# slinderman/theano_pyglm

Measured on AMD Instinct MI355X. Metric: population ll+grad evals/sec (N neurons x T bins), higher is better.
Workload: dtype f64

## Files before the change

include/pyglm_hip.h:

```cpp
#ifndef PYGLM_HIP_H
#define PYGLM_HIP_H

#include <stdint.h>

#ifdef __cplusplus
extern "C" {
#endif

typedef struct pgl_context* pgl_handle;

#define PGL_OK 0
#define PGL_ERR_ARG (-1)
#define PGL_ERR_HIP (-2)
#define PGL_ERR_STATE (-3)
#define PGL_ERR_UNSUPPORTED (-4)

#define PGL_NLIN_EXP 0
#define PGL_NLIN_EXPLINEAR 1

#define PGL_OPT_FEATURE_F32 1
#define PGL_OPT_NCHUNKS 2
#define PGL_OPT_KERNEL 3

#define PGL_OPT_GIBBS_KERNEL 4
#define PGL_OPT_EPI_F64 5

#define PGL_OPT_TIMING 6
#define PGL_OPT_BFGS_MERGE 7

#define PGL_OPT_RECORD_KERNELS 96


const char* pgl_last_error(void);
int pgl_version(void);
int pgl_device_count(void);

int pgl_create(int N, int64_t nT, int B, int R, int nlin, double dt, int device,
               pgl_handle* out);
int pgl_destroy(pgl_handle h);
int pgl_set_option(pgl_handle h, int option, int value);

int pgl_set_spikes_u8(pgl_handle h, const uint8_t* S);
int pgl_set_spikes_f64(pgl_handle h, const double* S);

int pgl_set_basis(pgl_handle h, const double* ibasis);

int pgl_set_stim_features(pgl_handle h, const double* fstim, int Dstim);

int pgl_set_stimulus(pgl_handle h, const double* stim, int64_t Tstim, int D, double dt_stim,
                     const double* basis_x, int Bx, const double* basis_t, int Rt, int Bt,
                     int layout);
int pgl_get_stim_features(pgl_handle h, double* fstim_out);

int pgl_set_stimulus_separable(pgl_handle h, const double* stim, int64_t Tstim, int D, double dt_stim,
                               const double* basis_x, int Bx, const double* basis_t, int Rt, int Bt);

int pgl_set_time_range(pgl_handle h, int64_t t_lo, int64_t t_hi);

int pgl_ll_grad(pgl_handle h, int n_lo, int n_hi, const double* theta,
                const double* Weff, double* ll_out, double* grad_out);

int pgl_ll_grad_dev(pgl_handle h, int n_lo, int n_hi, const double* d_theta,
                    const double* d_Weff, double* d_ll, double* d_grad);
int pgl_ll_grad_list_dev(pgl_handle h, const int* d_idx, int count, const double* d_theta,
                         const double* d_Weff, double* d_ll, double* d_grad);
int pgl_sync(pgl_handle h);

int pgl_hvp_prepare_dev(pgl_handle h, int n_lo, int n_hi, const double* d_theta, const double* d_Weff);
int pgl_hvp_prepare_list_dev(pgl_handle h, const int* d_idx, int count, const double* d_theta, const double* d_Weff);
int pgl_hvp_apply_dev(pgl_handle h, const double* d_v, double* d_hv);
int pgl_hvp(pgl_handle h, int n_lo, int n_hi, const double* theta, const double* v, const double* Weff, double* hv_out);

long long pgl_bfgs_state_doubles(int M, int P);
int pgl_bfgs_init_dev(pgl_handle h, double* d_state, int M, int P, double gtol);
int pgl_bfgs_trial_dev(pgl_handle h, double* d_state, int M, int P, const int* d_rows, int L, double* d_Xt);
int pgl_bfgs_objective_dev(pgl_handle h, int L, int P, const double* d_Xt, double* d_ll_f, double* d_grad_g,
                           int prior_kind, double mu_b, double sg_b, double stim_sigma, double mu, double sigma,
                           double lam);
int pgl_bfgs_linesearch_dev(pgl_handle h, double* d_state, int M, int P, const int* d_rows, int L, const double* d_Xt,
                            const double* d_f, const double* d_g, int max_trials);
int pgl_bfgs_hmul_dev(pgl_handle h, double* d_state, int M, int P, const int* d_rows, int L, double* d_H, int ld);
int pgl_bfgs_hmul_hist_dev(pgl_handle h, double* d_state, int M, int P, const int* d_rows, int L, const double* d_hist,
                           const double* d_coef, int Kmax, double* d_ab);
int pgl_bfgs_update_dev(pgl_handle h, double* d_state, int M, int P, double gtol, int maxiter, int init_scaling, double* d_hist,
                        double* d_coef, int Kmax);
int pgl_bfgs_step_dev(pgl_handle h, double* d_state, int M, int P, const int* d_rows, int L, const double* d_Xt, double* d_ll_f,
                      double* d_grad_g, int prior_kind, double mu_b, double sg_b, double stim_sigma, double mu, double sigma,
                      double lam, int max_trials, double gtol, int maxiter, int init_scaling, double* d_hist, double* d_coef,
                      int Kmax, double* d_ab, int hk_bound, double* d_H, int ld, const int* d_pos_next, double* d_Xt_next,
                      double* flags_out);

long long pgl_ncg_state_doubles(int M, int P);
int pgl_ncg_init_dev(pgl_handle h, double* d_state, int M, int P, double* d_ll, double* d_grad, int prior_kind, double mu_b,
                     double sg_b, double stim_sigma, double mu, double sigma, double lam, int maxiter, double* d_V,
                     double* flags_out);
int pgl_ncg_cg_step_dev(pgl_handle h, double* d_state, int M, int P, double* d_hv, int prior_kind, double mu_b, double sg_b,
                        double stim_sigma, double mu, double sigma, double lam, double* d_V, double* flags_out);
int pgl_ncg_trial_dev(pgl_handle h, double* d_state, int M, int P, const int* d_rows, int L, double* d_Xt);
int pgl_ncg_search_step_dev(pgl_handle h, double* d_state, int M, int P, const int* d_rows, int L, const double* d_Xt,
                            double* d_ll_f, double* d_grad_g, int prior_kind, double mu_b, double sg_b, double stim_sigma,
                            double mu, double sigma, double lam, int maxiter, const int* d_pos_next, double* d_Xt_next,
                            double* d_V, double* flags_out);

int pgl_features(pgl_handle h, double* fS_out);

int pgl_impulse_currents(pgl_handle h, const double* w, double* I_imp_out);

int pgl_state(pgl_handle h, int n, const double* theta_n, const double* Weff_col,
              double* lam_out, double* I_net_out, double* I_stim_out);

int pgl_ll_from_current(pgl_handle h, int n_post, double I_bias, const double* I_stim,
                        const double* I_other, const double* I_col, const double* w,
                        int K, double* ll_out);

int pgl_gibbs_prepare(pgl_handle h, int n_post, const double* theta_n,
                      const double* Weff_col);
int pgl_gibbs_ll(pgl_handle h, int n_pre, double aw_cur, const double* w, int K,
                 double* ll_out);
int pgl_gibbs_update(pgl_handle h, int n_pre, double delta);

int pgl_gibbs_prepare_all(pgl_handle h, const double* theta, const double* Weff);
int pgl_gibbs_ll_cols(pgl_handle h, int ncols, const int* n_post, const int* n_pre,
                      const double* aw_cur, const double* w, int K, double* ll_out);
int pgl_gibbs_update_cols(pgl_handle h, int ncols, const int* n_post, const int* n_pre,
                          const double* delta);
int pgl_gibbs_currents(pgl_handle h, int n_post, double* x_out);

int pgl_sta(pgl_handle h, const double* stim, int64_t Tstim, int D, double dt_stim, int L,
            const int* neurons, int n_sel, double* A_out);

int pgl_leading_singular_pairs(pgl_handle h, const double* A, int n, int L, int D, double* U, double* sigma, double* V);

int pgl_simulate(int N, int64_t nT, int R, int nlin, double dt, double* X, const double* AW,
                 const double* uniforms, int64_t n_uniforms, uint64_t seed, double* S,
                 int64_t* n_exceptions_out);

int pgl_last_timing(pgl_handle h, double* fused_ms, double* total_ms);

int pgl_timing_summary(pgl_handle h, int reset, int* n_launches, double* mean_fused_ms,
                       double* mean_total_ms);

int pgl_set_stream(pgl_handle h, void* stream);

int pgl_plan_kernels(int N, int B, int R, int Dstim, long long nT, int stim, int n_lo, int count, int path, int opt_kernel,
                     int opt_f32, char* out, int cap);

int pgl_last_kernels(pgl_handle h, char* out, int cap);

int pgl_info(pgl_handle h, int n_lo, int n_hi, double* info, int n_info);

#ifdef __cplusplus
}
#endif
#endif
```

theano_pyglm_amd/_lib.py:

```python
import ctypes as C
import os

import numpy as np

_HERE = os.path.dirname(os.path.abspath(__file__))
LIB_PATH = os.environ.get('PYGLM_HIP_LIB', os.path.join(_HERE, 'libpyglm_hip.so'))

NLIN_EXP = 0
NLIN_EXPLINEAR = 1
OPT_FEATURE_F32 = 1
OPT_NCHUNKS = 2
OPT_KERNEL = 3
OPT_GIBBS_KERNEL = 4
OPT_EPI_F64 = 5
OPT_TIMING = 6
OPT_BFGS_MERGE = 7
OPT_RECORD_KERNELS = 96

SYMBOLS = [
    'pgl_last_error', 'pgl_version', 'pgl_device_count', 'pgl_create', 'pgl_destroy',
    'pgl_set_option', 'pgl_set_time_range', 'pgl_set_spikes_u8', 'pgl_set_spikes_f64', 'pgl_set_basis',
    'pgl_set_stim_features', 'pgl_set_stimulus', 'pgl_get_stim_features', 'pgl_ll_grad', 'pgl_ll_grad_dev', 'pgl_sync', 'pgl_features',
    'pgl_impulse_currents', 'pgl_state', 'pgl_ll_from_current', 'pgl_gibbs_prepare',
    'pgl_gibbs_ll', 'pgl_gibbs_update', 'pgl_last_timing', 'pgl_info', 'pgl_simulate', 'pgl_sta',
    'pgl_timing_summary', 'pgl_set_stream',
    'pgl_set_stimulus_separable', 'pgl_ll_grad_list_dev', 'pgl_gibbs_prepare_all', 'pgl_gibbs_ll_cols', 'pgl_gibbs_update_cols', 'pgl_gibbs_currents',
    'pgl_bfgs_state_doubles', 'pgl_bfgs_init_dev', 'pgl_bfgs_trial_dev', 'pgl_bfgs_objective_dev',
    'pgl_bfgs_linesearch_dev', 'pgl_bfgs_hmul_dev', 'pgl_bfgs_hmul_hist_dev', 'pgl_bfgs_update_dev', 'pgl_bfgs_step_dev', 'pgl_plan_kernels', 'pgl_last_kernels', 'pgl_leading_singular_pairs',
    'pgl_hvp_prepare_dev', 'pgl_hvp_prepare_list_dev', 'pgl_hvp_apply_dev', 'pgl_hvp',
    'pgl_ncg_state_doubles', 'pgl_ncg_init_dev', 'pgl_ncg_cg_step_dev', 'pgl_ncg_trial_dev', 'pgl_ncg_search_step_dev',
]


class PglError(RuntimeError):
    pass


def plan_kernels(N, B=5, R=200, Dstim=0, nT=300000, stim=0, n_lo=0, count=None, path=0, opt_kernel=0, opt_f32=0):
    lib = load()
    buf = C.create_string_buffer(4096)
    rc = lib.pgl_plan_kernels(int(N), int(B), int(R), int(Dstim), int(nT), int(stim), int(n_lo), int(N - n_lo if count is None else count),
                              int(path), int(opt_kernel), int(opt_f32), buf, 4096)
    if rc != 0:
        raise PglError(lib.pgl_last_error().decode())
    return [ln for ln in buf.value.decode().splitlines() if ln]


_lib = None


def _preload_torch_hip():
    if os.environ.get('PYGLM_NO_TORCH_PRELOAD'):
        return
    try:
        import importlib.util
        spec = importlib.util.find_spec('torch')
        if spec is None or not spec.submodule_search_locations:
            return
        libdir = os.path.join(list(spec.submodule_search_locations)[0], 'lib')
        for name in ('libhsa-runtime64.so', 'libamdhip64.so'):
            path = os.path.join(libdir, name)
            if os.path.exists(path):
                C.CDLL(path, mode=C.RTLD_GLOBAL)
    except Exception:
        pass


def load():
    global _lib
    if _lib is not None:
        return _lib
    if not os.path.exists(LIB_PATH):
        raise PglError("HIP library %s not found: run `python -c 'import __graft_entry__ as g; "
                       "g.build()'` (hipcc --offload-arch=gfx950). There is no CPU fallback."
                       % LIB_PATH)
    _preload_torch_hip()
    lib = C.CDLL(LIB_PATH)
    dp = C.POINTER(C.c_double)
    vp = C.c_void_p
    lib.pgl_last_error.restype = C.c_char_p
    lib.pgl_last_error.argtypes = []
    lib.pgl_version.restype = C.c_int
    lib.pgl_device_count.restype = C.c_int
    lib.pgl_create.argtypes = [C.c_int, C.c_int64, C.c_int, C.c_int, C.c_int, C.c_double, C.c_int,
                               C.POINTER(vp)]
    lib.pgl_destroy.argtypes = [vp]
    lib.pgl_set_option.argtypes = [vp, C.c_int, C.c_int]
    lib.pgl_set_time_range.argtypes = [vp, C.c_int64, C.c_int64]
    lib.pgl_set_spikes_u8.argtypes = [vp, vp]
    lib.pgl_set_spikes_f64.argtypes = [vp, vp]
    lib.pgl_set_basis.argtypes = [vp, vp]
    lib.pgl_set_stim_features.argtypes = [vp, vp, C.c_int]
    lib.pgl_set_stimulus.argtypes = [vp, vp, C.c_int64, C.c_int, C.c_double, vp, C.c_int, vp, C.c_int,
                                     C.c_int, C.c_int]
    lib.pgl_get_stim_features.argtypes = [vp, vp]
    lib.pgl_set_stimulus_separable.argtypes = [vp, vp, C.c_int64, C.c_int, C.c_double, vp, C.c_int, vp, C.c_int,
                                               C.c_int]
    lib.pgl_timing_summary.argtypes = [vp, C.c_int, C.POINTER(C.c_int), C.POINTER(C.c_double), C.POINTER(C.c_double)]
    lib.pgl_set_stream.argtypes = [vp, vp]
    lib.pgl_sta.argtypes = [vp, vp, C.c_int64, C.c_int, C.c_double, C.c_int, vp, C.c_int, vp]
    if hasattr(lib, 'pgl_leading_singular_pairs'):
        lib.pgl_leading_singular_pairs.argtypes = [vp, vp, C.c_int, C.c_int, C.c_int, vp, vp, vp]
    lib.pgl_ll_grad.argtypes = [vp, C.c_int, C.c_int, vp, vp, vp, vp]
    lib.pgl_ll_grad_dev.argtypes = [vp, C.c_int, C.c_int, vp, vp, vp, vp]
    lib.pgl_ll_grad_list_dev.argtypes = [vp, vp, C.c_int, vp, vp, vp, vp]
    lib.pgl_sync.argtypes = [vp]
    if hasattr(lib, 'pgl_hvp'):
        lib.pgl_hvp_prepare_dev.argtypes = [vp, C.c_int, C.c_int, vp, vp]
        lib.pgl_hvp_prepare_list_dev.argtypes = [vp, vp, C.c_int, vp, vp]
        lib.pgl_hvp_apply_dev.argtypes = [vp, vp, vp]
        lib.pgl_hvp.argtypes = [vp, C.c_int, C.c_int, vp, vp, vp, vp]
    if hasattr(lib, 'pgl_bfgs_hmul_dev'):
        lib.pgl_bfgs_state_doubles.argtypes = [C.c_int, C.c_int]
        lib.pgl_bfgs_init_dev.argtypes = [vp, vp, C.c_int, C.c_int, C.c_double]
        lib.pgl_bfgs_trial_dev.argtypes = [vp, vp, C.c_int, C.c_int, vp, C.c_int, vp]
        lib.pgl_bfgs_objective_dev.argtypes = [vp, C.c_int, C.c_int, vp, vp, vp, C.c_int] + [C.c_double] * 6
        lib.pgl_bfgs_linesearch_dev.argtypes = [vp, vp, C.c_int, C.c_int, vp, C.c_int, vp, vp, vp, C.c_int]
        lib.pgl_bfgs_hmul_dev.argtypes = [vp, vp, C.c_int, C.c_int, vp, C.c_int, vp, C.c_int]
        lib.pgl_bfgs_update_dev.argtypes = [vp, vp, C.c_int, C.c_int, C.c_double, C.c_int, C.c_int, vp, vp, C.c_int]
        lib.pgl_bfgs_hmul_hist_dev.argtypes = [vp, vp, C.c_int, C.c_int, vp, C.c_int, vp, vp, C.c_int, vp]
    if hasattr(lib, 'pgl_bfgs_step_dev'):
        lib.pgl_bfgs_step_dev.argtypes = ([vp, vp, C.c_int, C.c_int, vp, C.c_int, vp, vp, vp, C.c_int] + [C.c_double] * 6 +
                                          [C.c_int, C.c_double, C.c_int, C.c_int, vp, vp, C.c_int, vp, C.c_int, vp, C.c_int,
                                           vp, vp, vp])
    if hasattr(lib, 'pgl_ncg_init_dev'):
        lib.pgl_ncg_state_doubles.argtypes = [C.c_int, C.c_int]
        lib.pgl_ncg_init_dev.argtypes = [vp, vp, C.c_int, C.c_int, vp, vp, C.c_int] + [C.c_double] * 6 + [C.c_int, vp, vp]
        lib.pgl_ncg_cg_step_dev.argtypes = [vp, vp, C.c_int, C.c_int, vp, C.c_int] + [C.c_double] * 6 + [vp, vp]
        lib.pgl_ncg_trial_dev.argtypes = [vp, vp, C.c_int, C.c_int, vp, C.c_int, vp]
        lib.pgl_ncg_search_step_dev.argtypes = ([vp, vp, C.c_int, C.c_int, vp, C.c_int, vp, vp, vp, C.c_int] +
                                                [C.c_double] * 6 + [C.c_int, vp, vp, vp, vp])
    lib.pgl_features.argtypes = [vp, vp]
    lib.pgl_impulse_currents.argtypes = [vp, vp, vp]
    lib.pgl_state.argtypes = [vp, C.c_int, vp, vp, vp, vp, vp]
    lib.pgl_ll_from_current.argtypes = [vp, C.c_int, C.c_double, vp, vp, vp, vp, C.c_int, vp]
    lib.pgl_gibbs_prepare.argtypes = [vp, C.c_int, vp, vp]
    lib.pgl_gibbs_ll.argtypes = [vp, C.c_int, C.c_double, vp, C.c_int, vp]
    lib.pgl_gibbs_update.argtypes = [vp, C.c_int, C.c_double]
    lib.pgl_gibbs_prepare_all.argtypes = [vp, vp, vp]
    lib.pgl_gibbs_ll_cols.argtypes = [vp, C.c_int, vp, vp, vp, vp, C.c_int, vp]
    lib.pgl_gibbs_update_cols.argtypes = [vp, C.c_int, vp, vp, vp]
    lib.pgl_gibbs_currents.argtypes = [vp, C.c_int, vp]
    lib.pgl_last_timing.argtypes = [vp, dp, dp]
    lib.pgl_info.argtypes = [vp, C.c_int, C.c_int, vp, C.c_int]
    if hasattr(lib, 'pgl_plan_kernels'):
        lib.pgl_plan_kernels.argtypes = [C.c_int, C.c_int, C.c_int, C.c_int, C.c_longlong, C.c_int, C.c_int, C.c_int, C.c_int,
                                         C.c_int, C.c_int, C.c_char_p, C.c_int]
    if hasattr(lib, 'pgl_last_kernels'):
        lib.pgl_last_kernels.argtypes = [vp, C.c_char_p, C.c_int]
    lib.pgl_simulate.argtypes = [C.c_int, C.c_int64, C.c_int, C.c_int, C.c_double, vp, vp, vp,
                                 C.c_int64, C.c_uint64, vp, vp]
    for name in SYMBOLS:
        if 'PYGLM_HIP_LIB' in os.environ and not hasattr(lib, name):
            continue
        fn = getattr(lib, name)
        if name in ('pgl_bfgs_state_doubles', 'pgl_ncg_state_doubles'):
            fn.restype = C.c_longlong
        elif name not in ('pgl_last_error',):
            fn.restype = C.c_int
    _lib = lib
    return lib


def device_count():
    return load().pgl_device_count()


def _chk(rc):
    if rc != 0:
        raise PglError("libpyglm_hip error %d: %s" % (rc, load().pgl_last_error().decode()))


def _f64(a, shape=None):
    a = np.ascontiguousarray(a, dtype=np.float64)
    if shape is not None and tuple(a.shape) != tuple(shape):
        raise ValueError("expected shape %s, got %s" % (shape, a.shape))
    return a


def _ptr(a):
    return None if a is None else a.ctypes.data_as(C.c_void_p)


def simulate(X0, AW, nlin, dt, uniforms=None, seed=0):
    lib = load()
    X = np.array(X0, dtype=np.float64, order='C')
    nT, N = X.shape
    AW = _f64(AW)
    assert AW.ndim == 3 and AW.shape[0] == N and AW.shape[2] == N
    R = AW.shape[1]
    S = np.empty((nT, N))
    u = None if uniforms is None else _f64(uniforms)
    nexc = C.c_int64(0)
    kind = {'exp': NLIN_EXP, 'explinear': NLIN_EXPLINEAR}.get(nlin, nlin)
    _chk(lib.pgl_simulate(N, nT, R, int(kind), float(dt), _ptr(X), _ptr(AW), _ptr(u),
                          0 if u is None else u.size, int(seed), _ptr(S), C.byref(nexc)))
    return S, X, int(nexc.value)


class DeviceGlm(object):

    def __init__(self, N, nT, B, R, nlin, dt, device=0):
        self.lib = load()
        self.N, self.nT, self.B, self.R, self.dt = int(N), int(nT), int(B), int(R), float(dt)
        self.nlin = {'exp': NLIN_EXP, 'explinear': NLIN_EXPLINEAR}.get(nlin, nlin)
        self.Dstim = 0
        h = C.c_void_p()
        _chk(self.lib.pgl_create(self.N, self.nT, self.B, self.R, int(self.nlin), self.dt,
                                 int(device), C.byref(h)))
        self.h = h

    def close(self):
        if getattr(self, 'h', None) is not None and self.h.value:
            self.lib.pgl_destroy(self.h)
            self.h = C.c_void_p()

    def __del__(self):
        try:
            self.close()
        except Exception:
            pass

    @property
    def P(self):
        return 1 + self.Dstim + self.N * self.B

    def set_option(self, opt, value):
        _chk(self.lib.pgl_set_option(self.h, int(opt), int(value)))

    def set_time_range(self, t_lo, t_hi):
        _chk(self.lib.pgl_set_time_range(self.h, int(t_lo), int(t_hi)))

    def set_spikes(self, S):
        S = np.asarray(S)
        if S.shape != (self.nT, self.N):
            raise ValueError("S must be (nT,N)=(%d,%d), got %s" % (self.nT, self.N, S.shape))
        if S.dtype == np.uint8:
            S = np.ascontiguousarray(S)
            _chk(self.lib.pgl_set_spikes_u8(self.h, _ptr(S)))
        else:
            S = _f64(S)
            _chk(self.lib.pgl_set_spikes_f64(self.h, _ptr(S)))

    def set_basis(self, ibasis):
        ib = _f64(ibasis, (self.R, self.B))
        _chk(self.lib.pgl_set_basis(self.h, _ptr(ib)))

    def set_stim_features(self, fstim):
        if fstim is None:
            _chk(self.lib.pgl_set_stim_features(self.h, None, 0))
            self.Dstim = 0
            return
        f = _f64(fstim)
        if f.ndim != 2 or f.shape[0] != self.nT:
            raise ValueError("fstim must be (nT,Dstim)")
        _chk(self.lib.pgl_set_stim_features(self.h, _ptr(f), int(f.shape[1])))
        self.Dstim = int(f.shape[1])

    def set_stimulus(self, stim, dt_stim, basis_t, basis_x=None, layout=0):
        stim = _f64(stim)
        if stim.ndim != 2:
            raise ValueError("stim must be (Tstim, D)")
        bt = _f64(basis_t)
        bx = None if basis_x is None else _f64(basis_x, (stim.shape[1], np.shape(basis_x)[1]))
        Bx = stim.shape[1] if bx is None else bx.shape[1]
        _chk(self.lib.pgl_set_stimulus(self.h, _ptr(stim), stim.shape[0], stim.shape[1], float(dt_stim),
                                       _ptr(bx), int(Bx), _ptr(bt), bt.shape[0], bt.shape[1],
                                       int(layout)))
        self.Dstim = int(Bx * bt.shape[1])

    def set_stimulus_separable(self, stim, dt_stim, basis_t, basis_x=None):
        stim = _f64(stim)
        if stim.ndim != 2:
            raise ValueError("stim must be (Tstim, D)")
        bt = _f64(basis_t)
        bx = None if basis_x is None else _f64(basis_x, (stim.shape[1], np.shape(basis_x)[1]))
        Bx = stim.shape[1] if bx is None else bx.shape[1]
        _chk(self.lib.pgl_set_stimulus_separable(self.h, _ptr(stim), stim.shape[0], stim.shape[1],
                                                 float(dt_stim), _ptr(bx), int(Bx), _ptr(bt), bt.shape[0],
                                                 bt.shape[1]))
        self.Dstim = int(Bx + bt.shape[1])

    def get_stim_features(self):
        out = np.empty((self.nT, self.Dstim))
# ... 21 lines not shown
            n, L, D = A.shape
        U, sig, V = np.empty((n, L)), np.empty(n), np.empty((n, D))
        _chk(self.lib.pgl_leading_singular_pairs(self.h, _ptr(A), n, L, D, _ptr(U), _ptr(sig), _ptr(V)))
        return U, sig, V

    def ll_grad(self, theta, Weff, n_lo=0, n_hi=None, want_grad=True):
        n_hi = self.N if n_hi is None else n_hi
        npost = n_hi - n_lo
        th = _f64(theta, (npost, self.P))
        We = _f64(Weff, (self.N, self.N))
        ll = np.empty(npost)
        g = np.empty((npost, self.P)) if want_grad else None
        _chk(self.lib.pgl_ll_grad(self.h, int(n_lo), int(n_hi), _ptr(th), _ptr(We), _ptr(ll),
                                  _ptr(g)))
        return ll, g

    def ll_grad_dev(self, d_theta, d_Weff, d_ll, d_grad, n_lo=0, n_hi=None):
        n_hi = self.N if n_hi is None else n_hi
        _chk(self.lib.pgl_ll_grad_dev(self.h, int(n_lo), int(n_hi), C.c_void_p(d_theta),
                                      C.c_void_p(d_Weff), C.c_void_p(d_ll),
                                      C.c_void_p(d_grad) if d_grad else None))

    def ll_grad_list_dev(self, d_idx, count, d_theta, d_Weff, d_ll, d_grad):
        _chk(self.lib.pgl_ll_grad_list_dev(self.h, C.c_void_p(d_idx), int(count), C.c_void_p(d_theta),
                                           C.c_void_p(d_Weff), C.c_void_p(d_ll),
                                           C.c_void_p(d_grad) if d_grad else None))

    def hvp_prepare(self, d_theta, d_Weff, n_lo=0, n_hi=None, d_idx=0, count=None):
        if d_idx:
            _chk(self.lib.pgl_hvp_prepare_list_dev(self.h, C.c_void_p(d_idx), int(count), C.c_void_p(d_theta),
                                                   C.c_void_p(d_Weff)))
            return
        n_hi = self.N if n_hi is None else n_hi
        _chk(self.lib.pgl_hvp_prepare_dev(self.h, int(n_lo), int(n_hi), C.c_void_p(d_theta), C.c_void_p(d_Weff)))

    def hvp_apply(self, d_v, d_hv):
        _chk(self.lib.pgl_hvp_apply_dev(self.h, C.c_void_p(d_v), C.c_void_p(d_hv)))

    def hvp(self, theta, v, Weff, n_lo=0, n_hi=None):
        n_hi = self.N if n_hi is None else n_hi
        npost = n_hi - n_lo
        th = _f64(theta, (npost, self.P))
        vv = _f64(v, (npost, self.P))
        We = _f64(Weff, (self.N, self.N))
        out = np.empty((npost, self.P))
        _chk(self.lib.pgl_hvp(self.h, int(n_lo), int(n_hi), _ptr(th), _ptr(vv), _ptr(We), _ptr(out)))
        return out

    def bfgs_state_doubles(self, M, P):
        return int(self.lib.pgl_bfgs_state_doubles(int(M), int(P)))

    def bfgs_trial_dev(self, d_state, M, P, d_rows, L, d_Xt):
        _chk(self.lib.pgl_bfgs_trial_dev(self.h, C.c_void_p(d_state), int(M), int(P),
                                         C.c_void_p(d_rows) if d_rows else None, int(L), C.c_void_p(d_Xt)))

    def bfgs_objective_dev(self, L, P, d_Xt, d_ll_f, d_grad_g, prior_kind, mu_b, sg_b, stim_sigma, mu, sigma, lam):
        _chk(self.lib.pgl_bfgs_objective_dev(self.h, int(L), int(P), C.c_void_p(d_Xt), C.c_void_p(d_ll_f),
                                             C.c_void_p(d_grad_g), int(prior_kind), float(mu_b), float(sg_b),
                                             float(stim_sigma), float(mu), float(sigma), float(lam)))

    def bfgs_init_dev(self, d_state, M, P, gtol):
        _chk(self.lib.pgl_bfgs_init_dev(self.h, C.c_void_p(d_state), int(M), int(P), float(gtol)))

    def bfgs_linesearch_dev(self, d_state, M, P, d_rows, L, d_Xt, d_f, d_g, max_trials=100):
        _chk(self.lib.pgl_bfgs_linesearch_dev(self.h, C.c_void_p(d_state), int(M), int(P),
                                              C.c_void_p(d_rows) if d_rows else None, int(L), C.c_void_p(d_Xt),
                                              C.c_void_p(d_f), C.c_void_p(d_g), int(max_trials)))

    def bfgs_hmul_dev(self, d_state, M, P, d_rows, L, d_H, ld):
        _chk(self.lib.pgl_bfgs_hmul_dev(self.h, C.c_void_p(d_state), int(M), int(P),
                                        C.c_void_p(d_rows) if d_rows else None, int(L), C.c_void_p(d_H), int(ld)))

    def bfgs_hmul_hist_dev(self, d_state, M, P, d_rows, L, d_hist, d_coef, Kmax, d_ab):
        _chk(self.lib.pgl_bfgs_hmul_hist_dev(self.h, C.c_void_p(d_state), int(M), int(P),
                                             C.c_void_p(d_rows) if d_rows else None, int(L), C.c_void_p(d_hist),
                                             C.c_void_p(d_coef), int(Kmax), C.c_void_p(d_ab)))

    def bfgs_update_dev(self, d_state, M, P, gtol, maxiter, init_scaling=False, d_hist=0, d_coef=0, Kmax=0):
        _chk(self.lib.pgl_bfgs_update_dev(self.h, C.c_void_p(d_state), int(M), int(P), float(gtol), int(maxiter),
                                          1 if init_scaling else 0, C.c_void_p(d_hist) if d_hist else None,
                                          C.c_void_p(d_coef) if d_coef else None, int(Kmax)))

    def bfgs_step_dev(self, d_state, M, P, d_rows, L, d_Xt, d_f, d_g, prior=None, max_trials=100, gtol=1e-5, maxiter=225,
                      init_scaling=False, d_hist=0, d_coef=0, Kmax=0, d_ab=0, hk_bound=0, d_H=0, ld=0, d_pos_next=0,
                      d_Xt_next=0, flags_out=0):
        vp = lambda a: C.c_void_p(a) if a else None
        pr = (-1, 0.0, 1.0, 1.0, 0.0, 1.0, 0.0) if prior is None else prior
        _chk(self.lib.pgl_bfgs_step_dev(self.h, C.c_void_p(d_state), int(M), int(P), vp(d_rows), int(L), C.c_void_p(d_Xt),
                                        C.c_void_p(d_f), C.c_void_p(d_g), int(pr[0]), *[float(z) for z in pr[1:]],
                                        int(max_trials), float(gtol), int(maxiter), 1 if init_scaling else 0, vp(d_hist),
                                        vp(d_coef), int(Kmax), vp(d_ab), int(hk_bound), vp(d_H), int(ld), vp(d_pos_next),
                                        vp(d_Xt_next), vp(flags_out)))

    def ncg_state_doubles(self, M, P):
        return int(self.lib.pgl_ncg_state_doubles(int(M), int(P)))

    def ncg_init_dev(self, d_state, M, P, d_ll, d_grad, prior, maxiter, d_V, flags_out=0):
        _chk(self.lib.pgl_ncg_init_dev(self.h, C.c_void_p(d_state), int(M), int(P), C.c_void_p(d_ll), C.c_void_p(d_grad),
                                       int(prior[0]), *[float(z) for z in prior[1:]], int(maxiter), C.c_void_p(d_V),
                                       C.c_void_p(flags_out) if flags_out else None))

    def ncg_cg_step_dev(self, d_state, M, P, d_hv, prior, d_V, flags_out=0):
        _chk(self.lib.pgl_ncg_cg_step_dev(self.h, C.c_void_p(d_state), int(M), int(P), C.c_void_p(d_hv), int(prior[0]),
                                          *[float(z) for z in prior[1:]], C.c_void_p(d_V),
                                          C.c_void_p(flags_out) if flags_out else None))

    def ncg_trial_dev(self, d_state, M, P, d_rows, L, d_Xt):
        _chk(self.lib.pgl_ncg_trial_dev(self.h, C.c_void_p(d_state), int(M), int(P),
                                        C.c_void_p(d_rows) if d_rows else None, int(L), C.c_void_p(d_Xt)))

    def ncg_search_step_dev(self, d_state, M, P, d_rows, L, d_Xt, d_f, d_g, prior, maxiter, d_pos_next, d_Xt_next, d_V,
                            flags_out=0):
        vp = lambda a: C.c_void_p(a) if a else None
        _chk(self.lib.pgl_ncg_search_step_dev(self.h, C.c_void_p(d_state), int(M), int(P), vp(d_rows), int(L),
                                              C.c_void_p(d_Xt), C.c_void_p(d_f), C.c_void_p(d_g), int(prior[0]),
                                              *[float(z) for z in prior[1:]], int(maxiter), vp(d_pos_next), vp(d_Xt_next),
                                              C.c_void_p(d_V), vp(flags_out)))

    def sync(self):
        _chk(self.lib.pgl_sync(self.h))

    def last_timing(self):
        a, b = C.c_double(), C.c_double()
        _chk(self.lib.pgl_last_timing(self.h, C.byref(a), C.byref(b)))
        return a.value, b.value

    def last_kernels(self):
        buf = C.create_string_buffer(16384)
        _chk(self.lib.pgl_last_kernels(self.h, buf, 16384))
        return [ln for ln in buf.value.decode().splitlines() if ln]

    def timing_summary(self, reset=True):
        n, a, b = C.c_int(), C.c_double(), C.c_double()
        _chk(self.lib.pgl_timing_summary(self.h, 1 if reset else 0, C.byref(n), C.byref(a), C.byref(b)))
        return n.value, a.value, b.value

    def set_stream(self, stream_ptr):
        if stream_ptr is None:
            _chk(self.lib.pgl_set_stream(self.h, None))
            return
        if int(stream_ptr) == 0:
            raise ValueError("stream handle 0 is the NULL stream: create a torch.cuda.Stream(), make it "
                             "current and pass its .cuda_stream")
        _chk(self.lib.pgl_set_stream(self.h, C.c_void_p(int(stream_ptr))))

    def info(self, n_lo=0, n_hi=None):
        n_hi = self.N if n_hi is None else n_hi
        v = np.zeros(13)
        _chk(self.lib.pgl_info(self.h, int(n_lo), int(n_hi), _ptr(v), 13))
        keys = ['blocks', 'threads', 'chunks', 'ktiles', 'lds_bytes', 'tile_rows', 'flops',
                'bytes', 'events', 'kernel_version', 'resident_feature_bytes', 'streamed_bytes', 'stim_path']
        return dict(zip(keys, v.tolist()))

    def features(self):
        out = np.empty((self.nT, self.N, self.B))
        _chk(self.lib.pgl_features(self.h, _ptr(out)))
        return out

    def impulse_currents(self, w):
        w = _f64(w, (self.N, self.B))
        out = np.empty((self.nT, self.N))
        _chk(self.lib.pgl_impulse_currents(self.h, _ptr(w), _ptr(out)))
        return out

    def state(self, n, theta_n, Weff_col):
        th = _f64(theta_n, (self.P,))
        wc = _f64(Weff_col, (self.N,))
        lam = np.empty(self.nT)
        inet = np.empty(self.nT)
        istim = np.empty(self.nT)
        _chk(self.lib.pgl_state(self.h, int(n), _ptr(th), _ptr(wc), _ptr(lam), _ptr(inet),
                                _ptr(istim)))
        return lam, inet, istim

    def ll_from_current(self, n_post, I_bias, I_stim, I_other, I_col, ws):
        ws = _f64(np.atleast_1d(ws))
        I_other = _f64(I_other, (self.nT,))
        I_col = _f64(I_col, (self.nT,))
        I_stim = None if I_stim is None else _f64(I_stim, (self.nT,))
        out = np.empty(len(ws))
        _chk(self.lib.pgl_ll_from_current(self.h, int(n_post), float(I_bias), _ptr(I_stim),
                                          _ptr(I_other), _ptr(I_col), _ptr(ws), len(ws),
                                          _ptr(out)))
        return out

    def gibbs_prepare(self, n_post, theta_n, Weff_col):
        th = _f64(theta_n, (self.P,))
        wc = _f64(Weff_col, (self.N,))
        _chk(self.lib.pgl_gibbs_prepare(self.h, int(n_post), _ptr(th), _ptr(wc)))

    def gibbs_ll(self, n_pre, aw_cur, ws):
        ws = _f64(np.atleast_1d(ws))
        out = np.empty(len(ws))
        _chk(self.lib.pgl_gibbs_ll(self.h, int(n_pre), float(aw_cur), _ptr(ws), len(ws),
                                   _ptr(out)))
        return out

    def gibbs_update(self, n_pre, delta):
        _chk(self.lib.pgl_gibbs_update(self.h, int(n_pre), float(delta)))

    def gibbs_prepare_all(self, theta, Weff):
        th = _f64(theta, (self.N, self.P))
        We = _f64(Weff, (self.N, self.N))
        _chk(self.lib.pgl_gibbs_prepare_all(self.h, _ptr(th), _ptr(We)))

    def gibbs_ll_cols(self, n_post, n_pre, aw_cur, ws):
        n_post = np.ascontiguousarray(n_post, dtype=np.int32)
        n_pre = np.ascontiguousarray(n_pre, dtype=np.int32)
        ws = _f64(ws)
        if ws.ndim == 1:
            ws = ws[None, :]
        aw = _f64(aw_cur, (len(n_post),))
        if n_pre.shape != n_post.shape or ws.shape[0] != len(n_post):
            raise ValueError("n_post, n_pre, aw_cur, ws must describe the same columns")
        out = np.empty(ws.shape)
        K = ws.shape[1]
        for k0 in range(0, K, 16):
            wk = np.ascontiguousarray(ws[:, k0:k0 + 16])
            ok = np.empty(wk.shape)
            _chk(self.lib.pgl_gibbs_ll_cols(self.h, len(n_post), _ptr(n_post), _ptr(n_pre), _ptr(aw),
                                            _ptr(wk), wk.shape[1], _ptr(ok)))
            out[:, k0:k0 + 16] = ok
        return out

    def gibbs_update_cols(self, n_post, n_pre, delta):
        n_post = np.ascontiguousarray(n_post, dtype=np.int32)
        n_pre = np.ascontiguousarray(n_pre, dtype=np.int32)
        d = _f64(delta, (len(n_post),))
        if len(n_post) == 0:
            return
        _chk(self.lib.pgl_gibbs_update_cols(self.h, len(n_post), _ptr(n_post), _ptr(n_pre), _ptr(d)))

    def gibbs_currents(self, n_post, nrows=None):
        out = np.empty(self.nT if nrows is None else int(nrows))
        _chk(self.lib.pgl_gibbs_currents(self.h, int(n_post), _ptr(out)))
        return out
```

theano_pyglm_amd/csrc/pglm_capi.hip:

```cpp
#include "pglm_kernels.hip.h"
#include "../../include/pyglm_hip.h"

#include <algorithm>
#include <cmath>
#include <cstdio>
#include <cstring>
#include <map>
#include <mutex>
#include <string>
#include <thread>
#include <type_traits>
#include <vector>

static thread_local std::string g_err;
static int fail(int code, const std::string& msg)
{
    g_err = msg;
    return code;
}
static thread_local std::vector<std::string>* g_dry = nullptr;
static thread_local std::vector<std::string>* g_rec = nullptr;
#define HIPCHK(expr)                                                                         \
    do {                                                                                     \
        hipError_t e_ = (expr);                                                              \
        if (e_ != hipSuccess)                                                                \
            return fail(PGL_ERR_HIP, std::string(#expr) + ": " + hipGetErrorString(e_));     \
    } while (0)

struct DevBuf {
    void* p = nullptr;
    size_t cap = 0;
};

struct pgl_context {
    int N = 0, B = 0, R = 0, nlin = 0, device = 0;
    int64_t nT = 0;
    double dt = 0;
    int Dstim = 0, Kimp = 0, Ktot = 0, nT16 = 0;
    int numCU = 256;
    hipStream_t stream = nullptr;
    hipStream_t own_stream = nullptr;
    hipStream_t aux_stream = nullptr;
    hipEvent_t ev_fork = nullptr, ev_join = nullptr;
    static constexpr int NEV = 256;
    hipEvent_t evr[NEV][4] = {};
    hipEvent_t* ev = evr[0];
    long long ev_launches = 0;
    bool have_spikes = false, have_basis = false;
    int64_t nnz = 0;
    DevBuf S, ST, spk, wlo, whi, phi, fstim;
    std::vector<int> h_ptr;
    std::vector<int2> h_ev;
    int Rk = 0;
    DevBuf theta, Weff, ll, grad, Wfrag, bias, Gpart, llpart, gbpart, Xbuf;
    struct ImgSlot {
        DevBuf buf;
        int key = 0, tile0 = 0, ntiles = 0;
        unsigned long long stamp = 0;
    };
    static constexpr int NIMG = 8;
    ImgSlot imgs[NIMG];
    int img_cur = 0;
    unsigned long long img_clock = 0;
    double* pin_out = nullptr;
    DevBuf IimpT, Inet, Istim, tmpA, tmpB, tmpC, wsmall, part, outK, lam, wcol, thetan;
    bool sep = false;
    int sepBt = 0, sepBx = 0, sepRt = 0;
    int64_t sepT = 0;
    double sep_dt_stim = 0;
    DevBuf zf, zfT, sbt, Yf, Qb, Qf, spart;
    bool sepf = false;
    int sepq = 0, sepM = 0, sepJ = 0, sepBTp = 0;
    int sepNH = 0, sepGs = 0;
    bool sepA_ok = false;
    DevBuf sepC, sepA, sepAT, sepD, YfT, Hb, wpart, QvT;
    int opt_sepf = 0;
    const int* cur_pidx = nullptr;
    int gibbs_npost = -1;
    double gibbs_bias = 0;
    DevBuf GX, gtheta, gargs, gpart, gout, ghs, gfs;
    DevBuf staA;
    int sta_n = 0, sta_L = 0, sta_D = 0;
    int gx_xs = 0;
    int64_t gx_t_lo = 0, gx_t_hi = 0;
    unsigned char* pin_args = nullptr;
    size_t pin_args_cap = 0;
    int opt_f32 = 0, opt_nchunks = 0, opt_dbg = 0, opt_kernel = 0, opt_ptw = 0, opt_gibbs = 0, opt_finw = 0, opt_sb6 = 0, opt_epi64 = 0, opt_timing = 1, opt_slice_cols = 0, opt_hlp = 0, opt_pbmajor = 0;
    int opt_img32 = 0;
    int opt_record = 0;
    std::vector<std::string> last_kernels;
    long long call_no = 0;
    int64_t t_lo = 0, t_hi = 0;
    bool timing_valid = false;
    double* flags_host[4] = {nullptr, nullptr, nullptr, nullptr};
    double* flags_dev[4] = {nullptr, nullptr, nullptr, nullptr};
    int flags_next = 0;
    int opt_bfgs_merge = 65536;
    bool hvp_ok = false, hvp_fused = false, hvp_list = false;
    int hvp_n_lo = 0, hvp_count = 0;
    int64_t hvp_t_lo = 0, hvp_t_hi = 0;
    DevBuf Cbuf, hvp_idx, hvp_Weff, hvp_ll, hvp_v, hvp_out;
    std::vector<double> hvp_host;
};

static int ensure(DevBuf& b, size_t bytes)
{
    if (g_dry) return PGL_OK;
    if (bytes <= b.cap && b.p) return PGL_OK;
    if (b.p) (void)hipFree(b.p);
    b.p = nullptr;
    b.cap = 0;
    if (bytes == 0) bytes = 16;
    HIPCHK(hipMalloc(&b.p, bytes));
    b.cap = bytes;
    return PGL_OK;
}
static void release(DevBuf& b)
{
    if (b.p) (void)hipFree(b.p);
    b.p = nullptr;
    b.cap = 0;
}
static int find_img(const pgl_context* h, int key, int tile0, int ntiles)
{
    for (int i = 0; i < pgl_context::NIMG; ++i)
        if (h->imgs[i].key == key && h->imgs[i].tile0 == tile0 && h->imgs[i].ntiles == ntiles && h->imgs[i].buf.p)
            return i;
    return -1;
}
static void invalidate_images(pgl_context* h)
{
    h->hvp_ok = false;
    for (int i = 0; i < pgl_context::NIMG; ++i) h->imgs[i].key = 0;
}
static bool img_room(const pgl_context* h, size_t want)
{
    size_t free_b = 0, total_b = 0;
    if (hipMemGetInfo(&free_b, &total_b) != hipSuccess) return true;
    size_t reclaim = 0;
    int lru = 0;
    for (int i = 1; i < pgl_context::NIMG; ++i)
        if (h->imgs[i].stamp < h->imgs[lru].stamp) lru = i;
    for (int i = 0; i < pgl_context::NIMG; ++i)
        if (h->imgs[i].key == 0) reclaim = std::max(reclaim, h->imgs[i].buf.cap);
    reclaim = std::max(reclaim, h->imgs[lru].buf.cap);
    return want <= reclaim || want - reclaim <= free_b / 10 * 9;
}
#define ENSURE(buf, bytes)                       \
    do {                                         \
        int rc_ = ensure(buf, bytes);            \
        if (rc_ != PGL_OK) return rc_;           \
    } while (0)

#include "pglm_plan.h"
#include "pglm_launch.h"

static int gibbs_rate_wg_per_cu(size_t lds)
{
    static std::map<size_t, int> cache;
    static std::mutex mu;
    std::lock_guard<std::mutex> lock(mu);
    int& c = cache[lds];
    if (c == 0) {
        int occ = 0;
        if (hipOccupancyMaxActiveBlocksPerMultiprocessor(&occ, k_gibbs_rate_cols, 256, lds) != hipSuccess || occ < 1)
            occ = 3;
        c = occ;
    }
    return c;
}

template <int J, int BT>
static void launch_sepf(int which, const SepfParams& sp, hipStream_t s);
static inline bool gemm_aligned(const void* p, long long ld) { return ((uintptr_t)p % 16) == 0 && (ld % 2) == 0; }

template <int J, int BT>
static void launch_sepf(int which, const SepfParams& sp, hipStream_t s)
{
    const long long nF = sp.F1 - sp.F0 + 1;
    const int nG = (sp.nPT + 3) / 4;
    dim3 grid((unsigned)((nF + 3) / 4), (unsigned)nG);
    if (which == 0) hipLaunchKernelGGL((k_sepf_fwd<J, BT>), grid, dim3(256), 0, s, sp);
    else if (which == 1) hipLaunchKernelGGL((k_sepf_bwd<J, BT>), grid, dim3(256), 0, s, sp);
    else {
        const int nA = (int)((sp.Tstim + 15) / 16) * nG;
        hipLaunchKernelGGL((k_sepf_finish<J, BT>), dim3(nA + nG * BT), dim3(1024), 0, s, sp, nA, nG);
    }
}

extern "C" {

const char* pgl_last_error(void) { return g_err.c_str(); }
int pgl_version(void) { return 103; }

int pgl_device_count(void)
{
    int n = 0;
    if (hipGetDeviceCount(&n) != hipSuccess) return 0;
    return n;
}

int pgl_create(int N, int64_t nT, int B, int R, int nlin, double dt, int device, pgl_handle* out)
{
    if (!out) return fail(PGL_ERR_ARG, "out is NULL");
    *out = nullptr;
    if (N <= 0 || nT <= 0 || B <= 0 || R <= 0) return fail(PGL_ERR_ARG, "N, nT, B, R must be positive");
    if (B > PGL_MAXB) return fail(PGL_ERR_UNSUPPORTED, "B > 8 basis functions");
    if (nlin != PGL_NLIN_EXP && nlin != PGL_NLIN_EXPLINEAR) return fail(PGL_ERR_ARG, "unknown nonlinearity");
    if (nT > (int64_t)1 << 30) return fail(PGL_ERR_UNSUPPORTED, "nT > 2^30 bins");
    if (!(dt > 0)) return fail(PGL_ERR_ARG, "dt must be positive");
    int ndev = 0;
    HIPCHK(hipGetDeviceCount(&ndev));
    if (ndev <= 0) return fail(PGL_ERR_HIP, "no HIP device visible");
    if (device < 0 || device >= ndev) return fail(PGL_ERR_ARG, "device index out of range");
    HIPCHK(hipSetDevice(device));
    pgl_context* h = new pgl_context();
    h->N = N; h->nT = nT; h->B = B; h->R = R; h->Rk = R; h->nlin = nlin; h->dt = dt; h->device = device;
    h->Kimp = N * B; h->Ktot = h->Kimp; h->nT16 = (int)((nT + 15) / 16);
    h->t_lo = 0; h->t_hi = nT;
    hipDeviceProp_t prop;
    if (hipGetDeviceProperties(&prop, device) == hipSuccess) h->numCU = prop.multiProcessorCount;
    hipError_t e = hipStreamCreateWithFlags(&h->own_stream, hipStreamNonBlocking);
    if (e != hipSuccess) { delete h; return fail(PGL_ERR_HIP, hipGetErrorString(e)); }
    h->stream = h->own_stream;
    {
        int prio_lo = 0, prio_hi = 0;
        if (hipDeviceGetStreamPriorityRange(&prio_lo, &prio_hi) != hipSuccess) prio_hi = 0;
        e = hipStreamCreateWithPriority(&h->aux_stream, hipStreamNonBlocking, prio_hi);
    }
    if (e == hipSuccess) e = hipEventCreateWithFlags(&h->ev_fork, hipEventDisableTiming);
    if (e == hipSuccess) e = hipEventCreateWithFlags(&h->ev_join, hipEventDisableTiming);
    if (e != hipSuccess) { pgl_destroy(h); return fail(PGL_ERR_HIP, hipGetErrorString(e)); }
    for (int s = 0; s < pgl_context::NEV; ++s)
        for (int i = 0; i < 4; ++i) {
            e = hipEventCreate(&h->evr[s][i]);
            if (e != hipSuccess) { pgl_destroy(h); return fail(PGL_ERR_HIP, hipGetErrorString(e)); }
        }
    *out = h;
    return PGL_OK;
}

int pgl_destroy(pgl_handle h)
{
    if (!h) return PGL_OK;
    (void)hipSetDevice(h->device);
    if (h->stream) (void)hipStreamSynchronize(h->stream);
    DevBuf* bufs[] = {&h->S, &h->ST, &h->spk, &h->wlo, &h->whi, &h->phi, &h->fstim, &h->theta,
                      &h->Weff, &h->ll, &h->grad, &h->Wfrag, &h->bias, &h->Gpart, &h->llpart,
                      &h->gbpart, &h->Xbuf, &h->imgs[0].buf, &h->imgs[1].buf, &h->imgs[2].buf, &h->imgs[3].buf, &h->imgs[4].buf, &h->imgs[5].buf, &h->imgs[6].buf, &h->imgs[7].buf, &h->IimpT, &h->Inet, &h->Istim, &h->tmpA, &h->tmpB, &h->tmpC,
                      &h->wsmall, &h->part, &h->outK, &h->lam, &h->wcol, &h->thetan, &h->GX, &h->gtheta,
                      &h->gargs, &h->gpart, &h->gout, &h->ghs, &h->gfs, &h->zf, &h->zfT, &h->sbt, &h->Yf, &h->Qb, &h->Qf,
                      &h->spart, &h->sepC, &h->sepA, &h->sepAT, &h->sepD, &h->YfT, &h->Hb, &h->wpart, &h->QvT, &h->staA,
                      &h->Cbuf, &h->hvp_idx, &h->hvp_Weff, &h->hvp_ll, &h->hvp_v, &h->hvp_out};
    for (DevBuf* b : bufs) release(*b);
    for (int s = 0; s < pgl_context::NEV; ++s)
        for (int i = 0; i < 4; ++i)
            if (h->evr[s][i]) (void)hipEventDestroy(h->evr[s][i]);
    if (h->pin_out) (void)hipHostFree(h->pin_out);
    if (h->pin_args) (void)hipHostFree(h->pin_args);
    if (h->ev_fork) (void)hipEventDestroy(h->ev_fork);
    if (h->ev_join) (void)hipEventDestroy(h->ev_join);
    if (h->aux_stream) { (void)hipStreamSynchronize(h->aux_stream); (void)hipStreamDestroy(h->aux_stream); }
    if (h->own_stream) (void)hipStreamDestroy(h->own_stream);
    delete h;
    return PGL_OK;
}

int pgl_set_time_range(pgl_handle h, int64_t t_lo, int64_t t_hi)
{
    if (!h) return fail(PGL_ERR_ARG, "null handle");
    if (t_lo < 0 || t_hi > h->nT || t_lo >= t_hi) return fail(PGL_ERR_ARG, "bad time range");
    if (t_lo % 16 != 0) return fail(PGL_ERR_ARG, "t_lo must be a multiple of 16 bins");
    h->t_lo = t_lo;
    h->t_hi = t_hi;
    return PGL_OK;
}

int pgl_set_option(pgl_handle h, int option, int value)
{
    if (!h) return fail(PGL_ERR_ARG, "null handle");
    switch (option) {
    case PGL_OPT_FEATURE_F32: h->opt_f32 = (value == 1) ? 1 : 0; h->opt_img32 = (value == 2) ? 1 : 0; return PGL_OK;
    case 99: h->opt_dbg = value; return PGL_OK;
    case 98: h->opt_ptw = value; return PGL_OK;
    case 97: if (value < 0 || value > 16) return fail(PGL_ERR_ARG, "finalize waves: 0 (auto) .. 16"); h->opt_finw = value; return PGL_OK;
    case 91: h->opt_pbmajor = value; return PGL_OK;
    case 92: h->opt_hlp = value; return PGL_OK;
    case 93: h->opt_slice_cols = value; return PGL_OK;
    case 94: h->opt_sepf = value; return PGL_OK;
    case 95: h->opt_sb6 = value; return PGL_OK;
    case PGL_OPT_RECORD_KERNELS: h->opt_record = value ? 1 : 0; h->last_kernels.clear(); return PGL_OK;
    case PGL_OPT_KERNEL: h->opt_kernel = value; return PGL_OK;
    case PGL_OPT_GIBBS_KERNEL: h->opt_gibbs = value; return PGL_OK;
    case PGL_OPT_EPI_F64: h->opt_epi64 = value ? 1 : 0; return PGL_OK;
    case PGL_OPT_TIMING: if (value < 0) return fail(PGL_ERR_ARG, "timing interval < 0"); h->opt_timing = value; h->call_no = 0; return PGL_OK;
    case PGL_OPT_BFGS_MERGE: if (value < 0) return fail(PGL_ERR_ARG, "merge threshold < 0"); h->opt_bfgs_merge = value; return PGL_OK;
    case PGL_OPT_NCHUNKS: if (value < 0) return fail(PGL_ERR_ARG, "nchunks < 0"); h->opt_nchunks = value; return PGL_OK;
    }
    return fail(PGL_ERR_ARG, "unknown option");
}

static int upload_windows(pgl_handle h)
{
    const int N = h->N, nT16 = h->nT16;
    const std::vector<int>& ptr = h->h_ptr;
    const std::vector<int2>& ev = h->h_ev;
    std::vector<int> wlo((size_t)nT16 * N), whi((size_t)nT16 * N);
    for (int n = 0; n < N; ++n) {
        int lo = ptr[n], hi = ptr[n];
        const int end = ptr[n + 1];
        for (int tile = 0; tile < nT16; ++tile) {
            const int64_t klo = (int64_t)16 * tile - h->Rk;
            const int64_t khi = (int64_t)16 * tile + 15;
            while (lo < end && ev[(size_t)lo].x < klo) ++lo;
            while (hi < end && ev[(size_t)hi].x < khi) ++hi;
            wlo[(size_t)tile * N + n] = lo;
            whi[(size_t)tile * N + n] = hi;
        }
    }
    ENSURE(h->wlo, wlo.size() * 4);
    ENSURE(h->whi, whi.size() * 4);
    HIPCHK(hipMemcpyAsync(h->wlo.p, wlo.data(), wlo.size() * 4, hipMemcpyHostToDevice, h->stream));
    HIPCHK(hipMemcpyAsync(h->whi.p, whi.data(), whi.size() * 4, hipMemcpyHostToDevice, h->stream));
    HIPCHK(hipStreamSynchronize(h->stream));
    return PGL_OK;
}

static int upload_spikes(pgl_handle h, const uint8_t* S)
{
    HIPCHK(hipSetDevice(h->device));
    const int N = h->N;
    const int64_t nT = h->nT;
    const int nth = (int)std::max<int64_t>(1, std::min<int64_t>(std::min<int64_t>(16, std::max(1u, std::thread::hardware_concurrency())),
                                                               nT / 65536));
    std::vector<int64_t> t0s(nth + 1);
    for (int i = 0; i <= nth; ++i) t0s[i] = nT * i / nth;
    std::vector<std::vector<int>> slab((size_t)nth, std::vector<int>((size_t)N, 0));
    auto run = [&](auto&& fn) {
        std::vector<std::thread> th;
        for (int i = 1; i < nth; ++i) th.emplace_back(fn, i);
        fn(0);
        for (auto& t : th) t.join();
    };
    run([&](const int i) {
        int* c = slab[(size_t)i].data();
        for (int64_t t = t0s[i]; t < t0s[i + 1]; ++t) {
            const uint8_t* row = S + t * N;
            for (int n = 0; n < N; ++n) c[n] += row[n] != 0;
        }
    });
    std::vector<int> cnt(N + 1, 0);
    for (int n = 0; n < N; ++n) {
        int tot = cnt[n];
        for (int i = 0; i < nth; ++i) {
            const int c = slab[(size_t)i][(size_t)n];
            slab[(size_t)i][(size_t)n] = tot;
            tot += c;
        }
        cnt[n + 1] = tot;
    }
    const int64_t nnz = cnt[N];
    std::vector<int2> ev((size_t)std::max<int64_t>(nnz, 1));
    run([&](const int i) {
        int* cur = slab[(size_t)i].data();
        for (int64_t t = t0s[i]; t < t0s[i + 1]; ++t) {
            const uint8_t* row = S + t * N;
            for (int n = 0; n < N; ++n)
                if (row[n]) ev[(size_t)cur[n]++] = make_int2((int)t, (int)row[n]);
        }
    });
    h->h_ptr = cnt;
    h->h_ev.swap(ev);
    const std::vector<int2>& evr = h->h_ev;
    const size_t s_rows = (size_t)h->nT16 * 16;
    ENSURE(h->S, s_rows * N);
    ENSURE(h->ST, (size_t)nT * N);
    ENSURE(h->spk, evr.size() * sizeof(int2));
    HIPCHK(hipMemsetAsync((uint8_t*)h->S.p + (size_t)nT * N, 0, (s_rows - (size_t)nT) * N, h->stream));
    HIPCHK(hipMemcpyAsync(h->S.p, S, (size_t)nT * N, hipMemcpyHostToDevice, h->stream));
    HIPCHK(hipMemcpyAsync(h->spk.p, evr.data(), evr.size() * sizeof(int2), hipMemcpyHostToDevice, h->stream));
    {
        const int rc = upload_windows(h);
        if (rc) return rc;
    }
    dim3 grid((unsigned)((nT + 63) / 64), (unsigned)((N + 63) / 64));
    hipLaunchKernelGGL(k_transpose_u8, grid, dim3(256), 0, h->stream, (const uint8_t*)h->S.p,
                       (uint8_t*)h->ST.p, (long long)nT, N);
    HIPCHK(hipGetLastError());
    HIPCHK(hipStreamSynchronize(h->stream));
    h->nnz = nnz;
    h->have_spikes = true;
    h->gibbs_npost = -1;
    invalidate_images(h);
    h->gx_xs = 0;
    return PGL_OK;
}

int pgl_set_spikes_u8(pgl_handle h, const uint8_t* S)
{
    if (!h || !S) return fail(PGL_ERR_ARG, "null argument");
    return upload_spikes(h, S);
}

int pgl_set_spikes_f64(pgl_handle h, const double* S)
{
    if (!h || !S) return fail(PGL_ERR_ARG, "null argument");
// ... 365 lines not shown
}

int pgl_sta(pgl_handle h, const double* stim, int64_t Tstim, int D, double dt_stim, int L,
            const int* neurons, int n_sel, double* A_out)
{
    if (!h || !stim) return fail(PGL_ERR_ARG, "null argument");
    if (!h->have_spikes) return fail(PGL_ERR_STATE, "pgl_set_spikes_* has not been called");
    if (Tstim <= 0 || D <= 0 || L <= 0 || !(dt_stim > 0)) return fail(PGL_ERR_ARG, "bad stimulus description");
    const int nSel = neurons ? n_sel : h->N;
    if (nSel <= 0 || nSel > 65535) return fail(PGL_ERR_ARG, "bad neuron selection");
    std::vector<int> eoff((size_t)2 * nSel);
    for (int i = 0; i < nSel; ++i) {
        const int n = neurons ? neurons[i] : i;
        if (n < 0 || n >= h->N) return fail(PGL_ERR_ARG, "neuron index out of range");
        eoff[2 * i] = h->h_ptr[n];
        eoff[2 * i + 1] = h->h_ptr[n + 1];
    }
    const long long LD = (long long)L * D;
    const long long xb = (LD + 255) / 256;
    if (xb > 0x7fffffffLL) return fail(PGL_ERR_UNSUPPORTED, "L*D too large");
    int echunks = (int)std::min<long long>(64, std::max<long long>(1, 4096 / (xb * nSel)));
    HIPCHK(hipSetDevice(h->device));
    DevBuf dstim, distim, deoff, dpart, dA;
    auto cleanup = [&]() { release(dstim); release(distim); release(deoff); release(dpart); release(dA); };
    auto keep = [&]() {
        release(h->staA);
        h->staA = dA;
        dA = DevBuf();
        h->sta_n = nSel; h->sta_L = L; h->sta_D = D;
    };
    const double ratio = dt_stim / h->dt;
    const long long q = llround(ratio);
    const bool frame_rate = q >= 1 && std::fabs(ratio - (double)q) <= 1e-9 * ratio && (Tstim % 2) == 0 && Tstim >= 2 &&
                            (long long)nSel * L * Tstim <= (1ll << 28) && h->opt_sepf != 7;
    int rc = ensure(dstim, (size_t)Tstim * D * 8);
    if (!rc && !frame_rate) rc = ensure(distim, (size_t)h->nT * D * 8);
    if (!rc) rc = ensure(deoff, eoff.size() * sizeof(int));
    if (!rc && !frame_rate) rc = ensure(dpart, (size_t)echunks * nSel * LD * 8);
    if (!rc) rc = ensure(dA, (size_t)nSel * LD * 8);
    if (rc) { cleanup(); return rc; }
    hipError_t e = hipMemcpyAsync(dstim.p, stim, (size_t)Tstim * D * 8, hipMemcpyHostToDevice, h->stream);
    if (e == hipSuccess)
        e = hipMemcpyAsync(deoff.p, eoff.data(), eoff.size() * sizeof(int), hipMemcpyHostToDevice, h->stream);
    if (frame_rate && e == hipSuccess) {
        DevBuf dW, dscale;
        std::vector<double> scale((size_t)nSel);
        for (int i = 0; i < nSel; ++i) {
            double cnt = 0.0;
            for (int j = eoff[2 * i]; j < eoff[2 * i + 1]; ++j) cnt += (double)h->h_ev[j].y;
            scale[i] = (h->dt / dt_stim) / cnt;
        }
        rc = ensure(dW, (size_t)nSel * L * Tstim * 8);
        if (!rc) rc = ensure(dscale, (size_t)nSel * 8);
        if (rc) { release(dW); release(dscale); cleanup(); return rc; }
        e = hipMemcpyAsync(dscale.p, scale.data(), (size_t)nSel * 8, hipMemcpyHostToDevice, h->stream);
        if (e == hipSuccess) {
            hipLaunchKernelGGL(k_sta_weights, dim3((unsigned)((Tstim + 255) / 256), (unsigned)L, (unsigned)nSel), dim3(256), 0,
                               h->stream, (const int2*)h->spk.p, (const int*)deoff.p, (const double*)dscale.p, L,
                               (long long)Tstim, (int)q, (double*)dW.p);
            e = hipGetLastError();
        }
        if (e == hipSuccess) {
            const int Mrows = nSel * L;
            hipLaunchKernelGGL((k_gemm_kc<1, 0, 16>), dim3((unsigned)((Mrows + 15) / 16), (unsigned)((D + 15) / 16)), dim3(512), 0,
                               h->stream, (const double*)dW.p, (long long)Tstim, (const double*)dstim.p, (long long)D,
                               (double*)dA.p, (long long)D, 1LL, Mrows, D, (int)Tstim);
            e = hipGetLastError();
        }
        if (e == hipSuccess && A_out)
            e = hipMemcpyAsync(A_out, dA.p, (size_t)nSel * LD * 8, hipMemcpyDeviceToHost, h->stream);
        if (e == hipSuccess) e = hipStreamSynchronize(h->stream);
        release(dW); release(dscale);
        if (e == hipSuccess && !A_out) keep();
        cleanup();
        if (e != hipSuccess) return fail(PGL_ERR_HIP, std::string("pgl_sta: ") + hipGetErrorString(e));
        return PGL_OK;
    }
    if (e == hipSuccess) {
        const long long total = (long long)h->nT * D;
        const int blocks = (int)std::min<long long>((total + 255) / 256, 65535);
        hipLaunchKernelGGL(k_stim_project, dim3(blocks), dim3(256), 0, h->stream, (const double*)dstim.p,
                           (long long)Tstim, D, dt_stim, h->dt, (const double*)nullptr, D,
                           (double*)distim.p, (long long)h->nT);
        e = hipGetLastError();
    }
    if (e == hipSuccess) {
        hipLaunchKernelGGL(k_sta, dim3((unsigned)xb, (unsigned)nSel, (unsigned)echunks), dim3(256), 0,
                           h->stream, (const int2*)h->spk.p, (const int*)deoff.p, (const double*)distim.p,
                           D, L, (double*)dpart.p);
        e = hipGetLastError();
    }
    if (e == hipSuccess) {
        hipLaunchKernelGGL(k_sta_finish, dim3((unsigned)xb, (unsigned)nSel), dim3(256), 0, h->stream,
                           (const double*)dpart.p, (const int2*)h->spk.p, (const int*)deoff.p, LD, echunks,
                           h->dt / dt_stim, (double*)dA.p);
        e = hipGetLastError();
    }
    if (e == hipSuccess && A_out)
        e = hipMemcpyAsync(A_out, dA.p, (size_t)nSel * LD * 8, hipMemcpyDeviceToHost, h->stream);
    if (e == hipSuccess) e = hipStreamSynchronize(h->stream);
    if (e == hipSuccess && !A_out) keep();
    cleanup();
    if (e != hipSuccess) return fail(PGL_ERR_HIP, std::string("pgl_sta: ") + hipGetErrorString(e));
    return PGL_OK;
}

int pgl_get_stim_features(pgl_handle h, double* fstim_out)
{
    if (h && h->sep) return fail(PGL_ERR_STATE, "a separable stimulus has no dense feature matrix");
    if (!h || !fstim_out) return fail(PGL_ERR_ARG, "null argument");
    if (h->Dstim <= 0) return fail(PGL_ERR_STATE, "no stimulus features on the device");
    HIPCHK(hipSetDevice(h->device));
    HIPCHK(hipMemcpyAsync(fstim_out, h->fstim.p, (size_t)h->nT * h->Dstim * 8, hipMemcpyDeviceToHost, h->stream));
    HIPCHK(hipStreamSynchronize(h->stream));
    return PGL_OK;
}

static int check_ready(pgl_handle h)
{
    if (!h) return fail(PGL_ERR_ARG, "null handle");
    if (!h->have_spikes) return fail(PGL_ERR_STATE, "pgl_set_spikes_* has not been called");
    if (!h->have_basis) return fail(PGL_ERR_STATE, "pgl_set_basis has not been called");
    return PGL_OK;
}

static void fill_params(pgl_handle h, const Plan& pl, const Slice& sl, int n_lo, bool want_grad,
                        int mode, FusedParams& fp)
{
    fp.nT = h->nT; fp.N = sl.Ns; fp.B = h->B; fp.R = h->Rk; fp.nlin = h->nlin;
    fp.Dstim = sl.Ds; fp.Kimp = sl.Ns * h->B; fp.Ktot = fp.Kimp + sl.Ds; fp.dt = h->dt;
    fp.Nall = h->N; fp.np0 = sl.np0; fp.DsAll = h->Dstim; fp.ds0 = sl.ds0;
    fp.mode = mode; fp.Xbuf = (double*)h->Xbuf.p; fp.xstride = pl.nPT * 16;
    fp.sepA = nullptr; fp.sepZ = nullptr; fp.sepTheta = nullptr; fp.sepT = 0;
    fp.sepLdy = fp.sepQ = fp.sepM = fp.sepNH = fp.sepG = fp.sepBt = 0;
    fp.sepAT = nullptr; fp.sepD = nullptr; fp.sepB0 = 0; fp.sepSL = 0;
    fp.spk = (const int2*)h->spk.p; fp.wlo = (const int*)h->wlo.p; fp.whi = (const int*)h->whi.p;
    fp.S = (const uint8_t*)h->S.p; fp.fstim = (const double*)h->fstim.p; fp.phi = (const double*)h->phi.p;
    fp.Wfrag = (const double*)h->Wfrag.p; fp.bias = (const double*)h->bias.p;
    fp.n_lo = n_lo; fp.npost = pl.npost; fp.nPT = pl.nPT;
    fp.nT16 = h->nT16; fp.tilesPerChunk = pl.tilesPerChunk; fp.nChunks = pl.nChunks; fp.nTiles = pl.nTiles;
    fp.pb_major = pl.pb_major;
    fp.rsf = pl.rsf;
    fp.RP = pl.RP;
    fp.Gpart = (double*)h->Gpart.p; fp.llpart = (double*)h->llpart.p; fp.gbpart = (double*)h->gbpart.p;
    fp.tile0 = pl.tile0;
    fp.t_hi = h->t_hi;
    fp.want_grad = want_grad ? 1 : 0;
    fp.dbg = h->opt_dbg;
    fp.Fimg = (const unsigned char*)h->imgs[h->img_cur].buf.p;
    fp.img_tile0 = h->imgs[h->img_cur].tile0;
    fp.pidx = h->cur_pidx;
    fp.theta = nullptr; fp.Weff = nullptr; fp.P = 1 + h->Dstim + h->Kimp;
    fp.epi64 = h->opt_epi64 ? 2 : 0;
}

static bool plan_reads_theta(const Plan& pl)
{
    return pl.version == 6 || (pl.version == 7 && pl.KS <= PGL_WREG_MAX);
}

static int launch_prep(pgl_handle h, const Plan& pl, const Slice& sl, int n_lo, const double* d_theta,
                       const double* d_Weff)
{
    if (g_dry) return PGL_OK;
    ENSURE(h->Wfrag, (size_t)pl.nPT * pl.KS * 64 * 8);
    ENSURE(h->bias, (size_t)pl.nPT * 16 * 8);
    const long long total = (long long)pl.nPT * pl.KS * 64;
    const int blocks = (int)std::min<long long>((total + 255) / 256, 1024);
    hipLaunchKernelGGL(k_prep_w, dim3(blocks), dim3(256), 0, h->stream, d_theta, d_Weff,
                       (double*)h->Wfrag.p, (double*)h->bias.p, sl.Ns, h->B, sl.Ds, sl.Ns * h->B,
                       sl.Ns * h->B + sl.Ds, pl.KS, n_lo, pl.npost, pl.nPT, 1,
                       h->N, sl.np0, h->Dstim, sl.ds0, h->cur_pidx);
    HIPCHK(hipGetLastError());
    return PGL_OK;
}

static int launch_finalize_grad(pgl_handle h, const Plan& pl, const Slice& sl, int n_lo,
                                const double* d_Weff, double* d_ll, double* d_grad, bool with_ll = false,
                                int kt0 = 0, int nkt = -1, hipStream_t stream = nullptr,
                                const double* wtpart = nullptr, int nwt = 0, int ldy = 0)
{
    if (g_dry) return PGL_OK;
    if (nkt < 0) nkt = pl.KT;
    if (!stream) stream = h->stream;
    const long long nfrag = (long long)pl.nPT * nkt * 256;
    int nwf = h->opt_finw > 0 ? h->opt_finw : std::max(4, std::min(8, pl.nChunks / 32));
    if (with_ll) nwf = std::max(nwf, 4);
    int blocks = (int)((nfrag + 63) / 64);
    if (with_ll) blocks += pl.npost;
    if (with_ll && wtpart) blocks += h->sepBt;
    hipLaunchKernelGGL(k_finalize, dim3(blocks), dim3(64 * nwf), 0, stream, (const double*)h->Gpart.p,
                       (const double*)h->llpart.p, (const double*)h->gbpart.p, d_Weff, d_ll, d_grad,
                       sl.Ns, h->B, sl.Ds, sl.Ns * h->B, sl.Ns * h->B + sl.Ds, pl.KT, n_lo, pl.npost,
                       pl.nPT, pl.nChunks, h->N, sl.np0, h->Dstim, sl.ds0, with_ll ? pl.KSPLIT : 0, kt0,
                       nkt, h->cur_pidx, wtpart, nwt, ldy, h->sepBt);
    HIPCHK(hipGetLastError());
    return PGL_OK;
}

static int ensure_feature_images(pgl_handle h, int ktl, int kth, int tile0, int ntiles, const Slice* sl = nullptr,
                                 int slice_no = 0, int blk = 0)
{
    if (g_dry) return PGL_OK;
    const int key = (sl ? (slice_no + 1) << 16 : 0) | (blk ? img_key6(ktl, blk) : ktl << 8 | kth);
    int slot = find_img(h, key, tile0, ntiles);
    if (slot >= 0) {
        h->img_cur = slot;
        h->imgs[slot].stamp = ++h->img_clock;
        return PGL_OK;
    }
    slot = 0;
    for (int i = 0; i < pgl_context::NIMG; ++i)
        if (h->imgs[i].key == 0) { slot = i; break; }
        else if (h->imgs[i].stamp < h->imgs[slot].stamp) slot = i;
    pgl_context::ImgSlot& im = h->imgs[slot];
    im.key = 0;
    const size_t bytes = (size_t)ntiles * (kth ? img_pair_bytes(ktl, kth) : img_bytes6(ktl, blk));
    if (bytes > im.buf.cap) {
        for (int i = 0; i < pgl_context::NIMG; ++i)
            if (i != slot && h->imgs[i].key == 0) release(h->imgs[i].buf);
    }
    ENSURE(im.buf, bytes);
    dim3 grid((unsigned)ntiles, kth ? 2 : 1);
    hipLaunchKernelGGL(k_build_fimg, grid, dim3(256), (size_t)h->B * h->Rk * 8, h->stream,
                       (const int2*)h->spk.p, (const int*)h->wlo.p, (const int*)h->whi.p,
                       (const double*)h->phi.p, (const double*)h->fstim.p, (long long)h->nT, sl ? sl->Ns : h->N, h->B,
                       h->Rk, sl ? sl->Ds : (h->sep ? 0 : h->Dstim), ktl, kth, tile0, (unsigned char*)im.buf.p,
                       h->N, sl ? sl->np0 : 0, h->Dstim, sl ? sl->ds0 : 0, blk);
    HIPCHK(hipGetLastError());
    im.key = key;
    im.tile0 = tile0;
    im.ntiles = ntiles;
    im.stamp = ++h->img_clock;
    h->img_cur = slot;
    return PGL_OK;
}


struct KernelRecord {
    explicit KernelRecord(pgl_context* h)
    {
        if (h->opt_record && !g_dry) {
            h->last_kernels.clear();
            g_rec = &h->last_kernels;
        }
    }
    ~KernelRecord() { g_rec = nullptr; }
};


static int ensure_partials(pgl_handle h, const std::vector<Plan>& plans, bool with_G)
{
    size_t maxG = 0, maxLL = 0;
    for (const Plan& pl : plans) {
        maxG = std::max(maxG, (size_t)pl.nChunks * pl.nPT * pl.KT * 256 * 8);
        maxLL = std::max(maxLL, (size_t)pl.nChunks * pl.nPT * pl.KSPLIT * 64 * 8);
    }
    ENSURE(h->llpart, maxLL);
    ENSURE(h->gbpart, maxLL);
    if (with_G) ENSURE(h->Gpart, maxG);
    return PGL_OK;
}

struct RowRange {
    int xs;
    long long row0, row1;
};
static RowRange row_range(const pgl_context* h, const Plan& p0)
{
    return RowRange{p0.nPT * 16, (long long)p0.tile0 * 16, std::min<long long>(h->nT, (long long)(p0.tile0 + p0.nTiles) * 16)};
}
static int zero_slab(pgl_handle h, double* X, const RowRange& rr)
{
    if (g_dry) return PGL_OK;
    HIPCHK(hipMemsetAsync(X + rr.row0 * rr.xs, 0, (size_t)(rr.row1 - rr.row0) * rr.xs * 8, h->stream));
    return PGL_OK;
}

static int ensure_tile_slab(pgl_handle h, const Plan& pl)
{
    const size_t need = (size_t)pl.nTiles * pl.nPT * 256 * 8;
    const bool fresh = need > h->Xbuf.cap || !h->Xbuf.p;
    ENSURE(h->Xbuf, need);
    if (fresh && !g_dry) HIPCHK(hipMemsetAsync(h->Xbuf.p, 0, need, h->stream));
    return PGL_OK;
}

static int ensure_plan_images(pgl_handle h, const Plan& pl)
{
    if (pl.version == 5) return ensure_feature_images(h, pl.ktl, pl.kth, pl.tile0, pl.nTiles);
    if (pl.version == 6 || pl.version == 7)
        return ensure_feature_images(h, pl.KT, 0, pl.tile0, pl.nTiles, nullptr, 0, (pl.version == 6 && pl.sb6 == 2) ? 1 + pl.img32 : 0);
    return PGL_OK;
}

static int launch_finalize_ll(pgl_handle h, const Plan& pl, double* d_ll, double* d_grad)
{
    if (g_dry) return PGL_OK;
    hipLaunchKernelGGL(k_finalize_ll, dim3(pl.npost), dim3(256), 0, h->stream, (const double*)h->llpart.p,
                       (const double*)h->gbpart.p, d_ll, d_grad, 1 + h->Dstim + h->Kimp, pl.npost, pl.nPT, pl.nChunks, pl.KSPLIT);
    HIPCHK(hipGetLastError());
    return PGL_OK;
}

static int forward_slices(pgl_handle h, const std::vector<Slice>& slices, const std::vector<Plan>& plans, int n_lo,
                          const double* d_theta, const double* d_Weff, double* X, int xs, const char* what)
{
    for (size_t i = 0; i < slices.size(); ++i) {
        int rc = launch_prep(h, plans[i], slices[i], n_lo, d_theta, d_Weff);
        if (rc) return rc;
        FusedParams fp;
        fill_params(h, plans[i], slices[i], n_lo, false, 1, fp);
        fp.Xbuf = X;
        fp.xstride = xs;
        hipError_t e = launch_plan(plans[i], fp, h->stream);
        if (e != hipSuccess) return fail(PGL_ERR_HIP, std::string(what) + hipGetErrorString(e));
    }
    return PGL_OK;
}

static int row_pass(pgl_handle h, const Plan& p0, const RowRange& rr, int n_lo, const double* c, double* d_ll, double* d_out)
{
    if (g_dry) return PGL_OK;
    const int rows = 512;
    const long long nrows = h->t_hi - h->t_lo;
    const int nblk = (int)((nrows + rows - 1) / rows);
    ENSURE(h->tmpA, (size_t)nblk * p0.npost * 8);
    ENSURE(h->tmpB, (size_t)nblk * p0.npost * 8);
    const dim3 grid((unsigned)nblk, (unsigned)((p0.npost + 255) / 256));
    if (c)
        hipLaunchKernelGGL(k_hvp_rows_mul, grid, dim3(256), 0, h->stream, (double*)h->Xbuf.p, c, rr.xs, (const double*)h->bias.p,
                           p0.npost, (long long)h->t_lo, (long long)h->t_hi, rows, (double*)h->tmpA.p, (double*)h->tmpB.p);
    else
        hipLaunchKernelGGL(k_rows_epilogue, grid, dim3(256), 0, h->stream, (double*)h->Xbuf.p, rr.xs, (const double*)h->bias.p,
                           (const uint8_t*)h->S.p, h->N, n_lo, p0.npost, (long long)h->t_lo, (long long)h->t_hi, rows, h->nlin,
                           h->dt, (double*)h->tmpA.p, (double*)h->tmpB.p, h->cur_pidx);
    HIPCHK(hipGetLastError());
    if (rr.row1 > h->t_hi) {
        hipLaunchKernelGGL(k_rows_zero, dim3(64), dim3(256), 0, h->stream, (double*)h->Xbuf.p, rr.xs, (long long)h->t_hi, rr.row1);
        HIPCHK(hipGetLastError());
    }
    hipLaunchKernelGGL(k_rows_reduce, dim3(p0.npost), dim3(64), 0, h->stream, (const double*)h->tmpA.p,
                       (const double*)h->tmpB.p, nblk, p0.npost, 1 + h->Dstim + h->Kimp, d_ll, d_out);
    HIPCHK(hipGetLastError());
    return PGL_OK;
}

static int backward_slices(pgl_handle h, const std::vector<Slice>& slices, const std::vector<Plan>& plans, int n_lo,
                           const double* d_theta, const double* d_Weff, double* d_ll, double* d_out)
{
    for (size_t i = 0; i < slices.size(); ++i) {
        int rc = launch_prep(h, plans[i], slices[i], n_lo, d_theta, d_Weff);
        if (rc) return rc;
        FusedParams fp;
        fill_params(h, plans[i], slices[i], n_lo, true, 2, fp);
        hipError_t e = launch_plan(plans[i], fp, h->stream);
        if (e != hipSuccess) return fail(PGL_ERR_HIP, std::string("backward launch: ") + hipGetErrorString(e));
        rc = launch_finalize_grad(h, plans[i], slices[i], n_lo, d_Weff, d_ll, d_out);
        if (rc) return rc;
    }
    return PGL_OK;
}

static int enqueue_ll_grad(pgl_handle h, int n_lo, int n_hi, const double* d_theta,
                           const double* d_Weff, double* d_ll, double* d_grad)
{
    KernelRecord record(h);
    std::vector<Slice> slices;
    std::vector<Plan> plans;
    bool sepf = false, sliced = false, wide = false;
    {
        int rc = select_plans(h, n_lo, n_hi, slices, plans, sepf, sliced, &wide);
        if (rc) return rc;
    }
    {
        int rc = ensure_partials(h, plans, d_grad != nullptr);
        if (rc) return rc;
    }

    const bool rec = h->opt_timing > 0 && (h->call_no++ % h->opt_timing) == 0;
    if (rec) {
        h->ev = h->evr[h->ev_launches % pgl_context::NEV];
        HIPCHK(hipEventRecord(h->ev[0], h->stream));
    }
    if (sepf) {
        const Plan& pl = plans[0];
        const bool direct = plan_reads_theta(pl);
        int rc = direct ? PGL_OK : launch_prep(h, pl, slices[0], n_lo, d_theta, d_Weff);
        if (rc) return rc;
        ENSURE(h->Xbuf, (size_t)pl.nTiles * pl.nPT * 256 * 8);
        rc = ensure_plan_images(h, pl);
        if (rc) return rc;
        if (rec) HIPCHK(hipEventRecord(h->ev[1], h->stream));
        SepfParams sp{};
        const bool fused_fwd = pl.version == 7 && fused7_built(pl.KT, pl.nw7, 2) && h->sepA_ok && h->opt_sepf != 3;
        const bool fused_bwd = fused_fwd && d_grad && fused7_built(pl.KT, pl.nw7, 3) && h->opt_sepf != 4;
        rc = sepf_forward(h, pl, d_theta, sp, fused_fwd);
        if (rc) return rc;
        if (fused_bwd && !g_dry) {
            const long long q = h->sepq, M = h->sepM;
            const long long tE = (long long)pl.tile0 + pl.nTiles - 1;
            sp.B0 = std::max<long long>(((long long)pl.tile0 * 16) / q - M, 0);
            sp.B1 = std::max<long long>((tE * 16) / q - M, 0);
            const long long span = ((M + 1) * q + 15) / 16 + 1;
            sp.SL = (int)(span / pl.tilesPerChunk) + 2;
            sp.tilesPerChunk = pl.tilesPerChunk;
            ENSURE(h->sepD, (size_t)(sp.B1 - sp.B0 + 1) * sp.SL * pl.nPT * 320 * 8);
            sp.D = (const double*)h->sepD.p;
        }
        FusedParams fp;
        fill_params(h, pl, slices[0], n_lo, d_grad != nullptr, 0, fp);
        if (direct) {
            fp.theta = d_theta;
            fp.Weff = d_Weff;
        }
        if (fused_fwd) {
            fp.sepA = (const double*)h->sepA.p; fp.sepZ = sp.YfT; fp.sepTheta = d_theta; fp.sepT = h->sepT;
            fp.sepLdy = sp.ldy; fp.sepQ = h->sepq; fp.sepM = h->sepM; fp.sepNH = h->sepNH; fp.sepG = h->sepGs;
            fp.sepBt = h->sepBt;
        }
        if (fused_bwd) {
            fp.sepAT = (const double*)h->sepAT.p; fp.sepD = (double*)h->sepD.p; fp.sepB0 = sp.B0; fp.sepSL = sp.SL;
        }
        hipError_t e = hipSuccess;
        if (pl.version == 5) {
            e = launch_fused5(pl, fp, h->stream, 1, 1);
            if (e == hipSuccess && d_grad) e = launch_fused5(pl, fp, h->stream, 2);
        } else {
            e = launch_fused7(pl, fp, h->stream, fused_bwd ? 3 : (fused_fwd ? 2 : 1));
        }
        if (e != hipSuccess) return fail(PGL_ERR_HIP, std::string("fused launch: ") + hipGetErrorString(e));
        if (d_grad) {
            int nwt = 0;
            rc = sepf_backward(h, sp, d_grad, fused_bwd, &nwt);
            if (rc) return rc;
            if (rec) HIPCHK(hipEventRecord(h->ev[2], h->stream));
            rc = launch_finalize_grad(h, pl, slices[0], n_lo, d_Weff, d_ll, d_grad, true, 0, -1, nullptr,
                                      fused_bwd ? (const double*)h->wpart.p : nullptr, nwt, sp.ldy);
            if (rc) return rc;
        } else {
            if (rec) HIPCHK(hipEventRecord(h->ev[2], h->stream));
            rc = launch_finalize_ll(h, pl, d_ll, d_grad);
            if (rc) return rc;
        }
    } else if (!sliced) {
        const Plan& pl = plans[0];
        const bool direct = plan_reads_theta(pl);
        int rc = direct ? PGL_OK : launch_prep(h, pl, slices[0], n_lo, d_theta, d_Weff);
        if (rc) return rc;
        if ((pl.version == 4 || pl.version == 5) && d_grad) {
            rc = ensure_tile_slab(h, pl);
            if (rc) return rc;
        }
        rc = ensure_plan_images(h, pl);
        if (rc) return rc;
        FusedParams fp;
        fill_params(h, pl, slices[0], n_lo, d_grad != nullptr, 0, fp);
        if (direct) {
            fp.theta = d_theta;
            fp.Weff = d_Weff;
        }
        if (rec) HIPCHK(hipEventRecord(h->ev[1], h->stream));
        hipError_t e = launch_plan(pl, fp, h->stream);
        if (e != hipSuccess) return fail(PGL_ERR_HIP, std::string("fused launch: ") + hipGetErrorString(e));
        if (rec) HIPCHK(hipEventRecord(h->ev[2], h->stream));
        rc = d_grad ? launch_finalize_grad(h, pl, slices[0], n_lo, d_Weff, d_ll, d_grad, true) : launch_finalize_ll(h, pl, d_ll, d_grad);
        if (rc) return rc;
    } else if (wide) {
        const Plan& p0 = plans[0];
        const size_t S = slices.size();
        ENSURE(h->Xbuf, (size_t)p0.nTiles * p0.nPT * 256 * 8);
        std::vector<int> slot(S);
        for (size_t i = 0; i < S; ++i) {
            int rc = ensure_feature_images(h, plans[i].ktl, plans[i].kth, p0.tile0, p0.nTiles, &slices[i], (int)i);
            if (rc) return rc;
            slot[i] = h->img_cur;
        }
        if (rec) HIPCHK(hipEventRecord(h->ev[1], h->stream));
        auto params = [&](const size_t i, FusedParams& fp) {
            h->img_cur = slot[i];
            fill_params(h, plans[i], slices[i], n_lo, d_grad != nullptr, 0, fp);
        };
        for (size_t i = 0; i < S; ++i) {
            int rc = launch_prep(h, plans[i], slices[i], n_lo, d_theta, d_Weff);
            if (rc) return rc;
            FusedParams fp;
            params(i, fp);
            const bool last = i + 1 == S;
            hipError_t e = launch_fused5_wide(plans[i], fp, h->stream, last ? 2 : (i == 0 ? 0 : 1));
            if (e == hipSuccess && last && d_grad) e = launch_fused5_wide(plans[i], fp, h->stream, 3);
            if (e != hipSuccess) return fail(PGL_ERR_HIP, std::string("wide launch: ") + hipGetErrorString(e));
        }
        if (d_grad) {
            int rc = launch_finalize_grad(h, plans[S - 1], slices[S - 1], n_lo, d_Weff, d_ll, d_grad, true);
            if (rc) return rc;
            for (size_t i = 0; i + 1 < S; ++i) {
                FusedParams fp;
                params(i, fp);
                hipError_t e = launch_fused5_wide(plans[i], fp, h->stream, 4);
                if (e == hipSuccess) e = launch_fused5_wide(plans[i], fp, h->stream, 3);
                if (e != hipSuccess) return fail(PGL_ERR_HIP, std::string("wide backward launch: ") + hipGetErrorString(e));
                rc = launch_finalize_grad(h, plans[i], slices[i], n_lo, d_Weff, d_ll, d_grad);
                if (rc) return rc;
            }
        } else {
            int rc = launch_finalize_ll(h, plans[S - 1], d_ll, d_grad);
            if (rc) return rc;
        }
        if (rec) HIPCHK(hipEventRecord(h->ev[2], h->stream));
    } else {
        const Plan& p0 = plans[0];
        const RowRange rr = row_range(h, p0);
        ENSURE(h->Xbuf, (size_t)h->nT * rr.xs * 8);
        double* X = (double*)h->Xbuf.p;
        int rc = zero_slab(h, X, rr);
        if (rc) return rc;
        if (rec) HIPCHK(hipEventRecord(h->ev[1], h->stream));
        SepParams sp;
        if (h->sep) {
            if (h->cur_pidx) return fail(PGL_ERR_UNSUPPORTED, "neuron lists with a separable stimulus");
            rc = sep_forward(h, d_theta, p0.npost, X, rr.xs, h->t_lo, h->t_hi, sp);
            if (rc) return rc;
        }
        rc = forward_slices(h, slices, plans, n_lo, d_theta, d_Weff, X, rr.xs, "forward launch: ");
        if (rc) return rc;
        rc = row_pass(h, p0, rr, n_lo, nullptr, d_ll, d_grad);
        if (rc) return rc;
        if (d_grad) {
            rc = backward_slices(h, slices, plans, n_lo, d_theta, d_Weff, d_ll, d_grad);
            if (rc) return rc;
            if (h->sep) {
                rc = sep_backward(h, sp, d_grad);
                if (rc) return rc;
            }
        }
        if (rec) HIPCHK(hipEventRecord(h->ev[2], h->stream));
    }
    if (rec) HIPCHK(hipEventRecord(h->ev[3], h->stream));
    h->timing_valid = rec;
    if (rec) ++h->ev_launches;
    return PGL_OK;
}

int pgl_ll_grad_dev(pgl_handle h, int n_lo, int n_hi, const double* d_theta, const double* d_Weff,
                    double* d_ll, double* d_grad)
{
    int rc = check_ready(h);
    if (rc) return rc;
    if (!d_theta || !d_Weff || !d_ll) return fail(PGL_ERR_ARG, "null argument");
    HIPCHK(hipSetDevice(h->device));
    if (n_lo < 0 || n_hi > h->N || n_lo >= n_hi) return fail(PGL_ERR_ARG, "bad neuron range");
    return enqueue_ll_grad(h, n_lo, n_hi, d_theta, d_Weff, d_ll, d_grad);
}

int pgl_ll_grad_list_dev(pgl_handle h, const int* d_idx, int count, const double* d_theta,
                         const double* d_Weff, double* d_ll, double* d_grad)
{
    int rc = check_ready(h);
    if (rc) return rc;
    if (!d_idx || !d_theta || !d_Weff || !d_ll) return fail(PGL_ERR_ARG, "null argument");
    if (count <= 0 || count > h->N) return fail(PGL_ERR_ARG, "bad neuron count");
    HIPCHK(hipSetDevice(h->device));
    h->cur_pidx = d_idx;
    rc = enqueue_ll_grad(h, 0, count, d_theta, d_Weff, d_ll, d_grad);
    h->cur_pidx = nullptr;
    return rc;
}



static int enqueue_hvp_prepare(pgl_handle h, int n_lo, int n_hi, const double* d_theta, const double* d_Weff)
{
    KernelRecord record(h);
    std::vector<Slice> slices;
    std::vector<Plan> plans;
    bool fused = false;
    int rc = hvp_select(h, n_lo, n_hi, slices, plans, fused);
    if (rc) return rc;
    rc = ensure_partials(h, plans, false);
    if (rc) return rc;
    const Plan& p0 = plans[0];
    const RowRange rr = row_range(h, p0);
    long long total = 0;
    double* cb = nullptr;
    if (fused) {
        total = (long long)p0.nTiles * p0.nPT * 256;
        ENSURE(h->Cbuf, (size_t)total * 8);
        cb = (double*)h->Cbuf.p;
        rc = launch_prep(h, p0, slices[0], n_lo, d_theta, d_Weff);
        if (rc) return rc;
        rc = ensure_plan_images(h, p0);
        if (rc) return rc;
        FusedParams fp;
        fill_params(h, p0, slices[0], n_lo, false, 0, fp);
        fp.Xbuf = cb;
        hipError_t e = launch_hvp5(p0, fp, nullptr, h->stream, 1);
        if (e != hipSuccess) return fail(PGL_ERR_HIP, std::string("curvature forward launch: ") + hipGetErrorString(e));
    } else {
        total = (rr.row1 - rr.row0) * rr.xs;
        ENSURE(h->Cbuf, (size_t)h->nT * rr.xs * 8);
        cb = (double*)h->Cbuf.p + rr.row0 * rr.xs;
        rc = zero_slab(h, (double*)h->Cbuf.p, rr);
        if (rc) return rc;
        rc = forward_slices(h, slices, plans, n_lo, d_theta, d_Weff, (double*)h->Cbuf.p, rr.xs, "curvature forward launch: ");
        if (rc) return rc;
    }
    if (!g_dry) {
        const int blocks = (int)std::min<long long>((total + 255) / 256, 8 * 1024);
        hipLaunchKernelGGL(k_hvp_curv, dim3(blocks), dim3(256), 0, h->stream, cb, (const double*)h->bias.p,
                           (const uint8_t*)h->S.p, h->N, n_lo, p0.npost, h->cur_pidx, rr.xs, rr.row0, (long long)h->t_hi, total,
                           fused ? 1 : 0, h->nlin, h->dt);
        HIPCHK(hipGetLastError());
    }
    h->hvp_fused = fused;
    return PGL_OK;
}

static int enqueue_hvp_apply(pgl_handle h, const double* d_v, double* d_hv)
{
    KernelRecord record(h);
    const int n_lo = h->hvp_list ? 0 : h->hvp_n_lo, n_hi = n_lo + h->hvp_count;
    const double* d_Weff = (const double*)h->hvp_Weff.p;
    std::vector<Slice> slices;
    std::vector<Plan> plans;
    bool fused = false;
    int rc = hvp_select(h, n_lo, n_hi, slices, plans, fused);
    if (rc) return rc;
    if (fused != h->hvp_fused) return fail(PGL_ERR_STATE, "the dispatch changed since pgl_hvp_prepare_*: prepare again");
    rc = ensure_partials(h, plans, true);
// ... 388 lines not shown
    int rc = check_ready(h);
    if (rc) return rc;
    if (!theta || !Weff || !ll_out) return fail(PGL_ERR_ARG, "null argument");
    HIPCHK(hipSetDevice(h->device));
    if (n_lo < 0 || n_hi > h->N || n_lo >= n_hi) return fail(PGL_ERR_ARG, "bad neuron range");
    const size_t P = 1 + (size_t)h->Dstim + h->Kimp;
    const size_t np = (size_t)(n_hi - n_lo);
    ENSURE(h->theta, np * P * 8);
    ENSURE(h->Weff, (size_t)h->N * h->N * 8);
    ENSURE(h->ll, np * 8);
    if (grad_out) ENSURE(h->grad, np * P * 8);
    HIPCHK(hipMemcpyAsync(h->theta.p, theta, np * P * 8, hipMemcpyHostToDevice, h->stream));
    HIPCHK(hipMemcpyAsync(h->Weff.p, Weff, (size_t)h->N * h->N * 8, hipMemcpyHostToDevice, h->stream));
    rc = enqueue_ll_grad(h, n_lo, n_hi, (const double*)h->theta.p, (const double*)h->Weff.p,
                         (double*)h->ll.p, grad_out ? (double*)h->grad.p : nullptr);
    if (rc) return rc;
    HIPCHK(hipMemcpyAsync(ll_out, h->ll.p, np * 8, hipMemcpyDeviceToHost, h->stream));
    if (grad_out)
        HIPCHK(hipMemcpyAsync(grad_out, h->grad.p, np * P * 8, hipMemcpyDeviceToHost, h->stream));
    HIPCHK(hipStreamSynchronize(h->stream));
    return PGL_OK;
}

int pgl_last_timing(pgl_handle h, double* fused_ms, double* total_ms)
{
    if (!h) return fail(PGL_ERR_ARG, "null handle");
    if (!h->timing_valid) return fail(PGL_ERR_STATE, "the last pgl_ll_grad call recorded no events (none yet, or PGL_OPT_TIMING skipped it)");
    HIPCHK(hipSetDevice(h->device));
    HIPCHK(hipEventSynchronize(h->ev[3]));
    float a = 0, b = 0;
    HIPCHK(hipEventElapsedTime(&a, h->ev[1], h->ev[2]));
    HIPCHK(hipEventElapsedTime(&b, h->ev[0], h->ev[3]));
    if (fused_ms) *fused_ms = a;
    if (total_ms) *total_ms = b;
    return PGL_OK;
}

int pgl_timing_summary(pgl_handle h, int reset, int* n_launches, double* mean_fused_ms, double* mean_total_ms)
{
    if (!h) return fail(PGL_ERR_ARG, "null handle");
    HIPCHK(hipSetDevice(h->device));
    HIPCHK(hipStreamSynchronize(h->stream));
    const long long n = std::min<long long>(h->ev_launches, pgl_context::NEV);
    double sa = 0, sb = 0;
    for (long long i = 0; i < n; ++i) {
        hipEvent_t* ev = h->evr[(h->ev_launches - 1 - i) % pgl_context::NEV];
        float a = 0, b = 0;
        HIPCHK(hipEventElapsedTime(&a, ev[1], ev[2]));
        HIPCHK(hipEventElapsedTime(&b, ev[0], ev[3]));
        sa += a;
        sb += b;
    }
    if (n_launches) *n_launches = (int)n;
    if (mean_fused_ms) *mean_fused_ms = n ? sa / n : 0.0;
    if (mean_total_ms) *mean_total_ms = n ? sb / n : 0.0;
    if (reset) h->ev_launches = 0;
    return PGL_OK;
}

int pgl_set_stream(pgl_handle h, void* stream)
{
    if (!h) return fail(PGL_ERR_ARG, "null handle");
    HIPCHK(hipSetDevice(h->device));
    HIPCHK(hipStreamSynchronize(h->stream));
    h->stream = stream ? (hipStream_t)stream : h->own_stream;
    h->ev_launches = 0;
    h->timing_valid = false;
    return PGL_OK;
}

static int enqueue_gibbs_forward(pgl_handle h);

int pgl_last_kernels(pgl_handle h, char* out, int cap)
{
    if (!h || !out || cap <= 0) return fail(PGL_ERR_ARG, "null argument");
    if (!h->opt_record) return fail(PGL_ERR_STATE, "kernel recording is off (PGL_OPT_RECORD_KERNELS)");
    std::string all;
    for (const std::string& n : h->last_kernels) all += n + "\n";
    if ((int)all.size() + 1 > cap) return fail(PGL_ERR_ARG, "output buffer too small");
    std::memcpy(out, all.c_str(), all.size() + 1);
    return PGL_OK;
}

int pgl_plan_kernels(int N, int B, int R, int Dstim, long long nT, int stim, int n_lo, int count, int path, int opt_kernel,
                     int opt_f32, char* out, int cap)
{
    if (!out || cap <= 0) return fail(PGL_ERR_ARG, "null argument");
    if (N <= 0 || B <= 0 || B > PGL_MAXB || R <= 0 || nT <= 0 || Dstim < 0 || count <= 0 || n_lo < 0 || n_lo + count > N)
        return fail(PGL_ERR_ARG, "bad shape");
    pgl_context c;
    c.N = N; c.B = B; c.R = R; c.Rk = R; c.nT = nT; c.Dstim = Dstim; c.Kimp = N * B;
    c.nT16 = (int)((nT + 15) / 16); c.t_lo = 0; c.t_hi = nT; c.numCU = 256;
    c.sep = stim >= 1; c.sepf = stim >= 2; c.sepA_ok = stim == 2; c.opt_sepf = 0;
    c.Ktot = c.Kimp + (c.sep ? 0 : Dstim);
    c.opt_kernel = opt_kernel; c.opt_f32 = (opt_f32 == 1) ? 1 : 0; c.opt_img32 = (opt_f32 == 2) ? 1 : 0;
    c.opt_timing = 0;
    std::vector<std::string> names;
    double dummy = 0;
    int rc = PGL_OK;
    if (path == 3 || path == 4) {
        if (c.sep) return fail(PGL_ERR_UNSUPPORTED, "Hessian-vector products with a separable stimulus");
        std::vector<std::string> prep;
        g_dry = (path == 3) ? &names : &prep;
        rc = enqueue_hvp_prepare(&c, n_lo, n_lo + count, nullptr, nullptr);
        if (rc == PGL_OK && path == 4) {
            c.hvp_n_lo = n_lo;
            c.hvp_count = count;
            g_dry = &names;
            rc = enqueue_hvp_apply(&c, nullptr, &dummy);
        }
    } else {
        g_dry = &names;
        rc = (path == 2) ? enqueue_gibbs_forward(&c)
                         : enqueue_ll_grad(&c, n_lo, n_lo + count, nullptr, nullptr, &dummy, path == 0 ? &dummy : nullptr);
    }
    g_dry = nullptr;
    if (rc == PGL_ERR_HIP) return fail(PGL_ERR_UNSUPPORTED, "no kernel instantiation for this plan");
    if (rc) return rc;
    std::string all;
    for (const std::string& n : names) all += n + "\n";
    if ((int)all.size() + 1 > cap) return fail(PGL_ERR_ARG, "output buffer too small");
    std::memcpy(out, all.c_str(), all.size() + 1);
    return PGL_OK;
}

int pgl_info(pgl_handle h, int n_lo, int n_hi, double* info, int n_info)
{
    if (!h || !info) return fail(PGL_ERR_ARG, "null argument");
    std::vector<Slice> slices;
    std::vector<Plan> plans;
    bool sepf = false, sliced = false, wide = false;
    int rc = select_plans(h, n_lo, n_hi, slices, plans, sepf, sliced, &wide);
    if (rc) return rc;
    const int stim_path = sepf ? 2 : (h->sep ? 1 : 0);
    const Plan& pl = plans[0];
    const double P = 1.0 + h->Dstim + h->Kimp;
    double v[13];
    v[12] = stim_path;
    v[9] = pl.version;
    v[10] = (pl.version == 5) ? (double)pl.nTiles * (double)img_pair_bytes(pl.ktl, pl.kth)
            : (pl.version == 6 || pl.version == 7) ? (double)pl.nTiles * (double)img_bytes6(pl.KT, (pl.version == 6 && pl.sb6 == 2) ? 1 + pl.img32 : 0) : 0.0;
    v[11] = (pl.version == 5) ? v[10] + (double)pl.nTiles * pgl_img_bytes(pl.kth) + 2.0 * (double)pl.nTiles * pl.nPT * 2048.0
            : (pl.version == 4) ? 2.0 * (double)pl.nTiles * pl.nPT * 2048.0
            : (pl.version == 6 || pl.version == 7) ? v[10] * pl.nPB : 0.0;
    if (wide) {
        v[10] = v[11] = 0.0;
        for (const Plan& q : plans) {
            const double b = (double)q.nTiles * (double)img_pair_bytes(q.ktl, q.kth);
            v[10] += b;
            v[11] += 2.0 * b * q.nPB;
        }
        v[11] += 2.0 * (double)plans.size() * (double)pl.nTiles * pl.nPT * 2048.0;
    }
    v[0] = pl.blocks; v[1] = pl.threads; v[2] = pl.nChunks; v[3] = pl.KT; v[4] = (double)pl.lds;
    v[5] = 16;
    const double nrows = (double)(h->t_hi - h->t_lo);
    v[6] = 4.0 * nrows * (double)h->Ktot * (double)pl.npost;
    v[7] = nrows * h->N + (h->sep ? (double)h->sepT * h->sepBx * 8.0 : nrows * h->Dstim * 8.0) + 8.0 * pl.npost * P +
           8.0 * pl.npost * (1.0 + P);
    v[8] = (double)h->nnz;
    for (int i = 0; i < n_info && i < 13; ++i) info[i] = v[i];
    return PGL_OK;
}

int pgl_features(pgl_handle h, double* fS_out)
{
    int rc = check_ready(h);
    if (rc) return rc;
    if (!fS_out) return fail(PGL_ERR_ARG, "null argument");
    HIPCHK(hipSetDevice(h->device));
    const size_t bytes = (size_t)h->nT * h->Kimp * 8;
    ENSURE(h->tmpA, bytes);
    hipLaunchKernelGGL(k_features, dim3(h->nT16), dim3(256), (size_t)h->B * h->Rk * 8, h->stream,
                       (const int2*)h->spk.p, (const int*)h->wlo.p, (const int*)h->whi.p,
                       (const double*)h->phi.p, (double*)h->tmpA.p, (long long)h->nT, h->N, h->B, h->Rk);
    HIPCHK(hipGetLastError());
    HIPCHK(hipMemcpyAsync(fS_out, h->tmpA.p, bytes, hipMemcpyDeviceToHost, h->stream));
    HIPCHK(hipStreamSynchronize(h->stream));
    return PGL_OK;
}

static int enqueue_impulse_T(pgl_handle h, const double* d_w)
{
    ENSURE(h->IimpT, (size_t)h->N * h->nT * 8);
    const int blocks = (int)((h->nT + 63) / 64);
    const size_t lds = ((size_t)h->B * h->Rk + (size_t)h->N * h->B) * 8;
    hipLaunchKernelGGL(k_impulse_T, dim3(blocks), dim3(256), lds, h->stream, (const int2*)h->spk.p,
                       (const int*)h->wlo.p, (const int*)h->whi.p, (const double*)h->phi.p, d_w,
                       (double*)h->IimpT.p, (long long)h->nT, h->nT16, h->N, h->B, h->Rk);
    HIPCHK(hipGetLastError());
    return PGL_OK;
}

int pgl_impulse_currents(pgl_handle h, const double* w, double* I_imp_out)
{
    int rc = check_ready(h);
    if (rc) return rc;
    if (!w || !I_imp_out) return fail(PGL_ERR_ARG, "null argument");
    HIPCHK(hipSetDevice(h->device));
    ENSURE(h->wsmall, (size_t)h->Kimp * 8);
    HIPCHK(hipMemcpyAsync(h->wsmall.p, w, (size_t)h->Kimp * 8, hipMemcpyHostToDevice, h->stream));
    rc = enqueue_impulse_T(h, (const double*)h->wsmall.p);
    if (rc) return rc;
    h->gibbs_npost = -1;
    std::vector<double> T((size_t)h->N * h->nT);
    HIPCHK(hipMemcpyAsync(T.data(), h->IimpT.p, T.size() * 8, hipMemcpyDeviceToHost, h->stream));
    HIPCHK(hipStreamSynchronize(h->stream));
    for (int n = 0; n < h->N; ++n)
        for (int64_t t = 0; t < h->nT; ++t) I_imp_out[(size_t)t * h->N + n] = T[(size_t)n * h->nT + t];
    return PGL_OK;
}

int pgl_gibbs_prepare(pgl_handle h, int n_post, const double* theta_n, const double* Weff_col)
{
    int rc = check_ready(h);
    if (rc) return rc;
    if (!theta_n || !Weff_col) return fail(PGL_ERR_ARG, "null argument");
    if (n_post < 0 || n_post >= h->N) return fail(PGL_ERR_ARG, "n_post out of range");
    HIPCHK(hipSetDevice(h->device));
    const size_t P = 1 + (size_t)h->Dstim + h->Kimp;
    ENSURE(h->thetan, P * 8);
    ENSURE(h->wcol, (size_t)h->N * 8);
    ENSURE(h->Inet, (size_t)h->nT * 8);
    ENSURE(h->Istim, (size_t)h->nT * 8);
    HIPCHK(hipMemcpyAsync(h->thetan.p, theta_n, P * 8, hipMemcpyHostToDevice, h->stream));
    HIPCHK(hipMemcpyAsync(h->wcol.p, Weff_col, (size_t)h->N * 8, hipMemcpyHostToDevice, h->stream));
    const double* d_th = (const double*)h->thetan.p;
    rc = enqueue_impulse_T(h, d_th + 1 + h->Dstim);
    if (rc) return rc;
    hipLaunchKernelGGL(k_inet, dim3(1024), dim3(256), 0, h->stream, (const double*)h->IimpT.p,
                       (const double*)h->wcol.p, (const double*)h->fstim.p, d_th + 1,
                       (double*)h->Inet.p, (double*)h->Istim.p, (long long)h->nT, h->N, h->sep ? 0 : h->Dstim);
    HIPCHK(hipGetLastError());
    if (h->sep) {
        SepParams sp;
        rc = sep_forward(h, d_th, 1, (double*)h->Istim.p, 1, 0, h->nT, sp);
        if (rc) return rc;
    }
    HIPCHK(hipStreamSynchronize(h->stream));
    h->gibbs_npost = n_post;
    h->gibbs_bias = theta_n[0];
    return PGL_OK;
}

static int run_ll_current(pgl_handle h, const double* d_base, const double* d_stim,
                          const double* d_col, int n_post, double bias, double aw_cur,
                          const double* w, int K, double* ll_out)
{
    const int nblocks = (int)std::min<int64_t>(1024, (h->t_hi - h->t_lo + 255) / 256);
    const int2* evb = h->h_ev.data();
    const auto before = [](const int2& e, int64_t t) { return (int64_t)e.x < t; };
    const int e_lo = (int)(std::lower_bound(evb + h->h_ptr[n_post], evb + h->h_ptr[n_post + 1], h->t_lo, before) - evb);
    const int e_hi = (int)(std::lower_bound(evb + h->h_ptr[n_post], evb + h->h_ptr[n_post + 1], h->t_hi, before) - evb);
    const int sblocks = std::max(1, std::min(256, (e_hi - e_lo + 255) / 256));
    ENSURE(h->part, (size_t)(nblocks + sblocks) * PGL_KMAX * 8);
    ENSURE(h->outK, PGL_KMAX * 8);
    if (!h->pin_out) HIPCHK(hipHostMalloc((void**)&h->pin_out, PGL_KMAX * 8, hipHostMallocDefault));
    for (int k0 = 0; k0 < K; k0 += PGL_KMAX) {
        const int kk = std::min(PGL_KMAX, K - k0);
        PglWeights wv;
        for (int k = 0; k < PGL_KMAX; ++k) wv.w[k] = (k < kk) ? w[k0 + k] : 0.0;
        hipLaunchKernelGGL(k_ll_current, dim3(nblocks), dim3(256), 0, h->stream, d_base, d_stim,
                           d_col, bias, aw_cur, wv, kk, h->nlin, h->dt,
                           (long long)h->t_lo, (long long)h->t_hi, (double*)h->part.p);
        HIPCHK(hipGetLastError());
        hipLaunchKernelGGL(k_ll_current_spikes, dim3(sblocks), dim3(256), 0, h->stream,
                           (const int2*)h->spk.p, e_lo, e_hi, d_base, d_stim, d_col, bias, aw_cur,
                           wv, kk, h->nlin,
                           (double*)h->part.p + (size_t)nblocks * PGL_KMAX);
        HIPCHK(hipGetLastError());
        hipLaunchKernelGGL(k_reduce_parts, dim3(kk), dim3(64), 0, h->stream, (const double*)h->part.p,
                           nblocks + sblocks, kk, (double*)h->outK.p);
        HIPCHK(hipGetLastError());
        HIPCHK(hipMemcpyAsync(h->pin_out, h->outK.p, (size_t)kk * 8, hipMemcpyDeviceToHost, h->stream));
        HIPCHK(hipStreamSynchronize(h->stream));
        std::memcpy(ll_out + k0, h->pin_out, (size_t)kk * 8);
    }
    return PGL_OK;
}

int pgl_gibbs_ll(pgl_handle h, int n_pre, double aw_cur, const double* w, int K, double* ll_out)
{
    int rc = check_ready(h);
    if (rc) return rc;
    if (h->gibbs_npost < 0) return fail(PGL_ERR_STATE, "pgl_gibbs_prepare has not been called");
    if (!w || !ll_out || K <= 0) return fail(PGL_ERR_ARG, "bad argument");
    if (n_pre < 0 || n_pre >= h->N) return fail(PGL_ERR_ARG, "n_pre out of range");
    HIPCHK(hipSetDevice(h->device));
    const double* col = (const double*)h->IimpT.p + (size_t)n_pre * h->nT;
    return run_ll_current(h, (const double*)h->Inet.p, (const double*)h->Istim.p, col,
                          h->gibbs_npost, h->gibbs_bias, aw_cur, w, K, ll_out);
}

int pgl_gibbs_update(pgl_handle h, int n_pre, double delta)
{
    int rc = check_ready(h);
    if (rc) return rc;
    if (h->gibbs_npost < 0) return fail(PGL_ERR_STATE, "pgl_gibbs_prepare has not been called");
    if (n_pre < 0 || n_pre >= h->N) return fail(PGL_ERR_ARG, "n_pre out of range");
    HIPCHK(hipSetDevice(h->device));
    const double* col = (const double*)h->IimpT.p + (size_t)n_pre * h->nT;
    hipLaunchKernelGGL(k_axpy, dim3(1024), dim3(256), 0, h->stream, (double*)h->Inet.p, col, delta,
                       (long long)h->nT);
    HIPCHK(hipGetLastError());
    return PGL_OK;
}

int pgl_gibbs_prepare_all(pgl_handle h, const double* theta, const double* Weff)
{
    int rc = check_ready(h);
    if (rc) return rc;
    if (!theta || !Weff) return fail(PGL_ERR_ARG, "null argument");
    HIPCHK(hipSetDevice(h->device));
    const size_t P = 1 + (size_t)h->Dstim + h->Kimp;
// ... 461 lines not shown
```

theano_pyglm_amd/csrc/pglm_common.hip.h:

```cpp
#pragma once
#include <hip/hip_runtime.h>
#include <stdint.h>
#include <type_traits>

typedef double d4_t __attribute__((ext_vector_type(4)));

#define PGL_CAP 16
#ifndef PGL_PD
#define PGL_PD 4
#endif
#ifndef PGL_PW
#define PGL_PW 8
#endif
#define PGL_MAXB 8
#ifdef PGL_ABLATE
#define PGL_DBG(bit) ((p.dbg & (bit)) != 0)
#else
#define PGL_DBG(bit) (false)
#endif
#ifndef PGL_PRIO
#define PGL_PRIO 1
#ifndef PGL_EPI_PRIO
#define PGL_EPI_PRIO 1
#endif
#endif
#ifndef PGL_EBAR
#define PGL_EBAR 1
#endif
#ifndef PGL_EPI_F32
#define PGL_EPI_F32 1
#endif
#ifndef PGL_DS1
#define PGL_DS1 4
#endif
#ifndef PGL_ENE
#define PGL_ENE 4
#endif

#ifndef PGL_DMA_IL
#define PGL_DMA_IL 1
#endif
#ifndef PGL_WREG_MAX
#define PGL_WREG_MAX 28
#endif
#ifndef PGL_LDS1
#define PGL_LDS1 1
#endif
__device__ __forceinline__ double pgl_lds_f64(const double* p)
{
#if PGL_LDS1
    return *(const volatile __attribute__((address_space(3))) double*)p;
#else
    return *p;
#endif
}

__device__ __forceinline__ double* pgl_gpart(double* G, const int pt, const int KT, const int kt0,
                                             const int nChunks, const int chunk, const int lane)
{
    return G + (((size_t)pt * KT + kt0) * 4) * ((size_t)nChunks * 64) + (size_t)chunk * 64 + lane;
}

struct FusedParams {
    long long nT;
    int N, B, R, nlin;
    int Dstim, Kimp, Ktot;
    double dt;
    const int2* __restrict__ spk;
    const int* __restrict__ wlo;
    const int* __restrict__ whi;
    const uint8_t* __restrict__ S;
    const double* __restrict__ fstim;
    const double* __restrict__ phi;
    const double* __restrict__ Wfrag;
    const double* __restrict__ bias;
    int n_lo, npost, nPT;
    int nT16, tilesPerChunk, nChunks, nTiles;
    int rsf;
    int RP;
    double* __restrict__ Gpart;
    double* __restrict__ llpart;
    double* __restrict__ gbpart;
    int Nall, np0, DsAll, ds0;
    int mode;
    double* __restrict__ Xbuf;
    int xstride;
    int tile0;
    long long t_hi;
    int want_grad;
    int dbg;
    const unsigned char* __restrict__ Fimg;
    int img_tile0;
    const int* __restrict__ pidx;
    const double* __restrict__ theta;
    const double* __restrict__ Weff;
    int P;
    int epi64;
    const double* __restrict__ sepA;
    const double* __restrict__ sepZ;
    const double* __restrict__ sepTheta;
    long long sepT;
    int sepLdy, sepQ, sepM, sepNH, sepG;
    int sepBt;
    const double* __restrict__ sepAT;
    double* __restrict__ sepD;
    long long sepB0;
    int sepSL;
    int pb_major;
};

__device__ __forceinline__ void pgl_store_ll(const FusedParams& p, const int chunk, const int pt, const int sub,
                                             const int nsub, const int lane, double ll, double gb)
{
    ll += __shfl_xor(ll, 16, 64);
    gb += __shfl_xor(gb, 16, 64);
    ll += __shfl_xor(ll, 32, 64);
    gb += __shfl_xor(gb, 32, 64);
    if (lane < 16) {
        const size_t o = (((size_t)pt * 16 + lane) * p.nChunks + chunk) * nsub + sub;
        p.llpart[o] = ll;
        p.gbpart[o] = gb;
    }
}

__device__ __forceinline__ long long pgl_sepd_first_tile(const long long b, const int M, const int q, const long long tile0)
{
    const long long t = (b <= 0) ? 0 : ((b + M) * (long long)q + 15) / 16;
    return t > tile0 ? t : tile0;
}

template <int NS>
__device__ __forceinline__ void pgl_wfrag_direct(const FusedParams& p, const int ks0, const int grp, const int nloc,
                                                 const int nglob, const bool valid_n, double (&w)[NS])
{
    const double* row = p.theta + (size_t)(valid_n ? nloc : 0) * p.P;
    const double* wcol = p.Weff + (valid_n ? nglob : 0);
    const int imp0 = 1 + p.DsAll + p.np0 * p.B, st0 = 1 + p.ds0 - p.Kimp;
    const float rB = 1.0f / (float)p.B;
    double tv[NS], wv[NS];
#pragma unroll
    for (int s = 0; s < NS; ++s) {
        const int k = 4 * (ks0 + s) + grp;
        const int kc = (k < p.Ktot) ? k : 0;
        const bool imp = kc < p.Kimp;
        const int npre = p.np0 + (int)(((float)(imp ? kc : 0) + 0.5f) * rB);
        tv[s] = row[(imp ? imp0 : st0) + kc];
        wv[s] = wcol[(size_t)npre * p.Nall];
    }
#pragma unroll
    for (int s = 0; s < NS; ++s) {
        const int k = 4 * (ks0 + s) + grp;
        const double v = (k < p.Kimp) ? tv[s] * wv[s] : tv[s];
        w[s] = (valid_n && k < p.Ktot) ? v : 0.0;
    }
}

__constant__ double PGL_C[32] = {
    1.4426950408889634,
    6.93147180369123816490e-01,
    1.90821492927058770002e-10,
    1.6059043836821613e-10,
    2.08767569878681e-09,
    2.505210838544172e-08,
    2.755731922398589e-07,
    2.7557319223985893e-06,
    2.48015873015873e-05,
    0.0001984126984126984,
    0.001388888888888889,
    0.008333333333333333,
    0.041666666666666664,
    0.16666666666666666,
    1.479819860511658591e-01,
    1.531383769920937332e-01,
    1.818357216161805012e-01,
    2.222219843214978396e-01,
    2.857142874366239149e-01,
    3.999999999940941908e-01,
    6.666666666666735130e-01,
    0.70710678118654752440,
    1.0 / 3.0,
    9.6e-5,
    0, 0, 0, 0, 0, 0, 0, 0};

__device__ __forceinline__ double pgl_rcp(const double b)
{
    double r = __builtin_amdgcn_rcp(b);
    r = fma(fma(-b, r, 1.0), r, r);
    r = fma(fma(-b, r, 1.0), r, r);
    return r;
}

template <typename CP>
__device__ __forceinline__ double pgl_exp(const double y, const CP C)
{
    const double k = rint(y * C[0]);
    double r = fma(-k, C[1], y);
    r = fma(-k, C[2], r);
    double p = C[3];
#pragma unroll
    for (int i = 4; i <= 13; ++i) p = fma(p, r, C[i]);
    p = fma(p, r, 0.5);
    p = fma(p, r, 1.0);
    p = fma(p, r, 1.0);
    const double kc = fmin(fmax(k, -2200.0), 2200.0);
    return ldexp(p, (int)kc);
}

template <typename CP>
__device__ __forceinline__ double pgl_log(const double v, const CP C)
{
    double m = __builtin_amdgcn_frexp_mant(v);
    int e = __builtin_amdgcn_frexp_exp(v);
    const bool lt = m < C[21];
    m = lt ? m + m : m;
    e = lt ? e - 1 : e;
    const double f = m - 1.0;
    const double den = 2.0 + f;
    const double rc = pgl_rcp(den);
    double s = f * rc;
    s = fma(fma(-den, s, f), rc, s);
    const double z = s * s;
    double R = C[14];
#pragma unroll
    for (int i = 15; i <= 20; ++i) R = fma(R, z, C[i]);
    R = R * z;
    const double hfsq = 0.5 * f * f;
    const double de = (double)e;
    double res = de * C[1] - ((hfsq - (s * (hfsq + R) + de * C[2])) - f);
    res = (v == 0.0) ? -__builtin_huge_val() : res;
    res = (v < __builtin_huge_val()) ? res : v;
    return res;
}

template <int NE, typename CP>
__device__ __forceinline__ void pgl_rate_terms_n(const double (&x)[NE], const double (&s)[NE],
                                                 const int nlin_, const double dt, double (&term)[NE],
                                                 double (&res)[NE], const CP C)
{
    const int nlin = nlin_ & 1;
    const bool allf64 = (nlin_ & 2) != 0;
    if (nlin == 1) {
        double e[NE], l1p[NE], inv[NE], lam[NE], sig[NE];
        bool small = true, spike = false, hi = (PGL_EPI_F32 != 0) && !allf64;
#pragma unroll
        for (int i = 0; i < NE; ++i) {
            hi = hi && (x[i] > 12.0);
            spike = spike || (s[i] > 0.0);
        }
        const bool fast = __all(hi);
        if (fast) {
#pragma unroll
            for (int i = 0; i < NE; ++i) e[i] = (double)__builtin_amdgcn_exp2f((float)x[i] * -1.44269504088896340736f);
        } else {
#pragma unroll
            for (int i = 0; i < NE; ++i) {
                e[i] = pgl_exp(-fabs(x[i]), C);
                small = small && (e[i] < C[23]);
            }
        }
        if (fast) {
#pragma unroll
            for (int i = 0; i < NE; ++i) {
                const double ei = e[i];
                l1p[i] = ei * fma(ei, -0.5, 1.0);
                inv[i] = fma(-ei, fma(-ei, fma(-ei, 1.0, 1.0), 1.0), 1.0);
            }
        } else if (__all(small)) {
#pragma unroll
            for (int i = 0; i < NE; ++i) {
                const double ei = e[i];
                l1p[i] = ei * fma(-ei, fma(-ei, fma(-ei, fma(-ei, 0.2, 0.25), C[22]), 0.5), 1.0);
                inv[i] = fma(-ei, fma(-ei, fma(-ei, fma(-ei, fma(-ei, 1.0, 1.0), 1.0), 1.0), 1.0), 1.0);
            }
        } else {
#pragma unroll
            for (int i = 0; i < NE; ++i) {
                const double u = 1.0 + e[i];
                inv[i] = pgl_rcp(u);
                l1p[i] = pgl_log(u, C) + (e[i] - (u - 1.0)) * inv[i];
            }
        }
#pragma unroll
        for (int i = 0; i < NE; ++i) {
            lam[i] = fmax(x[i], 0.0) + l1p[i];
            sig[i] = (x[i] >= 0.0) ? inv[i] : e[i] * inv[i];
            term[i] = -dt * lam[i];
            res[i] = -dt * sig[i];
        }
        if (spike) {
#pragma unroll
            for (int i = 0; i < NE; ++i) {
                const double tl = fma(pgl_log(lam[i], C), s[i], term[i]);
                const double rl = (-dt + s[i] * pgl_rcp(lam[i])) * sig[i];
                term[i] = (s[i] > 0.0) ? tl : term[i];
                res[i] = (s[i] > 0.0) ? rl : res[i];
            }
        }
#pragma unroll
        for (int i = 0; i < NE; ++i) {
            term[i] = (lam[i] == 0.0) ? __builtin_nan("") : term[i];
            res[i] = (lam[i] == 0.0 || x[i] != x[i]) ? __builtin_nan("") : res[i];
        }
    } else {
#pragma unroll
        for (int i = 0; i < NE; ++i) {
            const double lam = pgl_exp(x[i], C);
            term[i] = fma(x[i], s[i], -dt * lam);
            res[i] = fma(-dt, lam, s[i]);
        }
    }
}

#ifdef PGL_PROF
__device__ long long g_pgl_prof[2][4096][8][12];
__device__ long long g_pgl_prof_ts[4096][5];
#define PGL_PROF_ENTRY const long long prof_entry = __builtin_amdgcn_s_memrealtime();
#define PGL_PROF_EXIT                                                                              \
    do {                                                                                           \
        if (threadIdx.x == 0 && blockIdx.x < 4096) {                                               \
            g_pgl_prof_ts[blockIdx.x][0] = prof_entry;                                             \
            g_pgl_prof_ts[blockIdx.x][3] = __builtin_amdgcn_s_memrealtime();                       \
            g_pgl_prof_ts[blockIdx.x][4] = ((long long)__builtin_amdgcn_s_getreg((20 << 0) | (0 << 6) | (3 << 11)) << 16) | \
                                           (long long)__builtin_amdgcn_s_getreg((4 << 0) | (0 << 6) | (15 << 11));   \
        }                                                                                          \
    } while (0)
#define PGL_PROF_DECL long long prof_acc[12] = {0, 0, 0, 0, 0, 0, 0, 0, 0, 0, 0, 0}; long long prof_t = __builtin_amdgcn_s_memtime(); \
    const long long prof_rt0 = __builtin_amdgcn_s_memrealtime(), prof_t0 = prof_t;
#define PGL_PROF_MARK(i)                                           \
    do {                                                           \
        const long long t_ = __builtin_amdgcn_s_memtime();         \
        prof_acc[i] += t_ - prof_t;                                \
        prof_t = t_;                                               \
    } while (0)
#define PGL_PROF_STORE(pass)                                                                  \
    do {                                                                                      \
        prof_acc[10] = __builtin_amdgcn_s_memtime() - prof_t0;           \
        prof_acc[11] = __builtin_amdgcn_s_memrealtime() - prof_rt0;       \
        if (lane == 0 && blockIdx.x < 4096)                                                   \
            for (int i_ = 0; i_ < 12; ++i_) g_pgl_prof[pass - 1][blockIdx.x][wave][i_] = prof_acc[i_]; \
        if (threadIdx.x == 0 && blockIdx.x < 4096) {                                          \
            g_pgl_prof_ts[blockIdx.x][1] = prof_rt0;                                          \
            g_pgl_prof_ts[blockIdx.x][2] = prof_rt0 + prof_acc[11];                           \
        }                                                                                     \
    } while (0)
#else
#define PGL_PROF_ENTRY
#define PGL_PROF_EXIT
#define PGL_PROF_DECL
#define PGL_PROF_MARK(i)
#define PGL_PROF_STORE(pass)
#endif
#ifdef PGL_PROF
#define PGL_PROF_ARGS , long long (&prof_acc)[12], long long& prof_t
#define PGL_PROF_PASS , prof_acc, prof_t
#define PGL_PROF_DUMMY , pgl_prof_dummy_acc, pgl_prof_dummy_t
#else
#define PGL_PROF_ARGS
#define PGL_PROF_PASS
#define PGL_PROF_DUMMY
#endif
typedef double pgl_d2 __attribute__((ext_vector_type(2)));
typedef double pgl_d16 __attribute__((ext_vector_type(16)));
typedef const __attribute__((address_space(4))) double* pgl_k_cdp;
#define PGL_ROW __builtin_amdgcn_sched_barrier(0)

template <int NE, int CAP>
__device__ __forceinline__ bool pgl_rate_fx(const double (&x)[NE], const unsigned (&sc)[NE], const int nlin_,
                                            const double dt, const pgl_k_cdp C, double* scratch,
                                            const int lane, double& term, double (&res)[NE] PGL_PROF_ARGS)
{
    const int nlin = nlin_ & 1;
    const bool allf64 = (nlin_ & 2) != 0;
    double k[NE], r[NE], q[NE], e[NE];
    double c[14];
#pragma unroll
    for (int j = 0; j < 14; ++j) c[j] = C[j];
    const double c13 = C[22], cthr = C[23];
    double lam[NE], sig[NE];
    bool fastdone = false;
#if PGL_EPI_F32
    if (nlin == 1 && !allf64) {
        bool hi = true;
#pragma unroll
        for (int i = 0; i < NE; ++i) hi = hi && (x[i] > 12.0);
        if (__all(hi)) {
#pragma unroll
            for (int i = 0; i < NE; ++i) {
                const double ef = (double)__builtin_amdgcn_exp2f((float)x[i] * -1.44269504088896340736f);
                lam[i] = fma(ef, fma(ef, -0.5, 1.0), x[i]);
                sig[i] = fma(-ef, fma(-ef, fma(-ef, 1.0, 1.0), 1.0), 1.0);
            }
            fastdone = true;
        }
    }
#endif
    if (!fastdone) {
#pragma unroll
    for (int i = 0; i < NE; ++i) k[i] = rint((nlin == 1 ? -fabs(x[i]) : x[i]) * c[0]);
    PGL_ROW;
#pragma unroll
    for (int i = 0; i < NE; ++i) r[i] = fma(-k[i], c[1], (nlin == 1 ? -fabs(x[i]) : x[i]));
    PGL_ROW;
#pragma unroll
    for (int i = 0; i < NE; ++i) r[i] = fma(-k[i], c[2], r[i]);
    PGL_ROW;
#pragma unroll
    for (int i = 0; i < NE; ++i) q[i] = fma(c[3], r[i], c[4]);
    PGL_ROW;
#pragma unroll
    for (int j = 5; j <= 13; ++j) {
#pragma unroll
        for (int i = 0; i < NE; ++i) q[i] = fma(q[i], r[i], c[j]);
        PGL_ROW;
    }
#pragma unroll
    for (int i = 0; i < NE; ++i) q[i] = fma(q[i], r[i], 0.5);
    PGL_ROW;
#pragma unroll
    for (int i = 0; i < NE; ++i) q[i] = fma(q[i], r[i], 1.0);
    PGL_ROW;
#pragma unroll
    for (int i = 0; i < NE; ++i) q[i] = fma(q[i], r[i], 1.0);
    PGL_ROW;
#pragma unroll
    for (int i = 0; i < NE; ++i) k[i] = fmin(fmax(k[i], -2200.0), 2200.0);
    PGL_ROW;
#pragma unroll
    for (int i = 0; i < NE; ++i) e[i] = ldexp(q[i], (int)k[i]);
    PGL_ROW;
    PGL_PROF_MARK(7);
    if (nlin != 1) {
        double t = 0.0;
#pragma unroll
        for (int i = 0; i < NE; ++i) {
            const double sd = (double)sc[i];
            res[i] = fma(-dt, e[i], sd);
            t += fma(x[i], sd, -dt * e[i]);
        }
        term = t;
        return true;
    }
    bool small = true;
#pragma unroll
    for (int i = 0; i < NE; ++i) small = small && (e[i] < cthr);
    double l1p[NE], inv[NE];
    if (!__all(small)) {
#pragma unroll
        for (int i = 0; i < NE; ++i) {
            const double u = 1.0 + e[i];
            inv[i] = pgl_rcp(u);
            l1p[i] = pgl_log(u, C) + (e[i] - (u - 1.0)) * inv[i];
        }
        PGL_ROW;
    } else {
#pragma unroll
    for (int i = 0; i < NE; ++i) l1p[i] = fma(-e[i], 0.2, 0.25);
#pragma unroll
    for (int i = 0; i < NE; ++i) inv[i] = fma(-e[i], 1.0, 1.0);
    PGL_ROW;
#pragma unroll
    for (int i = 0; i < NE; ++i) l1p[i] = fma(-e[i], l1p[i], c13);
#pragma unroll
    for (int i = 0; i < NE; ++i) inv[i] = fma(-e[i], inv[i], 1.0);
    PGL_ROW;
#pragma unroll
    for (int i = 0; i < NE; ++i) l1p[i] = fma(-e[i], l1p[i], 0.5);
#pragma unroll
    for (int i = 0; i < NE; ++i) inv[i] = fma(-e[i], inv[i], 1.0);
    PGL_ROW;
#pragma unroll
    for (int i = 0; i < NE; ++i) l1p[i] = fma(-e[i], l1p[i], 1.0);
#pragma unroll
    for (int i = 0; i < NE; ++i) inv[i] = fma(-e[i], inv[i], 1.0);
    PGL_ROW;
#pragma unroll
    for (int i = 0; i < NE; ++i) l1p[i] = e[i] * l1p[i];
#pragma unroll
    for (int i = 0; i < NE; ++i) inv[i] = fma(-e[i], inv[i], 1.0);
    PGL_ROW;
    }
#pragma unroll
    for (int i = 0; i < NE; ++i) lam[i] = fmax(x[i], 0.0) + l1p[i];
#pragma unroll
    for (int i = 0; i < NE; ++i) sig[i] = (x[i] >= 0.0) ? inv[i] : e[i] * inv[i];
    PGL_ROW;
    }
    bool ok = true;
#pragma unroll
    for (int i = 0; i < NE; ++i) ok = ok && (lam[i] > 0.0);
    if (!__all(ok)) return false;
    double t = 0.0;
#pragma unroll
    for (int i = 0; i < NE; ++i) t = fma(-dt, lam[i], t);
    PGL_PROF_MARK(8);
    unsigned long long m[NE];
    int base[NE], total = 0;
#pragma unroll
    for (int i = 0; i < NE; ++i) {
        m[i] = __ballot(sc[i] != 0u);
        base[i] = total;
        total += __popcll(m[i]);
    }
    if (total == 0) {
#pragma unroll
        for (int i = 0; i < NE; ++i) res[i] = -dt * sig[i];
    } else if (total < CAP) {
        int slot[NE];
#pragma unroll
        for (int i = 0; i < NE; ++i) {
            slot[i] = base[i] + (int)__builtin_amdgcn_mbcnt_hi((unsigned)(m[i] >> 32),
                                         __builtin_amdgcn_mbcnt_lo((unsigned)m[i], 0u));
            if (sc[i] != 0u) scratch[slot[i]] = lam[i];
            slot[i] = (sc[i] != 0u) ? slot[i] : CAP - 1;
        }
        __builtin_amdgcn_wave_barrier();
        const double lc = (lane < total) ? scratch[lane] : 1.0;
        pgl_d2 LI;
        LI.x = pgl_log(lc, C);
        LI.y = pgl_rcp(lc);
        pgl_d2* const so = reinterpret_cast<pgl_d2*>(scratch + CAP);
        if (CAP == 64 || lane < CAP) so[lane] = LI;
        __builtin_amdgcn_wave_barrier();
        pgl_d2 g[NE];
#pragma unroll
        for (int i = 0; i < NE; ++i) g[i] = so[slot[i]];
#pragma unroll
        for (int i = 0; i < NE; ++i) {
            const double sd = (double)sc[i];
            t = fma(g[i].x, sd, t);
            res[i] = fma(sd, g[i].y, -dt) * sig[i];
        }
    } else {
#pragma unroll
        for (int i = 0; i < NE; ++i) {
            res[i] = -dt * sig[i];
            if (m[i] != 0ull) {
                const double sd = (double)sc[i];
                const double L = pgl_log(lam[i], C);
                const double I = pgl_rcp(lam[i]);
                t = (sc[i] != 0u) ? fma(L, sd, t) : t;
                res[i] = (sc[i] != 0u) ? fma(sd, I, -dt) * sig[i] : res[i];
            }
        }
    }
    PGL_PROF_MARK(9);
    term = t;
    return true;
}

__device__ __forceinline__ bool pgl_rate4(const double (&x)[4], const unsigned (&sc)[4], const int nlin,
                                          const double dt, const pgl_k_cdp C, double* scratch,
                                          const int lane, double& term, double (&res)[4] PGL_PROF_ARGS)
{
    return pgl_rate_fx<4, 64>(x, sc, nlin, dt, C, scratch, lane, term, res PGL_PROF_PASS);
}

template <typename CP>
__device__ __forceinline__ void pgl_rate_terms(const double x, const double s, const int nlin,
                                               const double dt, double& term, double& res,
                                               const CP C)
{
    const double xa[1] = {x}, sa[1] = {s};
    double ta[1], ra[1];
    pgl_rate_terms_n<1>(xa, sa, nlin, dt, ta, ra, C);
    term = ta[0];
    res = ra[0];
}

__device__ __forceinline__ double pgl_softplus_parts(double x, double& sig, double& loglam)
{
    const double e = exp(-fabs(x));
    const double lam = fmax(x, 0.0) + log1p(e);
    const double inv = 1.0 / (1.0 + e);
    sig = (x >= 0.0) ? inv : e * inv;
    loglam = log(lam);
    return lam;
}
```

theano_pyglm_amd/csrc/pglm_fused_resident.hip.h:

```cpp
#pragma once
__device__ __forceinline__ double conv_one(const int2* __restrict__ spk, int lo, int hi, int tg,
                                           int R, const double* __restrict__ phi_b)
{
    double a = 0.0;
    for (int j = lo; j < hi; ++j) {
        const int2 e = spk[j];
        const int d = tg - e.x - 1;
        if (d >= 0 && d < R) a = fma((double)e.y, phi_b[d], a);
    }
    return a;
}

__host__ __device__ constexpr int pgl_img_rsh(int kt) { return kt * 16 + 2; }
__host__ __device__ constexpr int pgl_img_row(int i) { return 2 * (i >> 2) + ((i & 1) << 3) + ((i >> 1) & 1); }
__host__ __device__ constexpr int pgl_img_brow(int grp) { return ((grp & 1) << 3) + (grp >> 1); }
__host__ __device__ constexpr int pgl_img_row_inv(int p) { return 4 * ((p & 7) >> 1) + ((p >> 3) & 1) + 2 * (p & 1); }
__host__ __device__ constexpr int pgl_img_bytes(int kt) { return ((16 * pgl_img_rsh(kt) * 8 + 1023) / 1024) * 1024; }

__global__ __launch_bounds__(256) void k_build_fimg(const int2* __restrict__ spk,
                                                    const int* __restrict__ wlo,
                                                    const int* __restrict__ whi,
                                                    const double* __restrict__ phi,
                                                    const double* __restrict__ fstim, long long nT,
                                                    int N, int B, int R, int Dstim, int ktl, int kth,
                                                    int tile0, unsigned char* __restrict__ Fimg,
                                                    int Nall, int np0, int DsAll, int ds0, int blk = 0)
{
    extern __shared__ __attribute__((aligned(16))) unsigned char smem[];
    double* phiS = reinterpret_cast<double*>(smem);
    for (int i = threadIdx.x; i < B * R; i += blockDim.x) phiS[i] = phi[i];
    __syncthreads();
    const int tile = tile0 + blockIdx.x, part = blockIdx.y;
    if (blk) {
        double* dstb = reinterpret_cast<double*>(Fimg + (size_t)blockIdx.x * ktl * 2048);
        const int Kimpb = N * B;
        for (int i = threadIdx.x; i < ktl * 256; i += blockDim.x) {
            const int kb = i >> 8, t = (i >> 4) & 15, pc = i & 15;
            const int col = kb * 16 + (pc ^ (2 * (t >> 1)));
            const long long tg = (long long)tile * 16 + t;
            double v = 0.0;
            if (col < Kimpb) {
                const int np = col / B, b = col - np * B;
                v = conv_one(spk, wlo[(size_t)tile * Nall + np0 + np], whi[(size_t)tile * Nall + np0 + np], (int)tg, R, phiS + b * R);
            } else if (col < Kimpb + Dstim) {
                v = (tg < nT) ? fstim[tg * DsAll + ds0 + (col - Kimpb)] : 0.0;
            }
            if (blk == 2) {
                float* dstf = reinterpret_cast<float*>(Fimg + (size_t)blockIdx.x * ktl * 1024) + kb * 256;
                const int e = i & 255, hi2 = e >> 7, l = (e & 127) >> 1;
                dstf[4 * l + 2 * hi2 + (e & 1)] = (float)v;
            } else {
                dstb[i] = v;
            }
        }
        return;
    }
    const int kt = part ? kth : ktl;
    const int rsh = pgl_img_rsh(kt), cw = kt * 16, cbeg = part ? ktl * 16 : 0, Kimp = N * B;
    const size_t imgl = (size_t)pgl_img_bytes(ktl), imgh = (gridDim.y > 1) ? (size_t)pgl_img_bytes(kth) : 0;
    double* dst = reinterpret_cast<double*>(Fimg + (size_t)blockIdx.x * (imgl + imgh) + (part ? imgl : 0));
    const int nel = (int)((part ? imgh : imgl) / 8);
    for (int i = threadIdx.x; i < nel; i += blockDim.x) {
        const int tp = i / rsh, c = i - tp * rsh;
        const int t = pgl_img_row_inv(tp & 15);
        double v = 0.0;
        if (tp < 16 && c < cw) {
            const int col = cbeg + c;
            const long long tg = (long long)tile * 16 + t;
            if (col < Kimp) {
                const int np = col / B, b = col - np * B;
                v = conv_one(spk, wlo[(size_t)tile * Nall + np0 + np], whi[(size_t)tile * Nall + np0 + np], (int)tg, R, phiS + b * R);
            } else if (col < Kimp + Dstim) {
                v = (tg < nT) ? fstim[tg * DsAll + ds0 + (col - Kimp)] : 0.0;
            }
        }
        dst[i] = v;
    }
}

template <int KT>
__device__ __forceinline__ void pgl_dma_half(const unsigned char* __restrict__ gimg, unsigned char* lds_dst,
                                             const int wave, const int lane)
{
    typedef __attribute__((address_space(1))) void gvoid;
    typedef __attribute__((address_space(3))) void lvoid;
    constexpr int NCH = pgl_img_bytes(KT) / 1024;
#pragma unroll
    for (int c0 = 0; c0 < NCH; c0 += 8) {
        const int c = c0 + wave;
        if (c < NCH)
            __builtin_amdgcn_global_load_lds((gvoid*)(gimg + (size_t)c * 1024 + lane * 16),
                                             (lvoid*)(lds_dst + (size_t)c * 1024), 16, 0, 0);
    }
}

template <int KT, int NWV>
__device__ __forceinline__ void pgl_dma_img(const unsigned char* __restrict__ gimg, unsigned char* lds_dst,
                                            const int wave, const int lane)
{
    typedef __attribute__((address_space(1))) void gvoid;
    typedef __attribute__((address_space(3))) void lvoid;
    constexpr int NCH = pgl_img_bytes(KT) / 1024;
#pragma unroll
    for (int c0 = 0; c0 < NCH; c0 += NWV) {
        const int c = c0 + wave;
        if (c < NCH)
            __builtin_amdgcn_global_load_lds((gvoid*)(gimg + (size_t)c * 1024 + lane * 16),
                                             (lvoid*)(lds_dst + (size_t)c * 1024), 16, 0, 0);
    }
}

template <int KT>
__device__ __forceinline__ void pgl_dma_round(const unsigned char* __restrict__ gimg, unsigned char* lds_dst,
                                              const int round, const int wave, const int lane)
{
    typedef __attribute__((address_space(1))) void gvoid;
    typedef __attribute__((address_space(3))) void lvoid;
    constexpr int NCH = pgl_img_bytes(KT) / 1024;
    const int c = round * 8 + wave;
    if (c < NCH) {
        const unsigned char* gs = gimg + (size_t)c * 1024;
        asm volatile("" : "+s"(gs));
        __builtin_amdgcn_global_load_lds((gvoid*)(gs + lane * 16), (lvoid*)(lds_dst + (size_t)c * 1024), 16, 0, 0);
    }
}

template <int KTL, int KTH, int PASS, int XIN = 0, int PART = 0, int HLP = 0>
__global__ __launch_bounds__(512, 2) void k_fused5(const FusedParams p)
{
    static_assert(!HLP || (KTL >= 2 && KTH >= 2), "helper waves: at least two k-tiles per column part");
    constexpr int TT = 16, NW = 8;
    constexpr int KT_ALL = KTL + KTH;
    constexpr int KS_ALL = 4 * KT_ALL;
    constexpr int KSL = 4 * KTL;
    constexpr int RSL = pgl_img_rsh(KTL), RSH = pgl_img_rsh(KTH);
    constexpr int IMGL = pgl_img_bytes(KTL), IMGH = pgl_img_bytes(KTH);
    constexpr int KTP = PART ? KTL : KTH;
    constexpr int IMGP = PART ? pgl_img_bytes(KTL) : pgl_img_bytes(KTH);
    constexpr size_t OFFP = PART ? 0 : (size_t)pgl_img_bytes(KTL);
    constexpr int KTG = (PASS == 1) ? KTL : KTP;
    constexpr bool FWO = (PASS == 1) && (XIN >= 2);
    constexpr bool XRD = (XIN == 1) || (XIN == 3);
    extern __shared__ __attribute__((aligned(16))) unsigned char smem[];
    PGL_PROF_ENTRY

    const int tid = threadIdx.x;
    const int lane = tid & 63;
    const int wave = __builtin_amdgcn_readfirstlane(tid >> 6);
    const int nPB = (p.nPT + NW - 1) / NW;
    const int pb = p.pb_major ? (int)blockIdx.x / p.nChunks : (int)blockIdx.x % nPB;
    const int chunk = p.pb_major ? (int)blockIdx.x % p.nChunks : (int)blockIdx.x / nPB;
    const int pt = pb * NW + wave;
    const bool active = pt < p.nPT;
    int role = 0, wpt = pt, hslot = 0;
    if constexpr (HLP != 0) {
        const int nb = (p.nPT - pb * NW < NW) ? p.nPT - pb * NW : NW;
        if (nb == 5) {
            role = (wave == 0 || wave == 4) ? 1 : ((wave == 5 || wave == 6) ? 2 : 0);
            wpt = pb * NW + ((wave == 5) ? 0 : ((wave == 6) ? 4 : wave));
            hslot = (wave == 4 || wave == 6) ? 1 : 0;
        } else if (nb == 6) {
            role = (wave <= 1) ? 1 : ((wave >= 6) ? 2 : 0);
            wpt = pb * NW + ((wave >= 6) ? wave - 6 : wave);
            hslot = (wave == 1 || wave == 7) ? 1 : 0;
        } else if (nb <= 4) {
            int ht = -1;
            if (nb == 4) ht = (wave >= 4) ? wave - 4 : -1;
            else if (nb == 3) ht = (wave == 3) ? 0 : ((wave == 7) ? 1 : ((wave == 5) ? 2 : -1));
            else if (nb == 2) ht = (wave == 2 || wave == 3) ? wave - 2 : -1;
            else ht = (wave == 1) ? 0 : -1;
            role = (wave < nb) ? 1 : ((ht >= 0) ? 2 : 0);
            wpt = pb * NW + ((ht >= 0) ? ht : wave);
            hslot = (ht >= 0) ? ht : ((wave < nb) ? wave : 0);
        }
        role = __builtin_amdgcn_readfirstlane(role);
        wpt = __builtin_amdgcn_readfirstlane(wpt);
        hslot = __builtin_amdgcn_readfirstlane(hslot);
    }
    const bool helper = (HLP != 0) && role == 2;
    const bool works = active || helper;
    constexpr int QS = ((4 * (KTL + KTH)) / 2 + 3) / 4 * 4;
    constexpr int KTPH = ((PART ? KTL : KTH) + 1) / 2;

    unsigned char* buf0 = smem;
    unsigned char* buf2 = smem + IMGL;
    unsigned char* buf1 = smem + ((PASS == 1) ? 2 * IMGL : IMGP);
    double* Cs = reinterpret_cast<double*>(smem + ((PASS == 1) ? 2 * IMGL + IMGH : 2 * IMGP));
    if (tid < 32) Cs[tid] = PGL_C[tid];


    const int col = lane & 15;
    const int grp = lane >> 4;
    const int nloc = pt * 16 + col;
    const bool valid_n = active && (nloc < p.npost);
    const int nglob = p.pidx ? p.pidx[valid_n ? nloc : 0] : p.n_lo + (valid_n ? nloc : 0);

    const int tile_beg = p.tile0 + chunk * p.tilesPerChunk;
    int tile_end = tile_beg + p.tilesPerChunk;
    if (tile_end > p.tile0 + p.nTiles) tile_end = p.tile0 + p.nTiles;
    double* const rslab = p.Xbuf + ((size_t)(works ? wpt : 0)) * 256 + lane;
    const size_t rstride = (size_t)p.nPT * 256;
    const unsigned char* __restrict__ fimg = p.Fimg - (size_t)p.img_tile0 * (IMGL + IMGH);
    constexpr size_t IMGS = (size_t)IMGL + IMGH;

    constexpr int NRL = (IMGL / 1024 + 7) / 8, NRH = (IMGH / 1024 + 7) / 8;
    constexpr int NR0 = (PASS == 1 || PART) ? NRL : NRH, NR1 = (PASS == 1) ? NRH : 0;
    constexpr int RSG = (PASS == 1 || PART) ? RSL : RSH;
    auto bwd_part = [&](auto k0c, auto nkc, auto& G, const int krt, const unsigned char* Fb, const double (&rq)[4],
                        const unsigned char* g0, unsigned char* l0, const unsigned char* g1, unsigned char* l1,
                        const bool dma) {
        constexpr int K0 = decltype(k0c)::value, NK = decltype(nkc)::value;
        const double* fb = reinterpret_cast<const double*>(Fb) + pgl_img_brow(grp) * RSG + col + 16 * (K0 + krt);
        constexpr int NS = 4 * NK;
        constexpr int PD = (NS < PGL_PD) ? NS : PGL_PD;
        constexpr int NRT = NR0 + NR1;
        constexpr int DSFULL = NS / NRT;
        constexpr int DSCAP = (PGL_DS1 > 0) ? PGL_DS1 : NS;
        constexpr int DSTEP = (NS >= 2 * NRT) ? ((DSFULL < DSCAP) ? DSFULL : DSCAP) : 0;
        double ar[PD];
#pragma unroll
        for (int s = 0; s < PD; ++s) ar[s] = pgl_lds_f64(fb + (2 * (s / NK)) * RSG + 16 * (s % NK));
        auto round = [&](const int j) {
            if (j < NR0) {
                pgl_dma_round<(PASS == 1 || PART) ? KTL : KTH>(g0, l0, j, wave, lane);
            } else {
                pgl_dma_round<KTH>(g1, l1, j - NR0, wave, lane);
            }
        };
        if (DSTEP == 0 && dma) {
#pragma unroll
            for (int j = 0; j < NRT; ++j) round(j);
        }
        const int phase = (wave < 4) ? ((DSTEP > 1) ? DSTEP / 2 - 1 : 0) : DSTEP - 1;
        if (PGL_PRIO && wave >= 4) __builtin_amdgcn_s_setprio(1);
#pragma unroll
        for (int s = 0; s < NS; ++s) {
            if (PGL_PRIO && s == NS / 2 && wave >= 4) __builtin_amdgcn_s_setprio(0);
            const double a = ar[s % PD];
            if (s + PD < NS) ar[s % PD] = pgl_lds_f64(fb + (2 * ((s + PD) / NK)) * RSG + 16 * ((s + PD) % NK));
            G[s % NK] = __builtin_amdgcn_mfma_f64_16x16x4f64(a, rq[s / NK], G[s % NK], 0, 0, 0);
            if ((s & 3) == 3) __builtin_amdgcn_sched_barrier(0);
            if (DSTEP > 0) {
                constexpr int DS = (DSTEP > 0) ? DSTEP : 1;
                const int j = s / DS;
                const int ph = s % DS;
                if ((ph == DS - 1 || (DS > 1 && ph == DS / 2 - 1)) && j < NRT) {
                    if (ph == phase && dma) round(j);
                    __builtin_amdgcn_sched_barrier(0);
                }
            }
        }
    };
    if constexpr (PASS == 1) {
        d4_t G[KTL];
#pragma unroll
        for (int kt = 0; kt < KTL; ++kt) G[kt] = (d4_t){0.0, 0.0, 0.0, 0.0};
        double ll_acc = 0.0, gb_acc = 0.0;
        const double bias_l = valid_n ? p.bias[nloc] : (p.nlin == 1 ? 30.0 : 0.0);
        const double* __restrict__ wrow = p.Wfrag + (size_t)(works ? wpt : 0) * KS_ALL * 64;
        double* const wscratch = reinterpret_cast<double*>(smem + 2 * IMGL + IMGH + 256) + wave * 192;
        double* const Xh = reinterpret_cast<double*>(smem + 2 * IMGL + IMGH + 256) + NW * 192 + hslot * 256 + lane;
        if (tile_beg < tile_end) {
            pgl_dma_half<KTL>(fimg + (size_t)tile_beg * IMGS, buf0, wave, lane);
            pgl_dma_half<KTH>(fimg + (size_t)tile_beg * IMGS + IMGL, buf1, wave, lane);
        }
        unsigned scb[4] = {0u, 0u, 0u, 0u}, scn[4] = {0u, 0u, 0u, 0u};
        const uint8_t* cnt_ptr = p.S + ((size_t)tile_beg * TT + grp) * p.Nall + nglob;
        const int cnt_r1 = 4 * p.Nall, cnt_tile = TT * p.Nall;
        auto load_counts = [&](unsigned (&dst)[4]) {
#pragma unroll
            for (int r = 0; r < 4; ++r) dst[r] = cnt_ptr[r * cnt_r1];
            cnt_ptr += cnt_tile;
        };
        if (tile_beg < tile_end) load_counts(scn);
        __builtin_amdgcn_s_waitcnt(0x0f70);
        __syncthreads();
        PGL_PROF_DECL
        for (int tile = tile_beg; tile < tile_end; ++tile) {
            const int t0 = tile * TT;
            const int par = (tile - tile_beg) & 1;
            const unsigned char* Lb = par ? buf2 : buf0;
            unsigned char* Ln = par ? buf0 : buf2;
            const bool more = tile + 1 < tile_end;
#pragma unroll
            for (int r = 0; r < 4; ++r) scb[r] = scn[r];
            d4_t acc0 = (d4_t){0.0, 0.0, 0.0, 0.0};
            d4_t acc1 = (d4_t){0.0, 0.0, 0.0, 0.0};
            auto forward = [&](auto q0c, auto q1c) {
                constexpr int Q0 = decltype(q0c)::value, Q1 = decltype(q1c)::value, NQ = Q1 - Q0;
                constexpr int PW2 = (NQ / 2 < PGL_PW / 2) ? NQ / 2 : PGL_PW / 2;
                static_assert(Q0 % 2 == 0 && NQ % 2 == 0 && NQ >= 2, "whole fragment pairs");
                const double* faL = reinterpret_cast<const double*>(Lb) + pgl_img_row(col) * RSL + grp;
                const double* faH = reinterpret_cast<const double*>(buf1) + pgl_img_row(col) * RSH + grp;
                const double* wr_s = wrow;
                asm volatile("" : "+s"(wr_s));
                constexpr int PA = 4;
                pgl_d2 wr[PW2];
                double ar[PA];
                auto afrag = [&](const int s) -> double {
                    return (s < KSL) ? pgl_lds_f64(faL + 4 * s) : pgl_lds_f64(faH + 4 * (s - KSL));
                };
                pgl_glb_cd2p wr_base[KS_ALL / 8 + 1];
#pragma unroll
                for (int b4 = Q0 / 8; b4 < (Q1 + 7) / 8; ++b4) {
                    const double* bs = wr_s + (size_t)b4 * 512;
                    asm volatile("" : "+s"(bs));
                    wr_base[b4] = (pgl_glb_cd2p)bs;
                }
#pragma unroll
                for (int q = 0; q < PW2; ++q) {
                    const int pair = Q0 / 2 + q;
                    wr[q] = wr_base[pair / 4][(pair % 4) * 64 + lane];
                }
#pragma unroll
                for (int q = 0; q < PA; ++q) ar[q] = afrag(Q0 + q);
                if (PGL_PRIO && wave >= 4) __builtin_amdgcn_s_setprio(1);
#pragma unroll
                for (int q = Q0; q < Q1; ++q) {
                    if (PGL_PRIO && q == Q0 + NQ / 2 && wave >= 4) __builtin_amdgcn_s_setprio(0);
                    const double a = ar[(q - Q0) % PA];
                    const double b = (q & 1) ? wr[((q - Q0) / 2) % PW2].y : wr[((q - Q0) / 2) % PW2].x;
                    if (q + PA < Q1) ar[(q - Q0) % PA] = afrag(q + PA);
                    if ((q & 1) && ((q - Q0) / 2 + PW2 < NQ / 2)) {
                        const int pair = q / 2 + PW2;
                        wr[((q - Q0) / 2) % PW2] = wr_base[pair / 4][(pair % 4) * 64 + lane];
                    }
                    if (q & 1)
                        acc1 = __builtin_amdgcn_mfma_f64_16x16x4f64(a, b, acc1, 0, 0, 0);
                    else
                        acc0 = __builtin_amdgcn_mfma_f64_16x16x4f64(a, b, acc0, 0, 0, 0);
                    if (((q - Q0) & 3) == 3) __builtin_amdgcn_sched_barrier(0);
                }
            };
            if (works && !PGL_DBG(8)) {
                if constexpr (HLP != 0) {
                    if (role == 1) forward(std::integral_constant<int, 0>{}, std::integral_constant<int, QS>{});
                    else if (role == 2) forward(std::integral_constant<int, QS>{}, std::integral_constant<int, KS_ALL>{});
                    else forward(std::integral_constant<int, 0>{}, std::integral_constant<int, KS_ALL>{});
                } else {
                    forward(std::integral_constant<int, 0>{}, std::integral_constant<int, KS_ALL>{});
                }
            }
            if constexpr (HLP != 0) {
                if (helper) {
#pragma unroll
                    for (int r = 0; r < 4; ++r) Xh[r * 64] = acc0[r] + acc1[r];
                }
            }
            PGL_PROF_MARK(0);
            const bool do_bwd = !FWO && active && p.want_grad && !PGL_DBG(16);
            double xin[XRD ? 4 : 1];
            if constexpr (XRD) {
                const double* xs_ = rslab + (size_t)(tile - p.tile0) * rstride;
#pragma unroll
                for (int r = 0; r < 4; ++r) xin[r] = xs_[r * 64];
            }
            __syncthreads();
            PGL_PROF_MARK(2);
            double xh[(HLP != 0) ? 4 : 1];
            if constexpr (HLP != 0) {
#pragma unroll
                for (int r = 0; r < 4; ++r) xh[r] = (role == 1) ? Xh[r * 64] : 0.0;
            }
            double rr[4];
            if constexpr (FWO) {
                if (active) {
                    double* rs = rslab + (size_t)(tile - p.tile0) * rstride;
#pragma unroll
                    for (int r = 0; r < 4; ++r) {
                        double x = acc0[r] + acc1[r];
                        if constexpr (HLP != 0) x += xh[r];
                        if constexpr (XRD) x += xin[r];
                        rs[r * 64] = x;
                    }
                }
#pragma unroll
                for (int r = 0; r < 4; ++r) rr[r] = 0.0;
            } else if (active) {
                bool done = false;
                if (PGL_ENE == 4 && !PGL_DBG(4) && (long long)t0 + TT <= p.t_hi) {
                    double xs[4], term4 = 0.0;
#pragma unroll
                    for (int r = 0; r < 4; ++r) {
                        if constexpr (HLP != 0) xs[r] = bias_l + ((acc0[r] + acc1[r]) + xh[r]);
                        else xs[r] = bias_l + (acc0[r] + acc1[r]);
                    }
                    if constexpr (XRD) {
#pragma unroll
                        for (int r = 0; r < 4; ++r) xs[r] += xin[r];
                    }
                    const double* cg = PGL_C;
                    asm volatile("" : "+s"(cg));
                    done = pgl_rate4(xs, scb, p.nlin | p.epi64, p.dt, (pgl_k_cdp)cg, wscratch, lane, term4, rr PGL_PROF_PASS);
                    if (done) {
                        ll_acc += term4;
#pragma unroll
                        for (int r = 0; r < 4; ++r) gb_acc += rr[r];
                    }
                }
                constexpr int ENE = (PGL_ENE == 4) ? 2 : PGL_ENE;
                if (!done) {
#pragma unroll
                    for (int h2 = 0; h2 < 4 / ENE; ++h2) {
                        double xe[ENE], se[ENE], terme[ENE], rese[ENE];
                        bool vte[ENE];
#pragma unroll
                        for (int e = 0; e < ENE; ++e) {
                            const int r = ENE * h2 + e;
                            if constexpr (HLP != 0) xe[e] = bias_l + ((acc0[r] + acc1[r]) + xh[r]);
                            else xe[e] = bias_l + (acc0[r] + acc1[r]);
                            if constexpr (XRD) xe[e] += xin[r];
                            se[e] = (double)scb[r];
                            const long long tg = (long long)t0 + grp + 4 * r;
                            vte[e] = valid_n && (tg < p.t_hi);
                        }
                        if PGL_DBG(4) {
#pragma unroll
                            for (int e = 0; e < ENE; ++e) {
                                terme[e] = xe[e] * se[e];
                                rese[e] = xe[e] - se[e];
                            }
                        } else {
                            pgl_lds_cdp Cl = (pgl_lds_cdp)Cs;
                            asm volatile("" : "+v"(Cl));
                            pgl_rate_terms_n<ENE>(xe, se, p.nlin | p.epi64, p.dt, terme, rese, Cl);
                        }
#pragma unroll
                        for (int e = 0; e < ENE; ++e) {
                            const double res = vte[e] ? rese[e] : 0.0;
                            rr[ENE * h2 + e] = res;
                            ll_acc += vte[e] ? terme[e] : 0.0;
                            gb_acc += res;
                        }
                    }
                }
            } else {
#pragma unroll
                for (int r = 0; r < 4; ++r) rr[r] = 0.0;
            }
            PGL_PROF_MARK(1);
            if (PGL_EBAR) __syncthreads();
            if (more) load_counts(scn);
            if (!do_bwd && more) {
                pgl_dma_half<KTL>(fimg + (size_t)(tile + 1) * IMGS, Ln, wave, lane);
                pgl_dma_half<KTH>(fimg + (size_t)(tile + 1) * IMGS + IMGL, buf1, wave, lane);
            }
            PGL_PROF_MARK(3);
            if (do_bwd) {
                double* rs = rslab + (size_t)(tile - p.tile0) * rstride;
#pragma unroll
                for (int r = 0; r < 4; ++r) rs[r * 64] = rr[r];
                bwd_part(std::integral_constant<int, 0>{}, std::integral_constant<int, KTL>{}, G, 0, Lb, rr,
                         fimg + (size_t)(tile + 1) * IMGS, Ln, fimg + (size_t)(tile + 1) * IMGS + IMGL, buf1, more);
            }
            PGL_PROF_MARK(4);
            __builtin_amdgcn_s_waitcnt(0x0f70);
            PGL_PROF_MARK(5);
            __syncthreads();
            PGL_PROF_MARK(6);
        }
        PGL_PROF_STORE(1);
        if (active && !FWO) {
            pgl_store_ll(p, chunk, pt, 0, 1, lane, ll_acc, gb_acc);
        }
        if (active && p.want_grad && !FWO) {
            double* gp = pgl_gpart(p.Gpart, pt, KT_ALL, 0, p.nChunks, chunk, lane);
            const size_t gcs = (size_t)p.nChunks * 64;
#pragma unroll
            for (int kt = 0; kt < KTL; ++kt) {
#pragma unroll
                for (int r = 0; r < 4; ++r) gp[(kt * 4 + r) * gcs] = G[kt][r];
            }
        }
    } else {
        auto pass2 = [&](auto nkc, const int krt, const int kskip) {
            constexpr int NK = decltype(nkc)::value;
            d4_t G[NK];
#pragma unroll
            for (int kt = 0; kt < NK; ++kt) G[kt] = (d4_t){0.0, 0.0, 0.0, 0.0};
            double rv[4] = {0.0, 0.0, 0.0, 0.0}, rn[4] = {0.0, 0.0, 0.0, 0.0};
            if (tile_beg < tile_end) {
                pgl_dma_half<KTP>(fimg + (size_t)tile_beg * IMGS + OFFP, buf0, wave, lane);
                if (works) {
#pragma unroll
                    for (int r = 0; r < 4; ++r) rn[r] = rslab[(size_t)(tile_beg - p.tile0) * rstride + r * 64];
                }
            }
            PGL_PROF_DECL
            for (int tile = tile_beg; tile < tile_end; ++tile) {
                const int par = (tile - tile_beg) & 1;
                const unsigned char* Hb = par ? buf1 : buf0;
                unsigned char* Hn = par ? buf0 : buf1;
                __builtin_amdgcn_s_waitcnt(0x0f70);
                PGL_PROF_MARK(0);
#pragma unroll
                for (int r = 0; r < 4; ++r) rv[r] = rn[r];
                __syncthreads();
                PGL_PROF_MARK(1);
                const bool more = tile + 1 < tile_end;
                const bool do_bwd = works && !PGL_DBG(16);
                if (more) {
                    if (!do_bwd) pgl_dma_half<KTP>(fimg + (size_t)(tile + 1) * IMGS + OFFP, Hn, wave, lane);
                    if (works) {
#pragma unroll
                        for (int r = 0; r < 4; ++r) rn[r] = rslab[(size_t)(tile + 1 - p.tile0) * rstride + r * 64];
                    }
                }
                PGL_PROF_MARK(2);
                if (do_bwd)
                    bwd_part(std::integral_constant<int, 0>{}, nkc, G, krt, Hb, rv, fimg + (size_t)(tile + 1) * IMGS + OFFP, Hn,
                             nullptr, nullptr, more);
                PGL_PROF_MARK(3);
            }
            PGL_PROF_STORE(2);
            if (works) {
                double* gp = pgl_gpart(p.Gpart, wpt, KT_ALL, (PART ? 0 : KTL) + krt, p.nChunks, chunk, lane);
                const size_t gcs = (size_t)p.nChunks * 64;
#pragma unroll
                for (int kt = 0; kt < NK; ++kt) {
                    if (HLP == 0 || kt >= kskip) {
#pragma unroll
                        for (int r = 0; r < 4; ++r) gp[(kt * 4 + r) * gcs] = G[kt][r];
                    }
                }
            }
        };
        if constexpr (HLP != 0) {
            if (role != 0) pass2(std::integral_constant<int, KTPH>{}, (role == 2) ? KTP - KTPH : 0, (role == 2) ? 2 * KTPH - KTP : 0);
            else pass2(std::integral_constant<int, KTP>{}, 0, 0);
        } else {
            pass2(std::integral_constant<int, KTP>{}, 0, 0);
        }
    }
    PGL_PROF_EXIT;
}

template <int KTW, int PTW, int MT, int NW, int DB = 1>
__global__ __launch_bounds__(NW * 64, 2) void k_fused6(const FusedParams p)
{
    constexpr int TT = 16;
    constexpr int KSPLIT = NW / PTW;
    constexpr int KSW = KTW * 4;
    constexpr int KT_ALL = KTW * KSPLIT;
    constexpr int KS_ALL = KSW * KSPLIT;
    constexpr int RS = pgl_img_rsh(KT_ALL);
    constexpr int IMG = pgl_img_bytes(KT_ALL);
    extern __shared__ __attribute__((aligned(16))) unsigned char smem[];
    PGL_PROF_ENTRY

    const int tid = threadIdx.x;
    const int lane = tid & 63;
    const int wave = __builtin_amdgcn_readfirstlane(tid >> 6);
    const int ptl = wave % PTW;
    const int ksl = wave / PTW;
    const int nPB = (p.nPT + PTW - 1) / PTW;
    const int pb = blockIdx.x % nPB;
    const int chunk = blockIdx.x / nPB;
    const int pt = pb * PTW + ptl;
    const bool active = pt < p.nPT;

    unsigned char* bufs = smem;
    double* Xp = reinterpret_cast<double*>(smem + (size_t)(DB ? 2 : 1) * MT * IMG);
    double* Rb = Xp;
    constexpr int RBS = NW;
    double* Cs = Xp + (size_t)MT * NW * 256;
    double* const wscratch = Cs + 32 + wave * 48;
    if (tid < 32) Cs[tid] = PGL_C[tid];

    d4_t G[KTW];
#pragma unroll
    for (int kt = 0; kt < KTW; ++kt) G[kt] = (d4_t){0.0, 0.0, 0.0, 0.0};
    double ll_acc = 0.0, gb_acc = 0.0;

    const int col = lane & 15;
    const int grp = lane >> 4;
    const int nloc = pt * 16 + col;
    const bool valid_n = active && (nloc < p.npost);
    const int nglob = p.pidx ? p.pidx[valid_n ? nloc : 0] : p.n_lo + (valid_n ? nloc : 0);
    const double bias_l = valid_n ? (p.theta ? p.theta[(size_t)nloc * p.P] : p.bias[nloc]) : (p.nlin == 1 ? 30.0 : 0.0);
    const double* __restrict__ wrow =
        p.Wfrag + ((size_t)(active ? pt : 0) * KS_ALL + (size_t)ksl * KSW) * 64;
    const int kcol0 = ksl * KTW * 16;
    constexpr int EPW = (KSPLIT >= 4) ? 1 : 4 / KSPLIT;
    int er[EPW];
#pragma unroll
    for (int e = 0; e < EPW; ++e) er[e] = (KSPLIT == 8) ? (ksl >> 1) : (KSPLIT == 4) ? ksl : ksl * EPW + e;
    const bool emine = (KSPLIT == 8) ? ((lane >> 5) == (ksl & 1)) : true;

    const int tile_beg = p.tile0 + chunk * p.tilesPerChunk;
    int tile_end = tile_beg + p.tilesPerChunk;
    if (tile_end > p.tile0 + p.nTiles) tile_end = p.tile0 + p.nTiles;
    const unsigned char* __restrict__ fimg = p.Fimg - (size_t)p.img_tile0 * IMG;

    auto dma_step = [&](const int tile0s, unsigned char* dst) {
#pragma unroll
        for (int m = 0; m < MT; ++m)
            if (tile0s + m < tile_end)
                pgl_dma_img<KT_ALL, NW>(fimg + (size_t)(tile0s + m) * IMG, dst + (size_t)m * IMG, wave, lane);
    };
    if (tile_beg < tile_end) dma_step(tile_beg, bufs);
    double wreg[KSW];
#pragma unroll
    for (int s = 0; s < KSW; ++s) wreg[s] = 0.0;
    if (active && p.theta) {
        pgl_wfrag_direct<KSW>(p, ksl * KSW, grp, nloc, nglob, valid_n, wreg);
    } else if (active) {
        const pgl_d2* wr2 = reinterpret_cast<const pgl_d2*>(wrow);
#pragma unroll
        for (int s2 = 0; s2 < KSW / 2; ++s2) {
            const pgl_d2 v = wr2[s2 * 64 + lane];
            wreg[2 * s2] = v.x;
            wreg[2 * s2 + 1] = v.y;
        }
    }

    unsigned scn[MT * EPW];
    const uint8_t* cptr[EPW];
    const int last_tile = p.nT16 - 1;
#pragma unroll
    for (int e = 0; e < EPW; ++e)
        cptr[e] = p.S + ((size_t)(tile_beg < last_tile ? tile_beg : last_tile) * TT + grp + 4 * er[e]) * p.Nall + nglob;
    const size_t ctile = (size_t)TT * p.Nall;
    auto load_counts = [&](const int tile0s) {
#pragma unroll
        for (int m = 0; m < MT; ++m) {
            const size_t moff = (tile0s + m <= last_tile) ? (size_t)m * ctile : 0;
#pragma unroll
            for (int e = 0; e < EPW; ++e) scn[m * EPW + e] = cptr[e][moff];
        }
#pragma unroll
        for (int e = 0; e < EPW; ++e) cptr[e] += (size_t)MT * ctile;
    };
    load_counts(tile_beg);
    constexpr bool BREG = (DB == 0 && MT == 1 && KTW <= 5);
    double fbreg[BREG ? 4 * KTW : 1], fareg[BREG ? KSW : 1];
    int par = 0;
    PGL_PROF_DECL
    for (int tile = tile_beg; tile < tile_end; tile += MT, par ^= 1) {
        const unsigned char* cur = bufs + (size_t)(DB ? par : 0) * MT * IMG;
        __builtin_amdgcn_s_waitcnt(0x0f70);
        PGL_PROF_MARK(0);
        __syncthreads();
        PGL_PROF_MARK(1);
        double sc[MT * EPW];
        unsigned scu[MT * EPW];
#pragma unroll
        for (int i = 0; i < MT * EPW; ++i) {
            scu[i] = scn[i];
            sc[i] = (double)scn[i];
        }
        const bool more = tile + MT < tile_end;
        unsigned char* const nxt = bufs + (size_t)(DB ? (par ^ 1) : 0) * MT * IMG;
        constexpr int NCH = IMG / 1024, PPI = (NCH + NW - 1) / NW, PWV = MT * PPI, NMF = MT * KSW;
        constexpr int DS = (DB && PGL_DMA_IL && NMF >= PWV) ? NMF / PWV : 0;
        auto piece = [&](const int j) {
            typedef __attribute__((address_space(1))) void gvoid;
            typedef __attribute__((address_space(3))) void lvoid;
            const int m = j / PPI, cc = (j % PPI) * NW + wave;
            if (cc < NCH && tile + MT + m < tile_end) {
// ... 820 lines not shown
```

Before: 316.9.

## Precompute packed per-tile spike records to skip in-kernel ballots in epilogue

Adds a small kernel that packs each tile's spike counts together with the precomputed compaction slots and the nonzero total into one uint2 per lane. The records are cached per neuron range. The two-pass resident kernel then loads one 8-byte record per tile instead of four strided byte loads from the spike matrix, and skips the per-tile ballot/popcount/mbcnt work in the rate epilogue. Row-slab and weight-fragment pointers also become incrementing scalar pointers to cut address arithmetic and register use. In exchange there is an extra build pass and buffer when the cache misses, a cache that must be invalidated correctly, and a debug export API.

```diff
diff --git a/include/pyglm_hip.h b/include/pyglm_hip.h
--- a/include/pyglm_hip.h
+++ b/include/pyglm_hip.h
@@ -149,6 +149,9 @@
 
 int pgl_info(pgl_handle h, int n_lo, int n_hi, double* info, int n_info);
 
+int pgl_spike_records(pgl_handle h, int n_lo, int n_hi, const int* d_idx, uint32_t* rec_out, long long cap_words,
+                      long long* dims);
+
 #ifdef __cplusplus
 }
 #endif
diff --git a/theano_pyglm_amd/_lib.py b/theano_pyglm_amd/_lib.py
--- a/theano_pyglm_amd/_lib.py
+++ b/theano_pyglm_amd/_lib.py
@@ -28,6 +28,7 @@
     'pgl_bfgs_state_doubles', 'pgl_bfgs_init_dev', 'pgl_bfgs_trial_dev', 'pgl_bfgs_objective_dev',
     'pgl_bfgs_linesearch_dev', 'pgl_bfgs_hmul_dev', 'pgl_bfgs_hmul_hist_dev', 'pgl_bfgs_update_dev', 'pgl_bfgs_step_dev', 'pgl_plan_kernels', 'pgl_last_kernels', 'pgl_leading_singular_pairs',
     'pgl_hvp_prepare_dev', 'pgl_hvp_prepare_list_dev', 'pgl_hvp_apply_dev', 'pgl_hvp',
+    'pgl_spike_records',
     'pgl_ncg_state_doubles', 'pgl_ncg_init_dev', 'pgl_ncg_cg_step_dev', 'pgl_ncg_trial_dev', 'pgl_ncg_search_step_dev',
 ]
 
@@ -130,6 +131,8 @@
         lib.pgl_ncg_trial_dev.argtypes = [vp, vp, C.c_int, C.c_int, vp, C.c_int, vp]
         lib.pgl_ncg_search_step_dev.argtypes = ([vp, vp, C.c_int, C.c_int, vp, C.c_int, vp, vp, vp, C.c_int] +
                                                 [C.c_double] * 6 + [C.c_int, vp, vp, vp, vp])
+    if hasattr(lib, 'pgl_spike_records'):
+        lib.pgl_spike_records.argtypes = [vp, C.c_int, C.c_int, vp, vp, C.c_longlong, vp]
     lib.pgl_features.argtypes = [vp, vp]
     lib.pgl_impulse_currents.argtypes = [vp, vp, vp]
     lib.pgl_state.argtypes = [vp, C.c_int, vp, vp, vp, vp, vp]
@@ -457,6 +460,14 @@
                 'bytes', 'events', 'kernel_version', 'resident_feature_bytes', 'streamed_bytes', 'stim_path']
         return dict(zip(keys, v.tolist()))
 
+    def spike_records(self, n_lo=0, n_hi=None, d_idx=0):
+        n_hi = self.N if n_hi is None else n_hi
+        dims = np.zeros(4, dtype=np.int64)
+        _chk(self.lib.pgl_spike_records(self.h, int(n_lo), int(n_hi), C.c_void_p(d_idx or None), None, 0, _ptr(dims)))
+        rec = np.zeros((int(dims[0]), int(dims[1]), 64, 2), dtype=np.uint32)
+        _chk(self.lib.pgl_spike_records(self.h, int(n_lo), int(n_hi), C.c_void_p(d_idx or None), _ptr(rec), rec.size, _ptr(dims)))
+        return rec, int(dims[2]), int(dims[3])
+
     def features(self):
         out = np.empty((self.nT, self.N, self.B))
         _chk(self.lib.pgl_features(self.h, _ptr(out)))
diff --git a/theano_pyglm_amd/csrc/pglm_capi.hip b/theano_pyglm_amd/csrc/pglm_capi.hip
--- a/theano_pyglm_amd/csrc/pglm_capi.hip
+++ b/theano_pyglm_amd/csrc/pglm_capi.hip
@@ -62,6 +62,16 @@
     ImgSlot imgs[NIMG];
     int img_cur = 0;
     unsigned long long img_clock = 0;
+    struct RecSlot {
+        DevBuf buf;
+        bool valid = false;
+        int n_lo = 0, npost = 0, tile0 = 0, ntiles = 0;
+        unsigned long long stamp = 0;
+    };
+    static constexpr int NREC = 4;
+    RecSlot recs[NREC], rec_list;
+    const void* rec_cur = nullptr;
+    long long rec_builds = 0;
     double* pin_out = nullptr;
     DevBuf IimpT, Inet, Istim, tmpA, tmpB, tmpC, wsmall, part, outK, lam, wcol, thetan;
     bool sep = false;
@@ -132,6 +142,7 @@
 {
     h->hvp_ok = false;
     for (int i = 0; i < pgl_context::NIMG; ++i) h->imgs[i].key = 0;
+    for (int i = 0; i < pgl_context::NREC; ++i) h->recs[i].valid = false;
 }
 static bool img_room(const pgl_context* h, size_t want)
 {
@@ -251,7 +262,8 @@
                       &h->wsmall, &h->part, &h->outK, &h->lam, &h->wcol, &h->thetan, &h->GX, &h->gtheta,
                       &h->gargs, &h->gpart, &h->gout, &h->ghs, &h->gfs, &h->zf, &h->zfT, &h->sbt, &h->Yf, &h->Qb, &h->Qf,
                       &h->spart, &h->sepC, &h->sepA, &h->sepAT, &h->sepD, &h->YfT, &h->Hb, &h->wpart, &h->QvT, &h->staA,
-                      &h->Cbuf, &h->hvp_idx, &h->hvp_Weff, &h->hvp_ll, &h->hvp_v, &h->hvp_out};
+                      &h->Cbuf, &h->hvp_idx, &h->hvp_Weff, &h->hvp_ll, &h->hvp_v, &h->hvp_out,
+                      &h->recs[0].buf, &h->recs[1].buf, &h->recs[2].buf, &h->recs[3].buf, &h->rec_list.buf};
     for (DevBuf* b : bufs) release(*b);
     for (int s = 0; s < pgl_context::NEV; ++s)
         for (int i = 0; i < 4; ++i)
@@ -923,6 +935,7 @@
     fp.pidx = h->cur_pidx;
     fp.theta = nullptr; fp.Weff = nullptr; fp.P = 1 + h->Dstim + h->Kimp;
     fp.epi64 = h->opt_epi64 ? 2 : 0;
+    fp.Srec = (const uint2*)h->rec_cur;
 }
 
 static bool plan_reads_theta(const Plan& pl)
@@ -1007,6 +1020,38 @@
     return PGL_OK;
 }
 
+static size_t srec_bytes(const Plan& pl) { return (size_t)pl.nTiles * pl.nPT * 64 * sizeof(uint2); }
+static int ensure_spike_records(pgl_handle h, const Plan& pl, int n_lo)
+{
+    if (g_dry || pl.version != 5) return PGL_OK;
+    pgl_context::RecSlot* rs = &h->rec_list;
+    if (!h->cur_pidx) {
+        rs = nullptr;
+        for (int i = 0; i < pgl_context::NREC; ++i) {
+            pgl_context::RecSlot& c = h->recs[i];
+            if (c.valid && c.n_lo == n_lo && c.npost == pl.npost && c.tile0 == pl.tile0 && c.ntiles == pl.nTiles && c.buf.p) {
+                c.stamp = ++h->img_clock;
+                h->rec_cur = c.buf.p;
+                return PGL_OK;
+            }
+        }
+        rs = &h->recs[0];
+        for (int i = 0; i < pgl_context::NREC; ++i)
+            if (!h->recs[i].valid) { rs = &h->recs[i]; break; }
+            else if (h->recs[i].stamp < rs->stamp) rs = &h->recs[i];
+    }
+    rs->valid = false;
+    ENSURE(rs->buf, srec_bytes(pl));
+    hipLaunchKernelGGL(k_build_srec, dim3((unsigned)pl.nTiles, (unsigned)pl.nPT), dim3(64), 0, h->stream,
+                       (const uint8_t*)h->S.p, h->cur_pidx, n_lo, pl.npost, h->N, pl.tile0, (uint2*)rs->buf.p);
+    HIPCHK(hipGetLastError());
+    ++h->rec_builds;
+    rs->valid = !h->cur_pidx;
+    rs->n_lo = n_lo; rs->npost = pl.npost; rs->tile0 = pl.tile0; rs->ntiles = pl.nTiles;
+    rs->stamp = ++h->img_clock;
+    h->rec_cur = rs->buf.p;
+    return PGL_OK;
+}
 
 struct KernelRecord {
     explicit KernelRecord(pgl_context* h)
@@ -1162,6 +1207,8 @@
         ENSURE(h->Xbuf, (size_t)pl.nTiles * pl.nPT * 256 * 8);
         rc = ensure_plan_images(h, pl);
         if (rc) return rc;
+        rc = ensure_spike_records(h, pl, n_lo);
+        if (rc) return rc;
         if (rec) HIPCHK(hipEventRecord(h->ev[1], h->stream));
         SepfParams sp{};
         const bool fused_fwd = pl.version == 7 && fused7_built(pl.KT, pl.nw7, 2) && h->sepA_ok && h->opt_sepf != 3;
@@ -1225,6 +1272,8 @@
         }
         rc = ensure_plan_images(h, pl);
         if (rc) return rc;
+        rc = ensure_spike_records(h, pl, n_lo);
+        if (rc) return rc;
         FusedParams fp;
         fill_params(h, pl, slices[0], n_lo, d_grad != nullptr, 0, fp);
         if (direct) {
@@ -1246,6 +1295,10 @@
             int rc = ensure_feature_images(h, plans[i].ktl, plans[i].kth, p0.tile0, p0.nTiles, &slices[i], (int)i);
             if (rc) return rc;
             slot[i] = h->img_cur;
+        }
+        {
+            int rc = ensure_spike_records(h, plans[S - 1], n_lo);
+            if (rc) return rc;
         }
         if (rec) HIPCHK(hipEventRecord(h->ev[1], h->stream));
         auto params = [&](const size_t i, FusedParams& fp) {
@@ -1940,6 +1993,10 @@
         }
         v[11] += 2.0 * (double)plans.size() * (double)pl.nTiles * pl.nPT * 2048.0;
     }
+    if (plans.back().version == 5 && (!sliced || wide)) {
+        v[10] += (double)srec_bytes(plans.back());
+        v[11] += (double)srec_bytes(plans.back());
+    }
     v[0] = pl.blocks; v[1] = pl.threads; v[2] = pl.nChunks; v[3] = pl.KT; v[4] = (double)pl.lds;
     v[5] = 16;
     const double nrows = (double)(h->t_hi - h->t_lo);
@@ -1948,6 +2005,34 @@
            8.0 * pl.npost * (1.0 + P);
     v[8] = (double)h->nnz;
     for (int i = 0; i < n_info && i < 13; ++i) info[i] = v[i];
+    return PGL_OK;
+}
+
+int pgl_spike_records(pgl_handle h, int n_lo, int n_hi, const int* d_idx, uint32_t* rec_out, long long cap_words, long long* dims)
+{
+    int rc = check_ready(h);
+    if (rc) return rc;
+    if (!dims) return fail(PGL_ERR_ARG, "null argument");
+    if (n_lo < 0 || n_hi > h->N || n_lo >= n_hi || (d_idx && n_lo != 0)) return fail(PGL_ERR_ARG, "bad neuron range");
+    HIPCHK(hipSetDevice(h->device));
+    std::vector<Slice> slices;
+    std::vector<Plan> plans;
+    bool sepf = false, sliced = false, wide = false;
+    h->cur_pidx = d_idx;
+    rc = select_plans(h, n_lo, n_hi, slices, plans, sepf, sliced, &wide);
+    const bool two_pass = rc == PGL_OK && plans.back().version == 5 && (!sliced || wide);
+    if (two_pass && rec_out) rc = ensure_spike_records(h, plans.back(), n_lo);
+    h->cur_pidx = nullptr;
+    if (rc) return rc;
+    if (!two_pass) return fail(PGL_ERR_STATE, "these neurons are not evaluated by the two-pass kernel on resident tiles");
+    const Plan& pl = plans.back();
+    dims[0] = pl.nTiles; dims[1] = pl.nPT; dims[2] = pl.tile0; dims[3] = h->rec_builds;
+    if (rec_out) {
+        const long long words = (long long)(srec_bytes(pl) / 4);
+        if (cap_words < words) return fail(PGL_ERR_ARG, "record buffer too small");
+        HIPCHK(hipMemcpyAsync(rec_out, h->rec_cur, (size_t)words * 4, hipMemcpyDeviceToHost, h->stream));
+    }
+    HIPCHK(hipStreamSynchronize(h->stream));
     return PGL_OK;
 }
 
diff --git a/theano_pyglm_amd/csrc/pglm_common.hip.h b/theano_pyglm_amd/csrc/pglm_common.hip.h
--- a/theano_pyglm_amd/csrc/pglm_common.hip.h
+++ b/theano_pyglm_amd/csrc/pglm_common.hip.h
@@ -107,7 +107,19 @@
     long long sepB0;
     int sepSL;
     int pb_major;
+    const uint2* __restrict__ Srec;
 };
+
+__device__ __forceinline__ uint2 pgl_srec_pack(const unsigned (&sc)[4], const int (&slot)[4], const int total)
+{
+    uint2 v;
+    v.x = sc[0] | sc[1] << 8 | sc[2] << 16 | sc[3] << 24;
+    const unsigned tc = total < 64 ? (unsigned)total : 64u;
+    v.y = (unsigned)slot[0] | (unsigned)slot[1] << 6 | (unsigned)slot[2] << 12 | (unsigned)slot[3] << 18 | tc << 24 |
+          (total >= 64 ? 0x80000000u : 0u);
+    return v;
+}
+__device__ __forceinline__ unsigned pgl_srec_count(const uint2 rec, const int r) { return (rec.x >> (8 * r)) & 0xffu; }
 
 __device__ __forceinline__ void pgl_store_ll(const FusedParams& p, const int chunk, const int pt, const int sub,
                                              const int nsub, const int lane, double ll, double gb)
@@ -364,11 +376,13 @@
 typedef const __attribute__((address_space(4))) double* pgl_k_cdp;
 #define PGL_ROW __builtin_amdgcn_sched_barrier(0)
 
-template <int NE, int CAP>
+template <int NE, int CAP, bool REC = false>
 __device__ __forceinline__ bool pgl_rate_fx(const double (&x)[NE], const unsigned (&sc)[NE], const int nlin_,
                                             const double dt, const pgl_k_cdp C, double* scratch,
-                                            const int lane, double& term, double (&res)[NE] PGL_PROF_ARGS)
-{
+                                            const int lane, double& term, double (&res)[NE] PGL_PROF_ARGS,
+                                            const unsigned rec_y = 0u)
+{
+    static_assert(!REC || (NE == 4 && CAP == 64), "spike records: four elements per lane, a list of 64");
     const int nlin = nlin_ & 1;
     const bool allf64 = (nlin_ & 2) != 0;
     double k[NE], r[NE], q[NE], e[NE];
@@ -495,23 +509,35 @@
     PGL_PROF_MARK(8);
     unsigned long long m[NE];
     int base[NE], total = 0;
-#pragma unroll
-    for (int i = 0; i < NE; ++i) {
-        m[i] = __ballot(sc[i] != 0u);
-        base[i] = total;
-        total += __popcll(m[i]);
+    if constexpr (REC) {
+        total = (int)(__builtin_amdgcn_readfirstlane(rec_y) >> 24 & 0x7fu);
+    } else {
+#pragma unroll
+        for (int i = 0; i < NE; ++i) {
+            m[i] = __ballot(sc[i] != 0u);
+            base[i] = total;
+            total += __popcll(m[i]);
+        }
     }
     if (total == 0) {
 #pragma unroll
         for (int i = 0; i < NE; ++i) res[i] = -dt * sig[i];
     } else if (total < CAP) {
         int slot[NE];
+        if constexpr (REC) {
+#pragma unroll
+            for (int i = 0; i < NE; ++i) {
+                slot[i] = (int)(rec_y >> (6 * i) & 63u);
+                scratch[slot[i]] = lam[i];
+            }
+        } else {
 #pragma unroll
         for (int i = 0; i < NE; ++i) {
             slot[i] = base[i] + (int)__builtin_amdgcn_mbcnt_hi((unsigned)(m[i] >> 32),
                                          __builtin_amdgcn_mbcnt_lo((unsigned)m[i], 0u));
             if (sc[i] != 0u) scratch[slot[i]] = lam[i];
             slot[i] = (sc[i] != 0u) ? slot[i] : CAP - 1;
+        }
         }
         __builtin_amdgcn_wave_barrier();
         const double lc = (lane < total) ? scratch[lane] : 1.0;
@@ -534,6 +560,7 @@
 #pragma unroll
         for (int i = 0; i < NE; ++i) {
             res[i] = -dt * sig[i];
+            if constexpr (REC) m[i] = __ballot(sc[i] != 0u);
             if (m[i] != 0ull) {
                 const double sd = (double)sc[i];
                 const double L = pgl_log(lam[i], C);
@@ -555,6 +582,14 @@
     return pgl_rate_fx<4, 64>(x, sc, nlin, dt, C, scratch, lane, term, res PGL_PROF_PASS);
 }
 
+__device__ __forceinline__ bool pgl_rate4_rec(const double (&x)[4], const uint2 rec, const int nlin,
+                                              const double dt, const pgl_k_cdp C, double* scratch,
+                                              const int lane, double& term, double (&res)[4] PGL_PROF_ARGS)
+{
+    const unsigned sc[4] = {pgl_srec_count(rec, 0), pgl_srec_count(rec, 1), pgl_srec_count(rec, 2), pgl_srec_count(rec, 3)};
+    return pgl_rate_fx<4, 64, true>(x, sc, nlin, dt, C, scratch, lane, term, res PGL_PROF_PASS, rec.y);
+}
+
 template <typename CP>
 __device__ __forceinline__ void pgl_rate_terms(const double x, const double s, const int nlin,
                                                const double dt, double& term, double& res,
diff --git a/theano_pyglm_amd/csrc/pglm_fused_resident.hip.h b/theano_pyglm_amd/csrc/pglm_fused_resident.hip.h
--- a/theano_pyglm_amd/csrc/pglm_fused_resident.hip.h
+++ b/theano_pyglm_amd/csrc/pglm_fused_resident.hip.h
@@ -76,6 +76,33 @@
         }
         dst[i] = v;
     }
+}
+
+__global__ __launch_bounds__(64) void k_build_srec(const uint8_t* __restrict__ S, const int* __restrict__ pidx, int n_lo,
+                                                   int npost, int Nall, int tile0, uint2* __restrict__ rec)
+{
+    const int lane = threadIdx.x, col = lane & 15, grp = lane >> 4;
+    const int pt = blockIdx.y, nPT = gridDim.y;
+    const int nloc = pt * 16 + col;
+    const bool valid_n = nloc < npost;
+    const int nglob = pidx ? pidx[valid_n ? nloc : 0] : n_lo + (valid_n ? nloc : 0);
+    const uint8_t* cp = S + ((size_t)(tile0 + blockIdx.x) * 16 + grp) * Nall + nglob;
+    unsigned sc[4];
+    unsigned long long m[4];
+    int base[4], slot[4], total = 0;
+#pragma unroll
+    for (int r = 0; r < 4; ++r) {
+        sc[r] = cp[(size_t)r * 4 * Nall];
+        m[r] = __ballot(sc[r] != 0u);
+        base[r] = total;
+        total += __popcll(m[r]);
+    }
+#pragma unroll
+    for (int r = 0; r < 4; ++r) {
+        const int rank = base[r] + (int)__builtin_amdgcn_mbcnt_hi((unsigned)(m[r] >> 32), __builtin_amdgcn_mbcnt_lo((unsigned)m[r], 0u));
+        slot[r] = (sc[r] != 0u && total < 64) ? rank : 63;
+    }
+    rec[((size_t)blockIdx.x * nPT + pt) * 64 + lane] = pgl_srec_pack(sc, slot, total);
 }
 
 template <int KT>
@@ -198,7 +225,6 @@
     const int tile_beg = p.tile0 + chunk * p.tilesPerChunk;
     int tile_end = tile_beg + p.tilesPerChunk;
     if (tile_end > p.tile0 + p.nTiles) tile_end = p.tile0 + p.nTiles;
-    double* const rslab = p.Xbuf + ((size_t)(works ? wpt : 0)) * 256 + lane;
     const size_t rstride = (size_t)p.nPT * 256;
     const unsigned char* __restrict__ fimg = p.Fimg - (size_t)p.img_tile0 * (IMGL + IMGH);
     constexpr size_t IMGS = (size_t)IMGL + IMGH;
@@ -260,19 +286,21 @@
         const double* __restrict__ wrow = p.Wfrag + (size_t)(works ? wpt : 0) * KS_ALL * 64;
         double* const wscratch = reinterpret_cast<double*>(smem + 2 * IMGL + IMGH + 256) + wave * 192;
         double* const Xh = reinterpret_cast<double*>(smem + 2 * IMGL + IMGH + 256) + NW * 192 + hslot * 256 + lane;
+        const int tile_whole = __builtin_amdgcn_readfirstlane((int)(p.t_hi >> 4));
         if (tile_beg < tile_end) {
             pgl_dma_half<KTL>(fimg + (size_t)tile_beg * IMGS, buf0, wave, lane);
             pgl_dma_half<KTH>(fimg + (size_t)tile_beg * IMGS + IMGL, buf1, wave, lane);
         }
-        unsigned scb[4] = {0u, 0u, 0u, 0u}, scn[4] = {0u, 0u, 0u, 0u};
-        const uint8_t* cnt_ptr = p.S + ((size_t)tile_beg * TT + grp) * p.Nall + nglob;
-        const int cnt_r1 = 4 * p.Nall, cnt_tile = TT * p.Nall;
-        auto load_counts = [&](unsigned (&dst)[4]) {
-#pragma unroll
-            for (int r = 0; r < 4; ++r) dst[r] = cnt_ptr[r * cnt_r1];
-            cnt_ptr += cnt_tile;
+        uint2 recb = make_uint2(0u, 0u), recn = make_uint2(0u, 0u);
+        const uint2* rec_s = p.Srec + ((size_t)(tile_beg - p.tile0) * p.nPT + (active ? pt : 0)) * 64;
+        const size_t rec_tile = (size_t)p.nPT * 64;
+        auto load_rec = [&]() {
+            asm volatile("" : "+s"(rec_s));
+            if constexpr (!FWO) recn = rec_s[lane];
+            rec_s += rec_tile;
         };
-        if (tile_beg < tile_end) load_counts(scn);
+        if (tile_beg < tile_end) load_rec();
+        double* rs_s = p.Xbuf + (size_t)(tile_beg - p.tile0) * rstride + (size_t)(works ? wpt : 0) * 256;
         __builtin_amdgcn_s_waitcnt(0x0f70);
         __syncthreads();
         PGL_PROF_DECL
@@ -282,8 +310,10 @@
             const unsigned char* Lb = par ? buf2 : buf0;
             unsigned char* Ln = par ? buf0 : buf2;
             const bool more = tile + 1 < tile_end;
-#pragma unroll
-            for (int r = 0; r < 4; ++r) scb[r] = scn[r];
+            recb = recn;
+            asm volatile("" : "+s"(rs_s));
+            double* const rs_t = rs_s + lane;
+            rs_s += rstride;
             d4_t acc0 = (d4_t){0.0, 0.0, 0.0, 0.0};
             d4_t acc1 = (d4_t){0.0, 0.0, 0.0, 0.0};
             auto forward = [&](auto q0c, auto q1c) {
@@ -300,18 +330,14 @@
                 auto afrag = [&](const int s) -> double {
                     return (s < KSL) ? pgl_lds_f64(faL + 4 * s) : pgl_lds_f64(faH + 4 * (s - KSL));
                 };
-                pgl_glb_cd2p wr_base[KS_ALL / 8 + 1];
-#pragma unroll
-                for (int b4 = Q0 / 8; b4 < (Q1 + 7) / 8; ++b4) {
-                    const double* bs = wr_s + (size_t)b4 * 512;
-                    asm volatile("" : "+s"(bs));
-                    wr_base[b4] = (pgl_glb_cd2p)bs;
-                }
-#pragma unroll
-                for (int q = 0; q < PW2; ++q) {
-                    const int pair = Q0 / 2 + q;
-                    wr[q] = wr_base[pair / 4][(pair % 4) * 64 + lane];
-                }
+                const double* wr_cur = wr_s + (size_t)(Q0 / 8) * 512;
+                auto wload = [&](const int pair) -> pgl_d2 {
+                    if (pair % 4 == 0 && pair != (Q0 / 8) * 4) wr_cur += 512;
+                    asm volatile("" : "+s"(wr_cur));
+                    return ((pgl_glb_cd2p)wr_cur)[(pair % 4) * 64 + lane];
+                };
+#pragma unroll
+                for (int q = 0; q < PW2; ++q) wr[q] = wload(Q0 / 2 + q);
 #pragma unroll
                 for (int q = 0; q < PA; ++q) ar[q] = afrag(Q0 + q);
                 if (PGL_PRIO && wave >= 4) __builtin_amdgcn_s_setprio(1);
@@ -322,8 +348,7 @@
                     const double b = (q & 1) ? wr[((q - Q0) / 2) % PW2].y : wr[((q - Q0) / 2) % PW2].x;
                     if (q + PA < Q1) ar[(q - Q0) % PA] = afrag(q + PA);
                     if ((q & 1) && ((q - Q0) / 2 + PW2 < NQ / 2)) {
-                        const int pair = q / 2 + PW2;
-                        wr[((q - Q0) / 2) % PW2] = wr_base[pair / 4][(pair % 4) * 64 + lane];
+                        wr[((q - Q0) / 2) % PW2] = wload(q / 2 + PW2);
                     }
                     if (q & 1)
                         acc1 = __builtin_amdgcn_mfma_f64_16x16x4f64(a, b, acc1, 0, 0, 0);
@@ -351,9 +376,8 @@
             const bool do_bwd = !FWO && active && p.want_grad && !PGL_DBG(16);
             double xin[XRD ? 4 : 1];
             if constexpr (XRD) {
-                const double* xs_ = rslab + (size_t)(tile - p.tile0) * rstride;
-#pragma unroll
-                for (int r = 0; r < 4; ++r) xin[r] = xs_[r * 64];
+#pragma unroll
+                for (int r = 0; r < 4; ++r) xin[r] = rs_t[r * 64];
             }
             __syncthreads();
             PGL_PROF_MARK(2);
@@ -365,20 +389,19 @@
             double rr[4];
             if constexpr (FWO) {
                 if (active) {
-                    double* rs = rslab + (size_t)(tile - p.tile0) * rstride;
 #pragma unroll
                     for (int r = 0; r < 4; ++r) {
                         double x = acc0[r] + acc1[r];
                         if constexpr (HLP != 0) x += xh[r];
                         if constexpr (XRD) x += xin[r];
-                        rs[r * 64] = x;
+                        rs_t[r * 64] = x;
                     }
                 }
 #pragma unroll
                 for (int r = 0; r < 4; ++r) rr[r] = 0.0;
             } else if (active) {
                 bool done = false;
-                if (PGL_ENE == 4 && !PGL_DBG(4) && (long long)t0 + TT <= p.t_hi) {
+                if (PGL_ENE == 4 && !PGL_DBG(4) && tile < tile_whole) {
                     double xs[4], term4 = 0.0;
 #pragma unroll
                     for (int r = 0; r < 4; ++r) {
@@ -391,7 +414,7 @@
                     }
                     const double* cg = PGL_C;
                     asm volatile("" : "+s"(cg));
-                    done = pgl_rate4(xs, scb, p.nlin | p.epi64, p.dt, (pgl_k_cdp)cg, wscratch, lane, term4, rr PGL_PROF_PASS);
+                    done = pgl_rate4_rec(xs, recb, p.nlin | p.epi64, p.dt, (pgl_k_cdp)cg, wscratch, lane, term4, rr PGL_PROF_PASS);
                     if (done) {
                         ll_acc += term4;
 #pragma unroll
@@ -410,7 +433,7 @@
                             if constexpr (HLP != 0) xe[e] = bias_l + ((acc0[r] + acc1[r]) + xh[r]);
                             else xe[e] = bias_l + (acc0[r] + acc1[r]);
                             if constexpr (XRD) xe[e] += xin[r];
-                            se[e] = (double)scb[r];
+                            se[e] = (double)pgl_srec_count(recb, r);
                             const long long tg = (long long)t0 + grp + 4 * r;
                             vte[e] = valid_n && (tg < p.t_hi);
                         }
@@ -440,16 +463,15 @@
             }
             PGL_PROF_MARK(1);
             if (PGL_EBAR) __syncthreads();
-            if (more) load_counts(scn);
+            if (more) load_rec();
             if (!do_bwd && more) {
                 pgl_dma_half<KTL>(fimg + (size_t)(tile + 1) * IMGS, Ln, wave, lane);
                 pgl_dma_half<KTH>(fimg + (size_t)(tile + 1) * IMGS + IMGL, buf1, wave, lane);
             }
             PGL_PROF_MARK(3);
             if (do_bwd) {
-                double* rs = rslab + (size_t)(tile - p.tile0) * rstride;
-#pragma unroll
-                for (int r = 0; r < 4; ++r) rs[r * 64] = rr[r];
+#pragma unroll
+                for (int r = 0; r < 4; ++r) rs_t[r * 64] = rr[r];
                 bwd_part(std::integral_constant<int, 0>{}, std::integral_constant<int, KTL>{}, G, 0, Lb, rr,
                          fimg + (size_t)(tile + 1) * IMGS, Ln, fimg + (size_t)(tile + 1) * IMGS + IMGL, buf1, more);
             }
@@ -479,12 +501,16 @@
 #pragma unroll
             for (int kt = 0; kt < NK; ++kt) G[kt] = (d4_t){0.0, 0.0, 0.0, 0.0};
             double rv[4] = {0.0, 0.0, 0.0, 0.0}, rn[4] = {0.0, 0.0, 0.0, 0.0};
+            const double* rn_s = p.Xbuf + (size_t)(tile_beg - p.tile0) * rstride + (size_t)(works ? wpt : 0) * 256;
+            auto load_r = [&]() {
+                asm volatile("" : "+s"(rn_s));
+#pragma unroll
+                for (int r = 0; r < 4; ++r) rn[r] = rn_s[lane + r * 64];
+                rn_s += rstride;
+            };
             if (tile_beg < tile_end) {
                 pgl_dma_half<KTP>(fimg + (size_t)tile_beg * IMGS + OFFP, buf0, wave, lane);
-                if (works) {
-#pragma unroll
-                    for (int r = 0; r < 4; ++r) rn[r] = rslab[(size_t)(tile_beg - p.tile0) * rstride + r * 64];
-                }
+                if (works) load_r();
             }
             PGL_PROF_DECL
             for (int tile = tile_beg; tile < tile_end; ++tile) {
@@ -501,10 +527,7 @@
                 const bool do_bwd = works && !PGL_DBG(16);
                 if (more) {
                     if (!do_bwd) pgl_dma_half<KTP>(fimg + (size_t)(tile + 1) * IMGS + OFFP, Hn, wave, lane);
-                    if (works) {
-#pragma unroll
-                        for (int r = 0; r < 4; ++r) rn[r] = rslab[(size_t)(tile + 1 - p.tile0) * rstride + r * 64];
-                    }
+                    if (works) load_r();
                 }
                 PGL_PROF_MARK(2);
                 if (do_bwd)
```

After: 317.0, median of 3. Within noise of the previous version (+0.0%).
